# danieldugas/DeepMimic_mujoco

Hardware: AMD Instinct MI355X
Metric: env-steps/sec (whole node), 34-DoF humanoid, 4096 envs, at 1/2/4/8 MI355X (higher is better)
Workload: dtype f32

## Files before the change

deepmimic_mujoco_amd/_lib.py:

```python
from __future__ import annotations

import ctypes as C
import os

import numpy as np

from .model import DmModel, NQ, NV, NU, NOBS

_HERE = os.path.dirname(os.path.abspath(__file__))
LIB_PATH = os.path.join(_HERE, "libdeepmimic_hip.so")
DEBUG_STRIDE = 416

REASONS = {0: None, 1: "low_z", 2: "high_z", 3: "max_ep_len", 4: "acyclical_end",
           5: "sim_error", 6: "obs_out_of_bounds", 7: "fallen without amnesty"}
TASK_DPENV, TASK_COMBINED = 0, 1

EXPORTS = ["dm_default_config", "dm_create", "dm_destroy", "dm_last_error", "dm_num_envs",
           "dm_load_clip", "dm_set_env_clips", "dm_reset", "dm_step", "dm_step_forced", "dm_physics_step",
           "dm_set_state", "dm_get_state", "dm_get_counters", "dm_set_counters", "dm_set_debug",
           "dm_fill_random_actions", "dm_last_step_ms", "dm_enable_timing", "dm_get_work",
           "dm_set_clip_flags", "dm_obs_dim", "dm_terms_dim", "dm_get_env_clips", "dm_mean_step_ms", "dm_ppo_loss", "dm_forward", "dm_linear_wgrad", "dm_ppo_gather", "dm_flat_adam_step", "dm_policy_sample",
           "dm_rollout_store", "dm_policy_pack", "dm_policy_forward", "dm_policy_packed_floats", "dm_ppo_mlp_grad", "dm_ppo_mlp_workspace_floats", "dm_flat_adam_update", "dm_flat_adam_step_gather", "dm_colsum", "dm_set_seed",
           "dm_linear_tanh", "dm_tanh_linear_wgrad", "dm_tanh_bwd_colsum",
           "dm_ppo_wide_grad", "dm_ppo_wide_packed_elems", "dm_ppo_wide_dp", "dm_ppo_wide_supported",
           "dm_sac_act", "dm_sac_store", "dm_sac_gather", "dm_sac_head_fwd", "dm_sac_critic_loss", "dm_sac_actor_loss",
           "dm_sac_head_bwd", "dm_sac_linear_relu", "dm_sac_relu_bwd_colsum", "dm_sac_polyak",
           "dm_rollout_finish", "dm_rollout_finish_workspace_bytes",
           "dm_policy_forward_bf16", "dm_rollout_store_bf16", "dm_ppo_gather_bf16", "dm_flat_adam_step_gather_bf16"]


class DmConfig(C.Structure):
    _fields_ = [("num_envs", C.c_int32), ("max_ep_length", C.c_int32),
                ("vel_obs_scale", C.c_float), ("low_z", C.c_float), ("high_z", C.c_float),
                ("w_pose", C.c_float), ("w_vel", C.c_float), ("w_end_eff", C.c_float),
                ("w_com", C.c_float), ("w_joint_limit", C.c_float), ("obs_bound", C.c_float),
                ("seed", C.c_uint64), ("auto_reset", C.c_int32), ("device", C.c_int32),
                ("lpt_schedule", C.c_int32), ("task", C.c_int32),
                ("amnesty_steps", C.c_int32), ("to_getup_len", C.c_int32),
                ("integrator", C.c_int32), ("stale_contact_slots", C.c_int32)]


INTEGRATORS = {None: 0, "model": 0, "Euler": 1, "euler": 1, "RK4": 2, "rk4": 2}


class DmPpoMlpStep(C.Structure):
    _fields_ = [("B", C.c_int32), ("D", C.c_int32), ("H1", C.c_int32), ("H2", C.c_int32), ("A", C.c_int32),
                ("normalize_advantage", C.c_int32), ("clip_range", C.c_float), ("vf_coef", C.c_float), ("ent_coef", C.c_float),
                ("reserved", C.c_int32),
                ("obs", C.c_void_p), ("act", C.c_void_p), ("adv", C.c_void_p), ("ret", C.c_void_p), ("old_logp", C.c_void_p),
                ("log_std", C.c_void_p),
                ("W", (C.c_void_p * 3) * 2), ("b", (C.c_void_p * 3) * 2), ("gW", (C.c_void_p * 3) * 2), ("gb", (C.c_void_p * 3) * 2),
                ("g_log_std", C.c_void_p), ("out8", C.c_void_p), ("workspace", C.c_void_p), ("workspace_floats", C.c_longlong),
                ("zero_ptr", C.c_void_p), ("zero_floats", C.c_longlong), ("adam_state2", C.c_void_p), ("loss_acc", C.c_void_p)]


class DmGatherSpec(C.Structure):
    _fields_ = [("idx", C.c_void_p), ("B", C.c_int32), ("D", C.c_int32), ("A", C.c_int32), ("reserved", C.c_int32),
                ("obs", C.c_void_p), ("act", C.c_void_p), ("adv", C.c_void_p), ("ret", C.c_void_p), ("logp", C.c_void_p),
                ("o_obs", C.c_void_p), ("o_act", C.c_void_p), ("o_adv", C.c_void_p), ("o_ret", C.c_void_p), ("o_logp", C.c_void_p)]


class DmGatherSpecBf16(DmGatherSpec):
    """include/deepmimic_hip.h: DmGatherSpecBf16 — DmGatherSpec's layout; obs / act point at bf16 rows"""


class DmPpoWideStep(C.Structure):
    _fields_ = [("B", C.c_int32), ("D", C.c_int32), ("H1", C.c_int32), ("H2", C.c_int32), ("A", C.c_int32),
                ("normalize_advantage", C.c_int32), ("clip_range", C.c_float), ("vf_coef", C.c_float), ("ent_coef", C.c_float),
                ("reserved", C.c_int32),
                ("obs", C.c_void_p), ("act", C.c_void_p), ("adv", C.c_void_p), ("ret", C.c_void_p), ("old_logp", C.c_void_p),
                ("log_std", C.c_void_p),
                ("W", (C.c_void_p * 3) * 2), ("b", (C.c_void_p * 3) * 2), ("gW", (C.c_void_p * 3) * 2), ("gb", (C.c_void_p * 3) * 2),
                ("g_log_std", C.c_void_p),
                ("wpk", C.c_void_p * 2), ("xbT", C.c_void_p), ("h1T", C.c_void_p * 2), ("dz1T", C.c_void_p * 2), ("h2T", C.c_void_p * 2),
                ("dz2T", C.c_void_p * 2), ("dz3T", C.c_void_p * 2), ("part", C.c_void_p), ("stats8", C.c_void_p), ("out8", C.c_void_p),
                ("zero_ptr", C.c_void_p), ("zero_floats", C.c_longlong), ("adam_state2", C.c_void_p), ("loss_acc", C.c_void_p)]


_LIB = None


def load_library():
    global _LIB
    if _LIB is not None:
        return _LIB
    if not os.path.exists(LIB_PATH):
        raise RuntimeError(
            "libdeepmimic_hip.so is missing (%s). Build it with `python -c 'import __graft_entry__ as g; "
            "g.build()'` or `make -C deepmimic_mujoco_amd/csrc`. There is no CPU fallback." % LIB_PATH)
    import torch
    L = C.CDLL(LIB_PATH)
    vp, i32 = C.c_void_p, C.c_int
    L.dm_default_config.argtypes = [C.POINTER(DmConfig)]
    L.dm_default_config.restype = None
    L.dm_create.argtypes = [C.POINTER(DmModel), C.POINTER(DmConfig), C.POINTER(vp)]
    L.dm_destroy.argtypes = [vp]
    L.dm_last_error.argtypes = [vp]
    L.dm_last_error.restype = C.c_char_p
    L.dm_num_envs.argtypes = [vp]
    L.dm_obs_dim.argtypes = [vp]
    L.dm_terms_dim.argtypes = [vp]
    L.dm_get_env_clips.argtypes = [vp, vp, vp]
    L.dm_load_clip.argtypes = [vp, i32, i32, vp, vp, vp, vp]
    L.dm_set_env_clips.argtypes = [vp, vp, vp]
    L.dm_reset.argtypes = [vp, vp, vp, vp, vp]
    L.dm_step.argtypes = [vp] * 9
    L.dm_step_forced.argtypes = [vp] * 9
    L.dm_physics_step.argtypes = [vp] * 3
    L.dm_set_state.argtypes = [vp, vp, i32, vp, vp, vp, vp, i32, vp]
    L.dm_get_state.argtypes = [vp, vp, i32, vp, vp, vp, vp, vp]
    L.dm_forward.argtypes = [vp, vp, i32, vp]
    L.dm_linear_wgrad.argtypes = [vp, vp, vp, vp, i32, i32, i32, vp]
    L.dm_policy_sample.argtypes = [vp, vp, i32, i32, C.c_uint64, vp, vp, vp, vp, vp, vp, vp]
    L.dm_rollout_store.argtypes = [i32, i32, i32] + [vp] * 16
    L.dm_rollout_store_bf16.argtypes = L.dm_rollout_store.argtypes
    L.dm_policy_packed_floats.argtypes = [i32] * 4
    L.dm_ppo_mlp_workspace_floats.argtypes = [i32] * 5
    L.dm_ppo_mlp_grad.argtypes = [C.POINTER(DmPpoMlpStep), vp]
    L.dm_ppo_wide_grad.argtypes = [C.POINTER(DmPpoWideStep), vp]
    L.dm_ppo_wide_packed_elems.argtypes = [i32, i32, i32]
    L.dm_ppo_wide_dp.argtypes = [i32]
    L.dm_ppo_wide_supported.argtypes = [i32] * 5
    L.dm_policy_pack.argtypes = [vp, vp, vp, i32, i32, i32, i32, vp, vp]
    L.dm_policy_forward.argtypes = [vp] + [i32] * 5 + [vp] * 9 + [C.c_uint64, vp, C.c_uint32, i32] + [vp] * 9
    L.dm_policy_forward_bf16.argtypes = L.dm_policy_forward.argtypes
    L.dm_flat_adam_step.argtypes = [vp, vp, vp, vp, i32] + [C.c_float] * 6 + [vp, i32, vp]
    L.dm_colsum.argtypes = [vp, i32, i32, vp, vp]
    L.dm_linear_tanh.argtypes = [vp, vp, vp, vp, i32, i32, i32, vp]
    L.dm_tanh_linear_wgrad.argtypes = [vp, vp, vp, vp, vp, i32, i32, i32, vp]
    L.dm_tanh_bwd_colsum.argtypes = [vp, vp, vp, vp, i32, i32, vp]
    L.dm_flat_adam_update.argtypes = [vp, vp, vp, vp, i32] + [C.c_float] * 6 + [vp, i32, vp]
    L.dm_flat_adam_step_gather.argtypes = [vp, vp, vp, vp, i32] + [C.c_float] * 6 + [vp, i32, i32, vp, vp]
    L.dm_flat_adam_step_gather.restype = i32
    L.dm_flat_adam_step_gather_bf16.argtypes = L.dm_flat_adam_step_gather.argtypes
    L.dm_ppo_gather.argtypes = [vp, i32, vp, i32, vp, i32, vp, vp, vp, vp, vp, vp, vp, vp, vp]
    L.dm_ppo_gather_bf16.argtypes = L.dm_ppo_gather.argtypes
    L.dm_get_counters.argtypes = [vp, vp, vp, vp, vp]
    L.dm_set_counters.argtypes = [vp, vp, vp, vp]
    L.dm_set_debug.argtypes = [vp, vp]
    L.dm_set_seed.argtypes = [vp, C.c_uint64]
    L.dm_get_work.argtypes = [vp, vp, vp]
    L.dm_set_clip_flags.argtypes = [vp, i32, i32]
    L.dm_fill_random_actions.argtypes = [vp, vp, C.c_uint32, vp]
    L.dm_last_step_ms.argtypes = [vp, C.POINTER(C.c_float)]
    L.dm_enable_timing.argtypes = [vp, i32]
    L.dm_ppo_loss.argtypes = [vp] * 7 + [i32, i32, C.c_float, C.c_float, C.c_float, i32] + [vp] * 6
    L.dm_mean_step_ms.argtypes = [vp, C.POINTER(C.c_float), C.POINTER(C.c_int32)]
    u64, f32 = C.c_uint64, C.c_float
    L.dm_sac_act.argtypes = [vp, i32, i32, i32, u64, vp, i32, i32, vp, vp, vp, vp, vp]
    L.dm_sac_store.argtypes = [i32, i32, i32, i32] + [vp] * 17
    L.dm_sac_gather.argtypes = [i32, i32, i32, i32, u64] + [vp] * 15
    L.dm_sac_head_fwd.argtypes = [vp, i32, i32, i32, u64, vp, vp, vp, i32, vp, vp, i32, f32, f32, vp]
    L.dm_sac_critic_loss.argtypes = [vp] * 5 + [i32, f32] + [vp] * 4
    L.dm_sac_actor_loss.argtypes = [vp, vp, i32, vp, vp, vp]
    L.dm_sac_head_bwd.argtypes = [vp, i32, i32, u64, vp, vp, i32, i32, vp, vp, vp, vp]
    L.dm_sac_linear_relu.argtypes = [vp, i32, vp, vp, vp, i32, i32, i32, i32, vp]
    L.dm_sac_relu_bwd_colsum.argtypes = [vp, vp, vp, vp, i32, i32, i32, vp]
    L.dm_sac_polyak.argtypes = [vp, vp, C.c_longlong, f32, vp, vp]
    L.dm_rollout_finish_workspace_bytes.argtypes = [i32, i32]
    L.dm_rollout_finish.argtypes = [i32, i32, vp, vp, i32, vp, vp, C.c_double, C.c_double] + [vp] * 7 + [C.c_longlong, vp]
    for name in EXPORTS:
        if name not in ("dm_default_config", "dm_last_error"):
            getattr(L, name).restype = C.c_longlong if name in ("dm_policy_packed_floats", "dm_ppo_mlp_workspace_floats", "dm_ppo_wide_packed_elems", "dm_rollout_finish_workspace_bytes") else C.c_int
    _LIB = L
    return L


def default_config(**kw) -> DmConfig:
    cfg = DmConfig()
    load_library().dm_default_config(C.byref(cfg))
    for k, v in kw.items():
        setattr(cfg, k, v)
    return cfg


def _ptr(t):
    return None if t is None else C.c_void_p(t.data_ptr())


class HipEngine:

    def __init__(self, model, num_envs, device=0, seed=1234, auto_reset=True, integrator=None, **cfg_kw):
        import torch
        cfg_kw["integrator"] = INTEGRATORS[integrator]
        if not torch.cuda.is_available():
            raise RuntimeError("no MI355X visible to HIP: the DeepMimic engine has no CPU fallback")
        self.torch = torch
        self.L = load_library()
        self.model = model
        self.N = int(num_envs)
        self.device = torch.device("cuda", device)
        self.cfg = default_config(num_envs=self.N, device=device, seed=seed,
                                  auto_reset=1 if auto_reset else 0, **cfg_kw)
        h = C.c_void_p()
        rc = self.L.dm_create(C.byref(model.cstruct), C.byref(self.cfg), C.byref(h))
        if rc != 0:
            raise RuntimeError("dm_create failed with code %d" % rc)
        self.h = h
        self.obs_dim = self.L.dm_obs_dim(h)
        self.terms_dim = self.L.dm_terms_dim(h)
        self.clip_len = {}
        self._debug = None

    def set_seed(self, seed):
        self._chk(self.L.dm_set_seed(self.h, C.c_uint64(int(seed) & 0xFFFFFFFFFFFFFFFF)), "dm_set_seed")

    def close(self):
        if getattr(self, "h", None):
            self.L.dm_destroy(self.h)
            self.h = None

    def __del__(self):
        try:
            self.close()
        except Exception:
            pass

    def _chk(self, rc, what):
        if rc != 0:
            msg = self.L.dm_last_error(self.h)
            raise RuntimeError("%s failed (%d): %s" % (what, rc, msg.decode() if msg else ""))

    def _stream(self):
        return C.c_void_p(self.torch.cuda.current_stream(self.device).cuda_stream)

    def load_clip(self, clip_id, mocap, floor=False, acyclic=False):
        q, v, b, g = [np.ascontiguousarray(a, np.float64) for a in mocap.tables()]
        self._chk(self.L.dm_load_clip(self.h, clip_id, len(q), q.ctypes.data_as(C.c_void_p),
                                      v.ctypes.data_as(C.c_void_p), b.ctypes.data_as(C.c_void_p),
                                      g.ctypes.data_as(C.c_void_p)), "dm_load_clip")
        self.clip_len[clip_id] = len(q)
        self._chk(self.L.dm_set_clip_flags(self.h, clip_id, (1 if floor else 0) | (2 if acyclic else 0)), "dm_set_clip_flags")

    def set_env_clips(self, clip_ids):
        t = None if clip_ids is None else clip_ids.to(self.device, self.torch.int32).contiguous()
        self._chk(self.L.dm_set_env_clips(self.h, _ptr(t), self._stream()), "dm_set_env_clips")
        self._keep = t

    def get_env_clips(self):
        out = self.torch.zeros(self.N, dtype=self.torch.int32, device=self.device)
        self._chk(self.L.dm_get_env_clips(self.h, _ptr(out), self._stream()), "dm_get_env_clips")
        return out

    def alloc_outputs(self):
        t, d = self.torch, self.device
        return dict(obs=t.zeros(self.N, self.obs_dim, device=d), rew=t.zeros(self.N, device=d),
                    done=t.zeros(self.N, dtype=t.uint8, device=d), terms=t.zeros(self.N, self.terms_dim, device=d),
                    reason=t.zeros(self.N, dtype=t.int32, device=d),
                    terminal_obs=t.zeros(self.N, self.obs_dim, device=d))

    def enable_debug(self, on=True):
        if on:
            self._debug = self.torch.zeros(self.N, DEBUG_STRIDE, device=self.device)
            self._chk(self.L.dm_set_debug(self.h, _ptr(self._debug)), "dm_set_debug")
        else:
            self._chk(self.L.dm_set_debug(self.h, None), "dm_set_debug")
            self._debug = None
        return self._debug

    def reset(self, obs, mask=None, idx_init=None):
        self._chk(self.L.dm_reset(self.h, _ptr(mask), _ptr(idx_init), _ptr(obs), self._stream()), "dm_reset")

    def step(self, actions, out):
        self._chk(self.L.dm_step(self.h, _ptr(actions), _ptr(out["obs"]), _ptr(out["rew"]), _ptr(out["done"]),
                                 _ptr(out.get("terms")), _ptr(out.get("reason")), _ptr(out.get("terminal_obs")),
                                 self._stream()), "dm_step")

    def physics_step(self, actions):
        self._chk(self.L.dm_physics_step(self.h, _ptr(actions), self._stream()), "dm_physics_step")

    def step_forced(self, qpos, qvel, out):
        self._chk(self.L.dm_step_forced(self.h, _ptr(qpos), _ptr(qvel), _ptr(out["obs"]), _ptr(out["rew"]),
                                        _ptr(out["done"]), _ptr(out.get("terms")), _ptr(out.get("reason")),
                                        self._stream()), "dm_step_forced")

    def set_state(self, qpos, qvel, warm=None, ctrl=None, env_ids=None, run_forward=False):
        n = qpos.shape[0]
        self._chk(self.L.dm_set_state(self.h, _ptr(env_ids), n, _ptr(qpos), _ptr(qvel), _ptr(warm), _ptr(ctrl),
                                      1 if run_forward else 0, self._stream()), "dm_set_state")

    def forward(self, env_ids=None, n=None):
        self._chk(self.L.dm_forward(self.h, _ptr(env_ids), self.N if n is None else n, self._stream()), "dm_forward")

    def get_state(self, env_ids=None, n=None):
        t, d = self.torch, self.device
        n = self.N if n is None else n
        qpos, qvel = t.zeros(n, NQ, device=d), t.zeros(n, NV, device=d)
        warm, ctrl = t.zeros(n, NV, device=d), t.zeros(n, NU, device=d)
        self._chk(self.L.dm_get_state(self.h, _ptr(env_ids), n, _ptr(qpos), _ptr(qvel), _ptr(warm), _ptr(ctrl),
                                      self._stream()), "dm_get_state")
        return qpos, qvel, warm, ctrl

    def get_counters(self):
        t, d = self.torch, self.device
        idx = t.zeros(self.N, dtype=t.int32, device=d)
        ln = t.zeros(self.N, dtype=t.int32, device=d)
        rew = t.zeros(self.N, device=d)
        self._chk(self.L.dm_get_counters(self.h, _ptr(idx), _ptr(ln), _ptr(rew), self._stream()), "dm_get_counters")
        return idx, ln, rew

    def set_counters(self, idx=None, ep_len=None):
        self._chk(self.L.dm_set_counters(self.h, _ptr(idx), _ptr(ep_len), self._stream()), "dm_set_counters")

    def fill_random_actions(self, actions, step_index):
        self._chk(self.L.dm_fill_random_actions(self.h, _ptr(actions), int(step_index), self._stream()),
                  "dm_fill_random_actions")

    def get_work(self):
        w = self.torch.zeros(self.N, dtype=self.torch.int32, device=self.device)
        self._chk(self.L.dm_get_work(self.h, _ptr(w), self._stream()), "dm_get_work")
        return w

    def enable_timing(self, on=True, stride=1):
        self._chk(self.L.dm_enable_timing(self.h, max(1, int(stride)) if on else 0), "dm_enable_timing")

    def mean_step_ms(self):
        ms, n = C.c_float(0), C.c_int32(0)
        self._chk(self.L.dm_mean_step_ms(self.h, C.byref(ms), C.byref(n)), "dm_mean_step_ms")
        return ms.value, n.value

    def last_step_ms(self):
        ms = C.c_float(0)
        self._chk(self.L.dm_last_step_ms(self.h, C.byref(ms)), "dm_last_step_ms")
        return ms.value
```

deepmimic_mujoco_amd/csrc/dm_abi.hip:

```cpp
#include "../../include/deepmimic_hip.h"
#include "dm_device.h"
#include "dm_topology.h"

#include <math.h>
#include <stdio.h>
#include <string.h>

#include <string>
#include <vector>

#include "dm_kernels.hip"
#include "dm_ppo.hip"
#include "dm_policy.hip"
#include "dm_ppo_mlp.hip"
#include "dm_ppo_wide.hip"
#include "dm_sac.hip"

struct DmEngine {
  DmConfig cfg;
  DmModel model;
  int N = 0;
  DmDev *dT = nullptr;
  float *dState = nullptr;
  float *dArScratch = nullptr;
  float *dClipRows[DM_MAX_CLIPS] = {nullptr};
  float *dClipReset[DM_MAX_CLIPS] = {nullptr};
  int clipL[DM_MAX_CLIPS] = {0};
  int clipFlags[DM_MAX_CLIPS] = {0};
  float *debug = nullptr;
  int32_t *dOrder = nullptr;
  int32_t *dCost = nullptr;
  static constexpr int NEV = 512;
  hipEvent_t ev0[NEV] = {}, ev1[NEV] = {};
  long nrec = 0;
  long nlaunch = 0;
  int stride = 1;
  int waves = 0;
  bool timing = false;
  float last_ms = 0;
  std::string err;
};

static int fail(DmEngine *e, int code, const char *what, hipError_t he = hipSuccess) {
  if (e) {
    e->err = what;
    if (he != hipSuccess) { e->err += ": "; e->err += hipGetErrorString(he); }
  }
  return code;
}
#define HIPCHK(e, call)                                   \
  do {                                                    \
    hipError_t _r = (call);                               \
    if (_r != hipSuccess) return fail(e, DM_EHIP, #call, _r); \
  } while (0)

extern "C" void dm_default_config(DmConfig *c) {
  memset(c, 0, sizeof(*c));
  c->num_envs = 1;
  c->max_ep_length = 1000;
  c->vel_obs_scale = 0.1f;
  c->low_z = 0.7f;
  c->high_z = 2.0f;
  c->w_pose = 0.75f; c->w_vel = 0.1f; c->w_end_eff = 0.15f; c->w_com = 0.0f; c->w_joint_limit = -0.1f;
  c->obs_bound = 100.0f;
  c->seed = 1234;
  c->auto_reset = 1;
  c->device = 0;
  c->lpt_schedule = 1;
  c->task = DM_TASK_DPENV;
  c->amnesty_steps = 150;
  c->to_getup_len = 180;
  c->integrator = DM_CFG_INT_MODEL;
}

static void build_tables(const DmModel &m, DmDev &T) {
  memset(&T, 0, sizeof(T));
  T.timestep = (float)m.timestep;
  T.tolerance = (float)m.tolerance;
  T.pgs_scale = (float)(1.0 / (m.meaninertia * (DM_NV > 1 ? DM_NV : 1)));
  for (int i = 0; i < 3; i++) T.gravity[i] = (float)m.gravity[i];
  double tc = fmax(m.solref[0], 2 * m.timestep), dr = m.solref[1], dmax = m.solimp[1];
  T.K = (float)(1.0 / fmax(1e-15, dmax * dmax * tc * tc * dr * dr));
  T.B = (float)(2.0 / fmax(1e-15, dmax * tc));
  for (int i = 0; i < 5; i++) T.solimp[i] = (float)m.solimp[i];
  double mt = 0;
  for (int b = 0; b < DM_NBODY; b++) mt += m.body_mass[b];
  T.total_mass_inv = (float)(1.0 / mt);
  for (int i = 0; i < DM_NQ; i++) T.qpos0[i] = (float)m.qpos0[i];
  T.iterations = m.iterations;
  T.npair = m.npair;
  T.torso_body = m.torso_body; T.rfoot_geom = m.rfoot_geom; T.lfoot_geom = m.lfoot_geom; T.floor_geom = m.floor_geom;
  for (int i = 0; i < 4; i++) T.ee_geom[i] = m.ee_geom[i];
  for (int b = 0; b < DM_NBODY; b++) {
    T.b_parent[b] = m.body_parent[b]; T.b_depth[b] = m.body_depth[b];
    T.b_dofadr[b] = m.body_dofadr[b] < 0 ? 0 : m.body_dofadr[b]; T.b_dofnum[b] = m.body_dofnum[b];
    for (int i = 0; i < 3; i++) { T.b_pos[b][i] = (float)m.body_pos[b][i]; T.b_ipos[b][i] = (float)m.body_ipos[b][i]; }
    for (int i = 0; i < 6; i++) T.b_inertia[b][i] = (float)m.body_inertia[b][i];
    T.b_mass[b] = (float)m.body_mass[b];
    T.b_invw[b] = (float)m.body_invweight0[b][0];
    uint32_t sub = 0;
    for (int c = 1; c < DM_NBODY; c++) {
      int a = c;
      while (a > 0 && a != b) a = m.body_parent[a];
      if (a == b && b > 0) sub |= 1u << c;
    }
    T.b_subtree[b] = sub;
    uint64_t chain = 0;
    for (int a = b; a > 0; a = m.body_parent[a])
      for (int k = 0; k < m.body_dofnum[a]; k++) chain |= 1ull << (m.body_dofadr[a] + k);
    T.b_chain[b] = chain;
    uint32_t cb = 0;
    int ids[8], nc = 0;
    for (int a = b; a > 0; a = m.body_parent[a]) ids[nc++] = a;
    for (int c = 0; c < nc && c < 4; c++) cb |= (uint32_t)ids[nc - 1 - c] << (8 * c);
    T.b_chainb[b] = cb;
  }
  for (int k = 0; k < DM_NV; k++) {
    int j = m.dof_jnt[k];
    T.d_body[k] = m.dof_body[k];
    T.d_act[k] = -1;
    T.d_limited[k] = (m.jnt_type[j] == DM_JNT_HINGE) ? m.jnt_limited[j] : 0;
    for (int i = 0; i < 3; i++) T.d_axis[k][i] = (float)m.jnt_axis[j][i];
    T.d_arm[k] = (float)m.dof_armature[k]; T.d_damp[k] = (float)m.dof_damping[k];
    T.d_invw[k] = (float)m.dof_invweight0[k];
    T.d_lo[k] = (float)m.jnt_range[j][0]; T.d_hi[k] = (float)m.jnt_range[j][1];
    int n = 0;
    for (int a = m.dof_parent[k]; a >= 0 && n < DMK_MAXANC; a = m.dof_parent[a]) T.d_anc[k][n++] = (uint8_t)a;
    T.d_nanc[k] = n;
    for (int d = 0; d < n; d++) T.d_ancabs[k][d] = T.d_anc[k][n - 1 - d];
    T.d_pbody[k] = m.body_parent[m.dof_body[k]];
  }
  for (int k = 0; k < DM_NV; k++) {
    for (int a = 0; a < T.d_nanc[k]; a++) T.d_desc[T.d_anc[k][a]] |= 1ull << k;
    T.nanc_pack[k >> 4] |= (uint64_t)T.d_nanc[k] << (4 * (k & 15));
    for (int a = 0; a < T.d_nanc[k]; a++) T.d_ancm[k] |= 1ull << T.d_anc[k][a];
    T.d_madr[k] = m.dof_Madr[k];
  }
  for (int a = 0; a < DM_NU; a++) {
    int k = m.act_dof[a];
    T.d_act[k] = a; T.d_gear[k] = (float)m.act_gear[a];
    T.d_clo[k] = (float)m.act_ctrlrange[a][0]; T.d_chi[k] = (float)m.act_ctrlrange[a][1];
  }
  for (int g = 0; g < DM_NGEOM; g++) {
    T.g_body[g] = m.geom_body[g]; T.g_type[g] = m.geom_type[g]; T.g_condim[g] = m.geom_condim[g];
    for (int i = 0; i < 3; i++) { T.g_pos[g][i] = (float)m.geom_pos[g][i]; T.g_size[g][i] = (float)m.geom_size[g][i]; }
    const double *q = m.geom_quat[g];
    double w = q[0], x = q[1], y = q[2], z = q[3];
    double M[9] = {w * w + x * x - y * y - z * z, 2 * (x * y - w * z), 2 * (x * z + w * y),
                   2 * (x * y + w * z), w * w - x * x + y * y - z * z, 2 * (y * z - w * x),
                   2 * (x * z - w * y), 2 * (y * z + w * x), w * w - x * x - y * y + z * z};
    for (int i = 0; i < 9; i++) T.g_mat[g][i] = (float)M[i];
    T.g_rbound[g] = (float)m.geom_rbound[g]; T.g_margin[g] = (float)m.geom_margin[g];
    T.g_mu[g] = (float)m.geom_friction[g][0];
  }
  for (int p = 0; p < DM_MAXPAIR; p++) { T.p_g1[p] = (int16_t)m.pair_geom1[p]; T.p_g2[p] = (int16_t)m.pair_geom2[p]; }
  for (int p = 0; p < m.npair; p++) {
    int g1 = m.pair_geom1[p], g2 = m.pair_geom2[p];
    DmPairDev &pr = T.pairs[p];
    pr.g1 = (int16_t)g1; pr.g2 = (int16_t)g2;
    pr.t1 = (int8_t)m.geom_type[g1]; pr.t2 = (int8_t)m.geom_type[g2];
    pr.margin = (float)fmax(m.geom_margin[g1], m.geom_margin[g2]);
    pr.rbsum = (float)((m.geom_type[g1] == DM_GEOM_PLANE ? 0.0 : m.geom_rbound[g1]) + m.geom_rbound[g2]);
    for (int i = 0; i < 3; i++) { pr.z1[i] = (float)m.geom_size[g1][i]; pr.z2[i] = (float)m.geom_size[g2][i]; }
  }
  int p = 0;
  for (int b = 0; b < DMK_MAXANC; b++)
    for (int a = 0; a <= b; a++) { T.tri_a[p] = (uint8_t)a; T.tri_b[p] = (uint8_t)b; p++; }
}

static int check_model(DmEngine *e, const DmModel &m) {
  if (m.nq != DM_NQ || m.nv != DM_NV || m.nu != DM_NU || m.nbody != DM_NBODY || m.ngeom != DM_NGEOM)
    return fail(e, DM_EINVAL, "model dimensions do not match the compiled-in humanoid3d dimensions");
  if (m.integrator != DM_INT_RK4 && m.integrator != DM_INT_EULER) return fail(e, DM_EINVAL, "integrator must be RK4 or Euler");
  if (m.npair < 0 || m.npair > DM_MAXPAIR) return fail(e, DM_EINVAL, "npair out of range");
  for (int b = 1; b < DM_NBODY; b++) {
    if (m.body_quat[b][0] != 1.0) return fail(e, DM_EINVAL, "kernels assume identity body quaternions");
    if (m.body_dofnum[b] != 1 && m.body_dofnum[b] != 3 && m.body_dofnum[b] != 6)
      return fail(e, DM_EINVAL, "kernels assume 1- or 3-hinge bodies under a free root");
    if (m.body_depth[b] < 1 || m.body_depth[b] > 4) return fail(e, DM_EINVAL, "tree depth > 4");
  }
  for (int j = 0; j < DM_NJNT; j++)
    for (int i = 0; i < 3; i++)
      if (m.jnt_pos[j][i] != 0.0) return fail(e, DM_EINVAL, "kernels assume joint anchors at the body origin");
  if (m.jnt_type[0] != DM_JNT_FREE || m.jnt_body[0] != 1) return fail(e, DM_EINVAL, "joint 0 must be the free root");
  for (int k = 0; k < DM_NV; k++)
    if (m.dof_parent[k] != topo::PARENT[k] || m.dof_Madr[k] != topo::MADR[k])
      return fail(e, DM_EINVAL, "dof tree differs from the compiled-in topology (regenerate csrc/dm_topology.h)");
  for (int b = 0; b < DM_NBODY; b++)
    if (m.body_parent[b] != topo::BPARENT[b])
      return fail(e, DM_EINVAL, "body tree differs from the compiled-in topology (regenerate csrc/dm_topology.h)");
  return DM_OK;
}

extern "C" int dm_create(const DmModel *model, const DmConfig *cfg, DmHandle *out) {
  if (!model || !cfg || !out || cfg->num_envs < 1) return DM_EINVAL;
  int ndev = 0;
  if (hipGetDeviceCount(&ndev) != hipSuccess || ndev <= 0) return DM_ENODEV;
  DmEngine *e = new DmEngine();
  e->cfg = *cfg;
  e->model = *model;
  e->N = cfg->num_envs;
  if (const char *w = getenv("DM_WAVES")) e->waves = atoi(w);
  int rc = check_model(e, *model);
  if (rc != DM_OK) { fprintf(stderr, "dm_create: %s\n", e->err.c_str()); delete e; return rc; }
  if (hipSetDevice(cfg->device) != hipSuccess) { delete e; return DM_ENODEV; }
  DmDev T;
  build_tables(*model, T);
  if (hipMalloc(&e->dT, sizeof(DmDev)) != hipSuccess) { delete e; return DM_ENOMEM; }
  hipMemcpy(e->dT, &T, sizeof(DmDev), hipMemcpyHostToDevice);
  size_t sb = (size_t)e->N * DMK_STATE_STRIDE * sizeof(float);
  if (hipMalloc(&e->dState, sb) != hipSuccess) { hipFree(e->dT); delete e; return DM_ENOMEM; }
  std::vector<float> init((size_t)e->N * DMK_STATE_STRIDE, 0.f);
  for (int i = 0; i < e->N; i++)
    for (int k = 0; k < DM_NQ; k++) init[(size_t)i * DMK_STATE_STRIDE + DMS_QPOS + k] = (float)model->qpos0[k];
  hipMemcpy(e->dState, init.data(), sb, hipMemcpyHostToDevice);
  if (hipMalloc(&e->dArScratch, (size_t)e->N * DMK_MAXROW * DMK_MAXROW * sizeof(float)) != hipSuccess) {
    hipFree(e->dState); hipFree(e->dT); delete e; return DM_ENOMEM;
  }
  if (hipMalloc(&e->dOrder, e->N * sizeof(int32_t)) != hipSuccess || hipMalloc(&e->dCost, e->N * sizeof(int32_t)) != hipSuccess) {
    hipFree(e->dArScratch); hipFree(e->dState); hipFree(e->dT); delete e; return DM_ENOMEM;
  }
  hipMemset(e->dCost, 0, e->N * sizeof(int32_t));
  { std::vector<int32_t> ident(e->N);
    for (int i = 0; i < e->N; i++) ident[i] = i;
    hipMemcpy(e->dOrder, ident.data(), e->N * sizeof(int32_t), hipMemcpyHostToDevice); }
  for (int i = 0; i < DmEngine::NEV; i++) { hipEventCreate(&e->ev0[i]); hipEventCreate(&e->ev1[i]); }
  *out = e;
  return DM_OK;
}

extern "C" int dm_destroy(DmHandle e) {
  if (!e) return DM_EINVAL;
  hipSetDevice(e->cfg.device);
  hipDeviceSynchronize();
  for (int i = 0; i < DM_MAX_CLIPS; i++) { if (e->dClipRows[i]) hipFree(e->dClipRows[i]); if (e->dClipReset[i]) hipFree(e->dClipReset[i]); }
  if (e->dState) hipFree(e->dState);
  if (e->dArScratch) hipFree(e->dArScratch);
  if (e->dOrder) hipFree(e->dOrder);
  if (e->dCost) hipFree(e->dCost);
  if (e->dT) hipFree(e->dT);
  for (int i = 0; i < DmEngine::NEV; i++) { if (e->ev0[i]) hipEventDestroy(e->ev0[i]); if (e->ev1[i]) hipEventDestroy(e->ev1[i]); }
  delete e;
  return DM_OK;
}

extern "C" const char *dm_last_error(DmHandle e) { return e ? e->err.c_str() : "null handle"; }
extern "C" int dm_num_envs(DmHandle e) { return e ? e->N : DM_EINVAL; }
extern "C" int dm_obs_dim(DmHandle e) { return e ? (e->cfg.task == DM_TASK_COMBINED ? DM_NOBS_COMBINED : DM_NOBS) : DM_EINVAL; }
extern "C" int dm_terms_dim(DmHandle e) { return e ? (e->cfg.task == DM_TASK_COMBINED ? 8 : 5) : DM_EINVAL; }

extern "C" int dm_load_clip(DmHandle e, int clip_id, int L, const double *qpos, const double *qvel,
                            const double *body_xpos, const double *geom_xpos) {
  if (!e || clip_id < 0 || clip_id >= DM_MAX_CLIPS || L < 1 || !qpos || !qvel || !body_xpos || !geom_xpos)
    return fail(e, DM_EINVAL, "dm_load_clip: bad argument");
  HIPCHK(e, hipSetDevice(e->cfg.device));
  const DmModel &m = e->model;
  std::vector<float> rows((size_t)L * DMK_CLIP_ROW, 0.f), reset((size_t)L * DMK_RESET_ROW, 0.f);
  double mt = 0;
  for (int b = 0; b < DM_NBODY; b++) mt += m.body_mass[b];
  for (int f = 0; f < L; f++) {
    float *r = &rows[(size_t)f * DMK_CLIP_ROW];
    const double *q = qpos + (size_t)f * DM_NQ, *v = qvel + (size_t)f * DM_NV;
    for (int i = 0; i < 28; i++) { r[i] = (float)q[7 + i]; r[28 + i] = (float)v[6 + i]; }
    for (int i = 0; i < 4; i++) r[56 + i] = (float)q[3 + i];
    for (int ee = 0; ee < 4; ee++)
      for (int i = 0; i < 3; i++) r[60 + 3 * ee + i] = (float)geom_xpos[((size_t)f * DM_NGEOM + m.ee_geom[ee]) * 3 + i];
    for (int i = 0; i < 3; i++) {
      double c = 0;
      for (int b = 0; b < DM_NBODY; b++) c += body_xpos[((size_t)f * DM_NBODY + b) * 3 + i] * m.body_mass[b];
      r[72 + i] = (float)(c / mt);
      r[75 + i] = (float)q[i];
    }
    r[78] = (float)v[0]; r[79] = (float)v[1];
    float *rr = &reset[(size_t)f * DMK_RESET_ROW];
    for (int i = 0; i < DM_NQ; i++) rr[i] = (float)q[i];
    for (int i = 0; i < DM_NV; i++) rr[35 + i] = (float)v[i];
  }
  if (e->dClipRows[clip_id]) { hipFree(e->dClipRows[clip_id]); hipFree(e->dClipReset[clip_id]); }
  HIPCHK(e, hipMalloc(&e->dClipRows[clip_id], rows.size() * sizeof(float)));
  HIPCHK(e, hipMalloc(&e->dClipReset[clip_id], reset.size() * sizeof(float)));
  HIPCHK(e, hipMemcpy(e->dClipRows[clip_id], rows.data(), rows.size() * sizeof(float), hipMemcpyHostToDevice));
  HIPCHK(e, hipMemcpy(e->dClipReset[clip_id], reset.data(), reset.size() * sizeof(float), hipMemcpyHostToDevice));
  e->clipL[clip_id] = L;
  return DM_OK;
}

__global__ void dm_schedule_kernel(const int32_t *cost, int32_t *order, int n);

__global__ void dm_set_clip_kernel(float *state, const int32_t *ids, int n) {
  int i = blockIdx.x * blockDim.x + threadIdx.x;
  if (i < n) reinterpret_cast<int *>(state + (size_t)i * DMK_STATE_STRIDE)[DMS_CLIP] = ids ? ids[i] : 0;
}
__global__ void dm_get_clip_kernel(const float *state, int32_t *ids, int n) {
  int i = blockIdx.x * blockDim.x + threadIdx.x;
  if (i < n) ids[i] = reinterpret_cast<const int *>(state + (size_t)i * DMK_STATE_STRIDE)[DMS_CLIP];
}
__global__ void dm_counters_kernel(float *state, int n, int32_t *idx, int32_t *len, float *rew, const int32_t *sidx,
                                   const int32_t *slen) {
  int i = blockIdx.x * blockDim.x + threadIdx.x;
  if (i >= n) return;
  int *si = reinterpret_cast<int *>(state + (size_t)i * DMK_STATE_STRIDE);
  if (sidx) si[DMS_IDX] = sidx[i];
  if (slen) si[DMS_EPLEN] = slen[i];
  if (idx) idx[i] = si[DMS_IDX];
  if (len) len[i] = si[DMS_EPLEN];
  if (rew) rew[i] = state[(size_t)i * DMK_STATE_STRIDE + DMS_EPREW];
}
__global__ void dm_get_state_kernel(const float *state, const int32_t *ids, int n, int N, float *qpos, float *qvel,
                                    float *warm, float *ctrl) {
  int slot = blockIdx.x, lane = threadIdx.x;
  if (slot >= n) return;
  int env = ids ? ids[slot] : slot;
  if (env < 0 || env >= N) return;
  const float *st = state + (size_t)env * DMK_STATE_STRIDE;
  if (qpos && lane < DM_NQ) qpos[(size_t)slot * DM_NQ + lane] = st[DMS_QPOS + lane];
  if (qvel && lane < DM_NV) qvel[(size_t)slot * DM_NV + lane] = st[DMS_QVEL + lane];
  if (warm && lane < DM_NV) warm[(size_t)slot * DM_NV + lane] = st[DMS_WARM + lane];
  if (ctrl && lane < DM_NU) ctrl[(size_t)slot * DM_NU + lane] = st[DMS_CTRL + lane];
}

extern "C" int dm_get_env_clips(DmHandle e, int32_t *clip_ids, void *stream) {
  if (!e || !clip_ids) return DM_EINVAL;
  HIPCHK(e, hipSetDevice(e->cfg.device));
  hipLaunchKernelGGL(dm_get_clip_kernel, dim3((e->N + 255) / 256), dim3(256), 0, (hipStream_t)stream, e->dState, clip_ids, e->N);
  HIPCHK(e, hipGetLastError());
  return DM_OK;
}

extern "C" int dm_set_clip_flags(DmHandle e, int clip_id, int flags) {
  if (!e || clip_id < 0 || clip_id >= DM_MAX_CLIPS) return DM_EINVAL;
  e->clipFlags[clip_id] = flags;
  return DM_OK;
}

extern "C" int dm_set_env_clips(DmHandle e, const int32_t *clip_ids, void *stream) {
  if (!e) return DM_EINVAL;
  HIPCHK(e, hipSetDevice(e->cfg.device));
  hipLaunchKernelGGL(dm_set_clip_kernel, dim3((e->N + 255) / 256), dim3(256), 0, (hipStream_t)stream, e->dState, clip_ids, e->N);
  HIPCHK(e, hipGetLastError());
  return DM_OK;
}

static void fill_launch(DmEngine *e, DmLaunch &P, int mode) {
  memset(&P, 0, sizeof(P));
  P.T = e->dT;
  P.state = e->dState;
  P.ar_scratch = e->dArScratch;
  for (int i = 0; i < DM_MAX_CLIPS; i++) { P.clips[i].rows = e->dClipRows[i]; P.clips[i].reset = e->dClipReset[i]; P.clips[i].L = e->clipL[i]; P.clips[i].flags = e->clipFlags[i]; }
  P.N = e->N; P.mode = mode; P.auto_reset = e->cfg.auto_reset; P.max_ep_length = e->cfg.max_ep_length;
  P.vel_obs_scale = e->cfg.vel_obs_scale; P.low_z = e->cfg.low_z; P.high_z = e->cfg.high_z; P.obs_bound = e->cfg.obs_bound;
  P.w_pose = e->cfg.w_pose; P.w_vel = e->cfg.w_vel; P.w_ee = e->cfg.w_end_eff; P.w_com = e->cfg.w_com; P.w_jl = e->cfg.w_joint_limit;
  P.seed = e->cfg.seed;
  P.amnesty_steps = e->cfg.amnesty_steps; P.to_getup_len = e->cfg.to_getup_len;
  P.integrator = e->cfg.integrator == DM_CFG_INT_EULER ? DM_INT_EULER : e->cfg.integrator == DM_CFG_INT_RK4 ? DM_INT_RK4 : e->model.integrator;
  P.f8 = e->cfg.stale_contact_slots ? 1 : 0;
  P.debug = e->debug;
}

static int launch(DmEngine *e, DmLaunch &P, int nslots, void *stream) {
  P.nslots = nslots;
  if (e->clipL[0] < 1) return fail(e, DM_EINVAL, "no clip loaded (dm_load_clip clip 0 first)");
  if (e->cfg.task == DM_TASK_COMBINED && (e->clipL[1] < 1 || e->clipL[2] < 2))
    return fail(e, DM_EINVAL, "combined task needs clips 0,1,2 = walk, run, getup");
  HIPCHK(e, hipSetDevice(e->cfg.device));
  hipStream_t s = (hipStream_t)stream;
  const int evi = (int)(e->nrec % DmEngine::NEV);
  const bool rec = e->timing && (e->nlaunch++ % e->stride) == 0;
  if (rec) hipEventRecord(e->ev0[evi], s);
  const dim3 grid((P.nslots + DMK_ENVS_PER_BLOCK - 1) / DMK_ENVS_PER_BLOCK), block(64 * DMK_ENVS_PER_BLOCK);
  const bool three_waves = e->waves == 3 || (e->waves == 0 && P.nslots >= 3072);
  if (e->cfg.task == DM_TASK_COMBINED) {
    if (three_waves) hipLaunchKernelGGL(dm_step_combined_kernel_w3, grid, block, 0, s, P);
    else hipLaunchKernelGGL(dm_step_combined_kernel, grid, block, 0, s, P);
#ifdef DM_EXPERIMENT_W4
  } else if (e->waves == 4) {
    hipLaunchKernelGGL(dm_step_kernel_w4, grid, block, 0, s, P);
#endif
  } else if (three_waves) {
    hipLaunchKernelGGL(dm_step_kernel_w3, grid, block, 0, s, P);
  } else {
    hipLaunchKernelGGL(dm_step_kernel, grid, block, 0, s, P);
  }
  if (rec) { hipEventRecord(e->ev1[evi], s); e->nrec++; }
  HIPCHK(e, hipGetLastError());
  return DM_OK;
}

extern "C" int dm_reset(DmHandle e, const uint8_t *mask, const int32_t *idx_init, float *obs_out, void *stream) {
  if (!e) return DM_EINVAL;
  DmLaunch P;
  fill_launch(e, P, DMK_MODE_RESET);
  P.mask = mask; P.idx_init = idx_init; P.obs = obs_out;
  return launch(e, P, e->N, stream);
}

extern "C" int dm_step(DmHandle e, const float *actions, float *obs, float *rew, uint8_t *done, float *terms,
                       int32_t *reason, float *terminal_obs, void *stream) {
  if (!e || !actions || !obs || !rew || !done) return fail(e, DM_EINVAL, "dm_step: null buffer");
  DmLaunch P;
  fill_launch(e, P, DMK_MODE_STEP);
  P.actions = actions; P.obs = obs; P.rew = rew; P.done = done; P.terms = terms; P.reason = reason; P.terminal_obs = terminal_obs;
  P.cost = e->dCost;
  if (e->cfg.lpt_schedule) {
    HIPCHK(e, hipSetDevice(e->cfg.device));
    hipLaunchKernelGGL(dm_schedule_kernel, dim3(1), dim3(1024), 0, (hipStream_t)stream, e->dCost, e->dOrder, e->N);
    P.env_ids = e->dOrder;
  }
  return launch(e, P, e->N, stream);
}

extern "C" int dm_physics_step(DmHandle e, const float *actions, void *stream) {
  if (!e || !actions) return fail(e, DM_EINVAL, "dm_physics_step: null buffer");
  DmLaunch P;
  fill_launch(e, P, DMK_MODE_PHYSICS);
  P.actions = actions;
  P.auto_reset = 0;
  if (e->cfg.lpt_schedule) {
    HIPCHK(e, hipSetDevice(e->cfg.device));
    hipLaunchKernelGGL(dm_schedule_kernel, dim3(1), dim3(1024), 0, (hipStream_t)stream, e->dCost, e->dOrder, e->N);
    P.env_ids = e->dOrder;
  }
  return launch(e, P, e->N, stream);
}

extern "C" int dm_step_forced(DmHandle e, const float *qpos, const float *qvel, float *obs, float *rew, uint8_t *done,
                              float *terms, int32_t *reason, void *stream) {
  if (!e || !qpos || !qvel || !obs || !rew || !done) return fail(e, DM_EINVAL, "dm_step_forced: null buffer");
  DmLaunch P;
  fill_launch(e, P, DMK_MODE_FORCED);
  P.in_qpos = qpos; P.in_qvel = qvel; P.obs = obs; P.rew = rew; P.done = done; P.terms = terms; P.reason = reason;
  P.auto_reset = 0;
  return launch(e, P, e->N, stream);
}

extern "C" int dm_set_state(DmHandle e, const int32_t *env_ids, int n, const float *qpos, const float *qvel,
                            const float *warm, const float *ctrl, int run_forward, void *stream) {
  if (!e || !qpos || !qvel || n < 1 || n > e->N) return fail(e, DM_EINVAL, "dm_set_state: bad argument");
  DmLaunch P;
  fill_launch(e, P, DMK_MODE_SETSTATE);
  P.env_ids = env_ids; P.in_qpos = qpos; P.in_qvel = qvel; P.in_warm = warm; P.in_ctrl = ctrl; P.run_forward = run_forward;
  return launch(e, P, n, stream);
}

extern "C" int dm_forward(DmHandle e, const int32_t *env_ids, int n, void *stream) {
  if (!e || n < 1 || n > e->N) return fail(e, DM_EINVAL, "dm_forward: bad argument");
  DmLaunch P;
  fill_launch(e, P, DMK_MODE_SETSTATE);
  P.env_ids = env_ids; P.run_forward = 1;
  return launch(e, P, n, stream);
}

extern "C" int dm_get_state(DmHandle e, const int32_t *env_ids, int n, float *qpos, float *qvel, float *warm,
                            float *ctrl, void *stream) {
  if (!e || n < 1 || n > e->N) return fail(e, DM_EINVAL, "dm_get_state: bad argument");
  HIPCHK(e, hipSetDevice(e->cfg.device));
  hipLaunchKernelGGL(dm_get_state_kernel, dim3(n), dim3(64), 0, (hipStream_t)stream, e->dState, env_ids, n, e->N, qpos, qvel, warm, ctrl);
  HIPCHK(e, hipGetLastError());
  return DM_OK;
}

extern "C" int dm_get_counters(DmHandle e, int32_t *idx, int32_t *len, float *rew, void *stream) {
  if (!e) return DM_EINVAL;
  HIPCHK(e, hipSetDevice(e->cfg.device));
  hipLaunchKernelGGL(dm_counters_kernel, dim3((e->N + 255) / 256), dim3(256), 0, (hipStream_t)stream, e->dState, e->N, idx, len, rew,
                     (const int32_t *)nullptr, (const int32_t *)nullptr);
  HIPCHK(e, hipGetLastError());
  return DM_OK;
}
extern "C" int dm_set_counters(DmHandle e, const int32_t *idx, const int32_t *len, void *stream) {
  if (!e) return DM_EINVAL;
  HIPCHK(e, hipSetDevice(e->cfg.device));
  hipLaunchKernelGGL(dm_counters_kernel, dim3((e->N + 255) / 256), dim3(256), 0, (hipStream_t)stream, e->dState, e->N,
                     (int32_t *)nullptr, (int32_t *)nullptr, (float *)nullptr, idx, len);
  HIPCHK(e, hipGetLastError());
  return DM_OK;
}

__global__ void dm_schedule_kernel(const int32_t *cost, int32_t *order, int n) {
  __shared__ int hist[256];
  __shared__ int base[256];
  const int tid = threadIdx.x;
  if (tid < 256) hist[tid] = 0;
  __syncthreads();
  for (int i = tid; i < n; i += 1024) {
    int b = cost[i] >> 5;
    b = 255 - (b > 255 ? 255 : (b < 0 ? 0 : b));
    atomicAdd(&hist[b], 1);
  }
  __syncthreads();
  if (tid == 0) {
    int acc = 0;
    for (int b = 0; b < 256; b++) { base[b] = acc; acc += hist[b]; }
  }
  __syncthreads();
  for (int i = tid; i < n; i += 1024) {
    int b = cost[i] >> 5;
    b = 255 - (b > 255 ? 255 : (b < 0 ? 0 : b));
    order[atomicAdd(&base[b], 1)] = i;
  }
}

extern "C" int dm_get_work(DmHandle e, int32_t *work_out, void *stream) {
  if (!e || !work_out) return DM_EINVAL;
  HIPCHK(e, hipSetDevice(e->cfg.device));
  HIPCHK(e, hipMemcpyAsync(work_out, e->dCost, e->N * sizeof(int32_t), hipMemcpyDeviceToDevice, (hipStream_t)stream));
  return DM_OK;
}

extern "C" int dm_set_seed(DmHandle e, uint64_t seed) {
  if (!e) return DM_EINVAL;
  e->cfg.seed = seed;
  return DM_OK;
}

extern "C" int dm_set_debug(DmHandle e, float *buf) {
  if (!e) return DM_EINVAL;
  e->debug = buf;
  return DM_OK;
}

extern "C" int dm_fill_random_actions(DmHandle e, float *actions, uint32_t step_index, void *stream) {
  if (!e || !actions) return DM_EINVAL;
  HIPCHK(e, hipSetDevice(e->cfg.device));
  int n = e->N * DM_NU;
  hipLaunchKernelGGL(dm_fill_actions_kernel, dim3((n + 255) / 256), dim3(256), 0, (hipStream_t)stream, actions, e->N, e->cfg.seed, step_index);
  HIPCHK(e, hipGetLastError());
  return DM_OK;
}

extern "C" int dm_enable_timing(DmHandle e, int enable) {
  if (!e) return DM_EINVAL;
  e->timing = enable != 0;
  e->stride = enable > 1 ? enable : 1;
  e->nrec = 0;
  e->nlaunch = 0;
  return DM_OK;
}
extern "C" int dm_last_step_ms(DmHandle e, float *ms) {
  if (!e || !ms || !e->timing || e->nrec < 1) return DM_EINVAL;
  const int i = (int)((e->nrec - 1) % DmEngine::NEV);
  HIPCHK(e, hipEventSynchronize(e->ev1[i]));
  HIPCHK(e, hipEventElapsedTime(ms, e->ev0[i], e->ev1[i]));
  return DM_OK;
}
extern "C" int dm_mean_step_ms(DmHandle e, float *ms, int32_t *count) {
  if (!e || !ms || !e->timing || e->nrec < 1) return DM_EINVAL;
  const long n = e->nrec < DmEngine::NEV ? e->nrec : DmEngine::NEV;
  double acc = 0;
  for (long k = 0; k < n; k++) {
    const int i = (int)((e->nrec - 1 - k) % DmEngine::NEV);
    float t = 0;
    HIPCHK(e, hipEventSynchronize(e->ev1[i]));
    HIPCHK(e, hipEventElapsedTime(&t, e->ev0[i], e->ev1[i]));
    acc += t;
  }
  *ms = (float)(acc / (double)n);
  if (count) *count = (int32_t)n;
  return DM_OK;
}
```

deepmimic_mujoco_amd/csrc/dm_device.h:

```cpp
#pragma once

#include <hip/hip_runtime.h>
#include <stdint.h>

#include "../../include/dm_model.h"

#define DMK_NQ DM_NQ
#define DMK_NV DM_NV
#define DMK_NU DM_NU
#define DMK_NB DM_NBODY
#define DMK_NG DM_NGEOM
#define DMK_MAXCON DM_MAXCON
#define DMK_MAXROW DM_MAXROW
#define DMK_LANEROW 64
#define DMK_REGROW 32
#define DMK_MSTRIDE 35
#define DMK_MAXANC 12
#define DMK_STATE_STRIDE 144
#define DMK_CLIP_ROW 80

struct DmPairDev {
  int16_t g1, g2;
  int8_t t1, t2, pad0, pad1;
  float margin, rbsum;
  float z1[3], z2[3];
};

struct DmDev {
  float timestep, tolerance, pgs_scale, gravity[3];
  float K, B;
  float solimp[5];
  float total_mass_inv;
  float qpos0[36];
  int32_t iterations, npair;
  int32_t torso_body, rfoot_geom, lfoot_geom, floor_geom;
  int32_t ee_geom[4];
  int32_t b_parent[16], b_depth[16], b_dofadr[16], b_dofnum[16];
  float b_pos[16][3], b_ipos[16][3], b_inertia[16][6], b_mass[16], b_invw[16];
  uint32_t b_subtree[16];
  uint64_t b_chain[16];
  uint32_t b_chainb[16];
  int32_t d_body[DM_NV], d_nanc[DM_NV], d_act[DM_NV], d_limited[DM_NV];
  float d_axis[DM_NV][3];
  float d_arm[DM_NV], d_damp[DM_NV], d_invw[DM_NV], d_lo[DM_NV], d_hi[DM_NV];
  float d_gear[DM_NV], d_clo[DM_NV], d_chi[DM_NV];
  uint8_t d_anc[DM_NV][DMK_MAXANC];
  uint8_t d_ancabs[DM_NV][DMK_MAXANC + 4];
  uint64_t d_desc[DM_NV];
  int32_t d_pbody[DM_NV];
  uint64_t nanc_pack[3];
  uint64_t d_ancm[DM_NV];
  int32_t d_madr[DM_NV];
  int32_t g_body[16], g_type[16], g_condim[16];
  float g_pos[16][3], g_mat[16][9], g_size[16][3], g_rbound[16], g_margin[16], g_mu[16];
  int16_t p_g1[DM_MAXPAIR], p_g2[DM_MAXPAIR];
  DmPairDev pairs[DM_MAXPAIR];
  uint8_t tri_a[80], tri_b[80];
};

struct EnvLds {
  float qpos[36], qvel[36], warm[36], ctrl[28];
  float qacc_smooth[36], qacc[36];
  float cs[36][2];
  float xpos[DMK_NB][3], xquat[DMK_NB][4], xmat[DMK_NB][9], xipos[DMK_NB][3];
  float xaxis[DMK_NV][3];
  float gpos[DMK_NG][3], gmat[DMK_NG][9];
  float com[4];
  float cinert[DMK_NB][10];
  float cdof[DMK_NV][8];
  float cvel[DMK_NB][6];
  float M[DM_NM + 2];
  float dinv[36], dsqrtinv[36];
  float rk[5][36], rkq[4];
  float c_dist[DMK_MAXCON], c_pos[DMK_MAXCON][3], c_frame[DMK_MAXCON][9];
  int32_t c_g1[DMK_MAXCON], c_g2[DMK_MAXCON];
#ifdef DM_PROFILE
  unsigned long long prof_t, prof_t0; unsigned prof[16], prof_stage[4];
#endif
  int32_t info[8];
  int16_t rowinfo[DMK_MAXROW];
  union {
    struct {
      float crb[DMK_NB][10];
      float qloc[DMK_NB][8];
      union {
        struct { float cdofdot[DMK_NV][6]; float cacc[DMK_NB][6]; };
        alignas(16) float mbuf[DMK_NV][8];
      };
      float cfrc[DMK_NB][6], cfrcsub[DMK_NB][6];
    } v;
    struct {
      float tr[20][DM_NV + 1];
    } fin;
    struct {
      float poly[2][16][3];
      float cand[8][8];
      int32_t ncand;
    } bb;
  } u;
};

#define DMS_QPOS 0
#define DMS_QVEL 35
#define DMS_WARM 69
#define DMS_CTRL 103
#define DMS_IDX 131
#define DMS_EPLEN 132
#define DMS_EPREW 133
#define DMS_CLIP 134
#define DMS_RCNT 135
#define DMS_F8R 136
#define DMS_F8L 137

#define DMK_RESET_ROW 72

struct DmClipDev {
  const float *rows;
  const float *reset;
  int32_t L, flags;
};

enum { DMK_MODE_STEP = 0, DMK_MODE_FORCED = 1, DMK_MODE_RESET = 2, DMK_MODE_SETSTATE = 3,
       DMK_MODE_PHYSICS = 4 };

struct DmLaunch {
  const DmDev *T;
  float *state;
  float *ar_scratch;
  DmClipDev clips[8];
  int32_t N, nslots, mode, auto_reset, max_ep_length;
  int32_t amnesty_steps, to_getup_len;
  int32_t integrator, f8;
  float vel_obs_scale, low_z, high_z, obs_bound;
  float w_pose, w_vel, w_ee, w_com, w_jl;
  uint64_t seed;
  const float *actions;
  const float *in_qpos;
  const float *in_qvel;
  const float *in_warm;
  const float *in_ctrl;
  const int32_t *env_ids;
  int32_t *cost;
  const uint8_t *mask;
  const int32_t *idx_init;
  int32_t run_forward;
  float *obs, *rew, *terms, *terminal_obs, *debug;
  uint8_t *done;
  int32_t *reason;
};
```

deepmimic_mujoco_amd/csrc/dm_kernels.hip:

```cpp
#include "../../include/deepmimic_hip.h"
#include "dm_device.h"
#include "dm_topology.h"

#include <math.h>

#include <type_traits>

#define SYNC()                                              \
  do {                                                      \
    __builtin_amdgcn_fence(__ATOMIC_RELEASE, "wavefront");  \
    __builtin_amdgcn_wave_barrier();                        \
    __builtin_amdgcn_fence(__ATOMIC_ACQUIRE, "wavefront");  \
  } while (0)
#define DMK_ENVS_PER_BLOCK 1
#ifndef DMK_WAVES_PER_SIMD
#define DMK_WAVES_PER_SIMD 2
#endif
#ifdef DM_PROFILE
#define PROF_DECL do { if ((threadIdx.x & 63) == 0) { for (int _i = 0; _i < 16; _i++) g_S.prof[_i] = 0; for (int _i = 0; _i < 4; _i++) g_S.prof_stage[_i] = 0; g_S.prof_t = g_S.prof_t0 = __builtin_amdgcn_s_memtime(); } } while (0)
#define PROF_STAGE(i) do { if ((threadIdx.x & 63) == 0 && (i) < 4) g_S.prof_stage[i] = (unsigned)(__builtin_amdgcn_s_memtime() - g_S.prof_t0); } while (0)
#define PROF(i) do { if ((threadIdx.x & 63) == 0) { unsigned long long _t = __builtin_amdgcn_s_memtime(); g_S.prof[i] += (unsigned)(_t - g_S.prof_t); g_S.prof_t = _t; } } while (0)
#if DM_PROFILE == 2
#define PROF2(i) PROF(i)
#else
#define PROF2(i) do {} while (0)
#endif
#else
#define PROF2(i) do {} while (0)
#define PROF_STAGE(i) do {} while (0)
#define PROF_DECL do {} while (0)
#define PROF(i) do {} while (0)
#endif
typedef __attribute__((address_space(3))) const float *lds_cfloat_p;
typedef float mfma_f16v __attribute__((ext_vector_type(16)));
#ifndef DMK_MFMA_MIN_ROWS
#define DMK_MFMA_MIN_ROWS 8
#endif
typedef const __attribute__((address_space(1))) DmDev GDev;
typedef const __attribute__((address_space(1))) DmPairDev GPair;
#define MINVALF 1e-15f
#define MAXVALF 1e10f

namespace {

template <int I, int N>
struct StaticFor {
  template <class F>
  static __device__ __forceinline__ void run(F &&f) {
    if constexpr (I < N) {
      if (f(std::integral_constant<int, I>{})) StaticFor<I + 1, N>::run(f);
    }
  }
};

__device__ __forceinline__ float rl(float v, int lane) {
  return __int_as_float(__builtin_amdgcn_readlane(__float_as_int(v), lane));
}
template <unsigned long long MASK>
__device__ __forceinline__ float lane_sel(float a, float b) {
  float out;
  asm("v_cndmask_b32_e64 %0, %1, %2, %3" : "=v"(out) : "v"(b), "v"(a), "s"(MASK));
  return out;
}
template <unsigned long long MASK>
__device__ __forceinline__ int lane_sel_i(int a, int b) {
  int out;
  asm("v_cndmask_b32_e64 %0, %1, %2, %3" : "=v"(out) : "v"(b), "v"(a), "s"(MASK));
  return out;
}
template <int K, int I>
struct ElimAnc {
  static __device__ __forceinline__ void run(float (&C)[DMK_NV], const float Cs) {
    if constexpr (I >= 0) {
      C[I] = fmaf(-rl(Cs, I), C[K], C[I]);
      ElimAnc<K, (I >= 0 ? topo::PARENT[I >= 0 ? I : 0] : -1)>::run(C, Cs);
    }
  }
};
__device__ __forceinline__ float solve_LT(float x, const float dv, const int negdep, const float *M) {
  StaticFor<0, DMK_NV - 1>::run([&](auto ic) {
    constexpr int i = DMK_NV - 1 - decltype(ic)::value;
    const float xi = rl(x * dv, i);
    const float l = lane_sel<topo::anc_mask(i)>(M[topo::MADR[i] + topo::NANC[i] + negdep], 0.f);
    x = fmaf(-l, xi, x);
    return true;
  });
  return x;
}
__device__ __forceinline__ float solve_L(float x, const float dv, const int mrow, const float *M) {
  StaticFor<0, DMK_NV - 1>::run([&](auto jc) {
    constexpr int j = decltype(jc)::value;
    const float xj = rl(x * dv, j);
    const float l = lane_sel<topo::desc_mask(j)>(M[mrow - topo::NANC[j]], 0.f);
    x = fmaf(-l, xj, x);
    return true;
  });
  return x;
}
template <int CTRL>
__device__ __forceinline__ float dpp_mov(float v) {
  return __int_as_float(__builtin_amdgcn_update_dpp(0, __float_as_int(v), CTRL, 0xF, 0xF, true));
}
__device__ __forceinline__ float wave_sum(float v) {
  v += dpp_mov<0xB1>(v);
  v += dpp_mov<0x4E>(v);
  v += dpp_mov<0x141>(v);
  v += dpp_mov<0x140>(v);
  return (rl(v, 0) + rl(v, 16)) + (rl(v, 32) + rl(v, 48));
}
__device__ __forceinline__ unsigned long long lanemask_lt(int lane) {
  return (lane == 0) ? 0ull : (~0ull >> (64 - lane));
}
__device__ __forceinline__ int prefix_count(bool flag, int lane, int *total) {
  unsigned long long m = __ballot(flag);
  *total = __popcll(m);
  return __popcll(m & lanemask_lt(lane));
}

__device__ __forceinline__ void cross3(float *r, const float *a, const float *b) {
  float x = a[1] * b[2] - a[2] * b[1], y = a[2] * b[0] - a[0] * b[2], z = a[0] * b[1] - a[1] * b[0];
  r[0] = x; r[1] = y; r[2] = z;
}
__device__ __forceinline__ float dot3(const float *a, const float *b) {
  return a[0] * b[0] + a[1] * b[1] + a[2] * b[2];
}
__device__ __forceinline__ void quat_mul(float *r, const float *a, const float *b) {
  float w = a[0] * b[0] - a[1] * b[1] - a[2] * b[2] - a[3] * b[3];
  float x = a[0] * b[1] + a[1] * b[0] + a[2] * b[3] - a[3] * b[2];
  float y = a[0] * b[2] - a[1] * b[3] + a[2] * b[0] + a[3] * b[1];
  float z = a[0] * b[3] + a[1] * b[2] - a[2] * b[1] + a[3] * b[0];
  r[0] = w; r[1] = x; r[2] = y; r[3] = z;
}
__device__ __forceinline__ void quat_rot(float *r, const float *q, const float *v) {
  float t[3], u[3];
  cross3(t, q + 1, v);
  t[0] *= 2.f; t[1] *= 2.f; t[2] *= 2.f;
  cross3(u, q + 1, t);
  r[0] = v[0] + q[0] * t[0] + u[0];
  r[1] = v[1] + q[0] * t[1] + u[1];
  r[2] = v[2] + q[0] * t[2] + u[2];
}
__device__ __forceinline__ void quat2mat(float *m, const float *q) {
  float w = q[0], x = q[1], y = q[2], z = q[3];
  m[0] = w * w + x * x - y * y - z * z; m[1] = 2 * (x * y - w * z); m[2] = 2 * (x * z + w * y);
  m[3] = 2 * (x * y + w * z); m[4] = w * w - x * x + y * y - z * z; m[5] = 2 * (y * z - w * x);
  m[6] = 2 * (x * z - w * y); m[7] = 2 * (y * z + w * x); m[8] = w * w - x * x - y * y + z * z;
}
__device__ __forceinline__ void quat_normalize(float *q) {
  float n = sqrtf(q[0] * q[0] + q[1] * q[1] + q[2] * q[2] + q[3] * q[3]);
  if (n < MINVALF) { q[0] = 1; q[1] = q[2] = q[3] = 0; }
  else { float i = 1.0f / n; q[0] *= i; q[1] *= i; q[2] *= i; q[3] *= i; }
}
__device__ __forceinline__ void mat_vec(float *r, const float *m, const float *v) {
  float x = m[0] * v[0] + m[1] * v[1] + m[2] * v[2];
  float y = m[3] * v[0] + m[4] * v[1] + m[5] * v[2];
  float z = m[6] * v[0] + m[7] * v[1] + m[8] * v[2];
  r[0] = x; r[1] = y; r[2] = z;
}
__device__ __forceinline__ void mat_t_vec(float *r, const float *m, const float *v) {
  float x = m[0] * v[0] + m[3] * v[1] + m[6] * v[2];
  float y = m[1] * v[0] + m[4] * v[1] + m[7] * v[2];
  float z = m[2] * v[0] + m[5] * v[1] + m[8] * v[2];
  r[0] = x; r[1] = y; r[2] = z;
}
__device__ __forceinline__ void mul_inert_vec(float *r, const float *I, const float *v) {
  r[0] = I[0] * v[0] + I[3] * v[1] + I[4] * v[2] - I[8] * v[4] + I[7] * v[5];
  r[1] = I[3] * v[0] + I[1] * v[1] + I[5] * v[2] - I[6] * v[5] + I[8] * v[3];
  r[2] = I[4] * v[0] + I[5] * v[1] + I[2] * v[2] - I[7] * v[3] + I[6] * v[4];
  r[3] = I[8] * v[1] - I[7] * v[2] + I[9] * v[3];
  r[4] = I[6] * v[2] - I[8] * v[0] + I[9] * v[4];
  r[5] = I[7] * v[0] - I[6] * v[1] + I[9] * v[5];
}
__device__ __forceinline__ void cross_motion(float *r, const float *vel, const float *v) {
  float a[3], b[3], c[3];
  cross3(a, vel, v);
  cross3(b, vel, v + 3);
  cross3(c, vel + 3, v);
  r[0] = a[0]; r[1] = a[1]; r[2] = a[2];
  r[3] = b[0] + c[0]; r[4] = b[1] + c[1]; r[5] = b[2] + c[2];
}
__device__ __forceinline__ void cross_force(float *r, const float *vel, const float *f) {
  float a[3], b[3], c[3];
  cross3(a, vel, f);
  cross3(b, vel + 3, f + 3);
  cross3(c, vel, f + 3);
  r[0] = a[0] + b[0]; r[1] = a[1] + b[1]; r[2] = a[2] + b[2];
  r[3] = c[0]; r[4] = c[1]; r[5] = c[2];
}
__device__ __forceinline__ float clampf(float x, float lo, float hi) { return fminf(fmaxf(x, lo), hi); }

__device__ __forceinline__ void quat_to_rpy(const float *q, float *rpy) {
  float w = q[0], x = q[1], y = q[2], z = q[3];
  rpy[0] = atan2f(2 * (w * x + y * z), 1 - 2 * (x * x + y * y));
  rpy[1] = asinf(clampf(2 * (w * y - z * x), -1.f, 1.f));
  rpy[2] = atan2f(2 * (w * z + x * y), 1 - 2 * (y * y + z * z));
}

__device__ __host__ __forceinline__ uint32_t dm_hash32(uint64_t seed, uint32_t env, uint32_t step, uint32_t j) {
  uint64_t x = seed ^ ((uint64_t)env * 0x9E3779B97F4A7C15ull) ^ ((uint64_t)step * 0xBF58476D1CE4E5B9ull) ^
               ((uint64_t)j * 0x94D049BB133111EBull);
  x ^= x >> 30; x *= 0xBF58476D1CE4E5B9ull;
  x ^= x >> 27; x *= 0x94D049BB133111EBull;
  x ^= x >> 31;
  return (uint32_t)(x >> 32);
}

struct Cand {
  float d[4], p[4][3], n[4][3], t[3];
  int valid;
};

template <int S>
__device__ __forceinline__ void np_plane_sphere(Cand &c, float margin, const float *ppos, const float *pn,
                                                const float *spos, float r) {
  float df[3] = {spos[0] - ppos[0], spos[1] - ppos[1], spos[2] - ppos[2]};
  float dist = dot3(df, pn) - r;
  if (dist > margin) return;
  c.valid |= 1 << S;
  c.d[S] = dist;
  for (int i = 0; i < 3; i++) { c.n[S][i] = pn[i]; c.p[S][i] = spos[i] - pn[i] * (r + 0.5f * dist); }
}
template <int S>
__device__ __forceinline__ void np_sphere_sphere(Cand &c, float margin, const float *p1, float r1,
                                                 const float *p2, float r2) {
  float df[3] = {p2[0] - p1[0], p2[1] - p1[1], p2[2] - p1[2]};
  float cd = sqrtf(dot3(df, df)), dist = cd - r1 - r2;
  if (dist > margin) return;
  c.valid |= 1 << S;
  c.d[S] = dist;
  float inv = (cd < MINVALF) ? 0.f : 1.0f / cd;
  c.n[S][0] = (cd < MINVALF) ? 1.f : df[0] * inv;
  c.n[S][1] = df[1] * inv;
  c.n[S][2] = df[2] * inv;
  for (int i = 0; i < 3; i++) c.p[S][i] = p1[i] + c.n[S][i] * (r1 + 0.5f * dist);
}
template <int S>
__device__ __forceinline__ void np_sphere_box(Cand &c, float margin, const float *spos, float r,
                                              const float *bpos, const float *bmat, const float *size) {
  float t[3] = {spos[0] - bpos[0], spos[1] - bpos[1], spos[2] - bpos[2]}, ctr[3], cl[3], nl[3];
  mat_t_vec(ctr, bmat, t);
  for (int i = 0; i < 3; i++) { cl[i] = clampf(ctr[i], -size[i], size[i]); nl[i] = cl[i] - ctr[i]; }
  float dd = sqrtf(dot3(nl, nl)), dist;
  if (dd - r > margin) return;
  if (dd <= MINVALF) {
    float closest = 2 * (size[0] + size[1] + size[2]);
    int k = 0;
#pragma unroll
    for (int i = 0; i < 6; i++) {
      float test = size[i / 2] - ((i % 2) ? -1.0f : 1.0f) * ctr[i / 2];
      if (test < closest) { closest = test; k = i; }
    }
    nl[0] = nl[1] = nl[2] = 0;
    float sgn = (k % 2) ? 1.0f : -1.0f;
    if (k / 2 == 0) nl[0] = sgn; else if (k / 2 == 1) nl[1] = sgn; else nl[2] = sgn;
    dist = -closest - r;
  } else {
    float inv = 1.0f / dd;
    nl[0] *= inv; nl[1] *= inv; nl[2] *= inv;
    dist = dd - r;
  }
  float pl[3] = {ctr[0] + nl[0] * (r + 0.5f * dist), ctr[1] + nl[1] * (r + 0.5f * dist),
                 ctr[2] + nl[2] * (r + 0.5f * dist)};
  c.valid |= 1 << S;
  c.d[S] = dist;
  mat_vec(c.n[S], bmat, nl);
  mat_vec(t, bmat, pl);
  for (int i = 0; i < 3; i++) c.p[S][i] = t[i] + bpos[i];
}
__device__ __forceinline__ float cb_grad(const float *p, const float *a, const float *size, float t) {
  float g = 0;
  for (int i = 0; i < 3; i++) {
    float x = p[i] + a[i] * t;
    g += a[i] * (x - clampf(x, -size[i], size[i]));
  }
  return g;
}

__device__ __forceinline__ void make_frame(float *f) {
  float n = sqrtf(dot3(f, f));
  if (n < MINVALF) { f[0] = 1; f[1] = 0; f[2] = 0; }
  else { float i = 1.f / n; f[0] *= i; f[1] *= i; f[2] *= i; }
  if (sqrtf(dot3(f + 3, f + 3)) < 0.5f) {
    f[3] = f[4] = f[5] = 0;
    if (f[1] < 0.5f && f[1] > -0.5f) f[4] = 1; else f[5] = 1;
  }
  float t = dot3(f, f + 3);
  f[3] -= t * f[0]; f[4] -= t * f[1]; f[5] -= t * f[2];
  n = sqrtf(dot3(f + 3, f + 3));
  if (n < MINVALF) { f[3] = 1; f[4] = 0; f[5] = 0; }
  else { float i = 1.f / n; f[3] *= i; f[4] *= i; f[5] *= i; }
  cross3(f + 6, f, f + 3);
}

__device__ __noinline__ void np_box_box(EnvLds &S, GPair *pr) {
  const float margin = pr->margin;
  float p1[3], p2[3], R1[9], R2[9], s1[3], s2[3];
  for (int i = 0; i < 3; i++) { p1[i] = S.gpos[pr->g1][i]; p2[i] = S.gpos[pr->g2][i]; s1[i] = pr->z1[i]; s2[i] = pr->z2[i]; }
  for (int i = 0; i < 9; i++) { R1[i] = S.gmat[pr->g1][i]; R2[i] = S.gmat[pr->g2][i]; }
  S.u.bb.ncand = 0;
  float R[9], AR[9], t[3], tw[3] = {p2[0] - p1[0], p2[1] - p1[1], p2[2] - p1[2]};
  mat_t_vec(t, R1, tw);
#pragma unroll
  for (int i = 0; i < 3; i++)
#pragma unroll
    for (int j = 0; j < 3; j++) {
      R[3 * i + j] = R1[i] * R2[j] + R1[3 + i] * R2[3 + j] + R1[6 + i] * R2[6 + j];
      AR[3 * i + j] = fabsf(R[3 * i + j]) + 1e-9f;
    }
  float best = -1e30f, bn[3] = {0, 0, 0};
  int code = -1;
#pragma unroll
  for (int i = 0; i < 3; i++) {
    float s = fabsf(t[i]) - (s1[i] + s2[0] * AR[3 * i] + s2[1] * AR[3 * i + 1] + s2[2] * AR[3 * i + 2]);
    if (s > margin) return;
    if (s > best) { best = s; code = i; }
  }
#pragma unroll
  for (int j = 0; j < 3; j++) {
    float tj = t[0] * R[j] + t[1] * R[3 + j] + t[2] * R[6 + j];
    float s = fabsf(tj) - (s2[j] + s1[0] * AR[j] + s1[1] * AR[3 + j] + s1[2] * AR[6 + j]);
    if (s > margin) return;
    if (s > best) { best = s; code = 3 + j; }
  }
#pragma unroll
  for (int i = 0; i < 3; i++)
#pragma unroll
    for (int j = 0; j < 3; j++) {
      float ei[3] = {0, 0, 0}, ej[3] = {R[j], R[3 + j], R[6 + j]}, ax[3];
      ei[i] = 1;
      cross3(ax, ei, ej);
      float l = sqrtf(dot3(ax, ax));
      if (l < 1e-6f) continue;
      ax[0] /= l; ax[1] /= l; ax[2] /= l;
      float ra = s1[0] * fabsf(ax[0]) + s1[1] * fabsf(ax[1]) + s1[2] * fabsf(ax[2]), rb = 0;
#pragma unroll
      for (int k = 0; k < 3; k++) {
        float ek[3] = {R[k], R[3 + k], R[6 + k]};
        rb += s2[k] * fabsf(dot3(ax, ek));
      }
      float s = fabsf(dot3(t, ax)) - (ra + rb);
      if (s > margin) return;
      if (s > best + 0.05f * fabsf(best) + 1e-6f) { best = s; code = 6 + 3 * i + j; bn[0] = ax[0]; bn[1] = ax[1]; bn[2] = ax[2]; }
    }
  if (code < 0) return;
  float (*cand)[8] = S.u.bb.cand;
  if (code >= 6) {
    int i = (code - 6) / 3, j = (code - 6) % 3;
    float n1[3] = {bn[0], bn[1], bn[2]};
    if (dot3(n1, t) < 0) { n1[0] = -n1[0]; n1[1] = -n1[1]; n1[2] = -n1[2]; }
    float pa[3], pb[3] = {t[0], t[1], t[2]};
    for (int k = 0; k < 3; k++) pa[k] = (k == i) ? 0.f : ((n1[k] > 0) ? s1[k] : -s1[k]);
    for (int k = 0; k < 3; k++) {
      if (k == j) continue;
      float ek[3] = {R[k], R[3 + k], R[6 + k]};
      float sg = (dot3(n1, ek) > 0) ? -s2[k] : s2[k];
      pb[0] += sg * ek[0]; pb[1] += sg * ek[1]; pb[2] += sg * ek[2];
    }
    float ua[3] = {0, 0, 0}, ub[3] = {R[j], R[3 + j], R[6 + j]}, w[3];
    ua[i] = 1;
    for (int k = 0; k < 3; k++) w[k] = pb[k] - pa[k];
    float uaub = dot3(ua, ub), q1 = dot3(ua, w), q2 = -dot3(ub, w), dd = 1 - uaub * uaub;
    float alpha = 0, beta = 0;
    if (dd > 1e-12f) { alpha = (q1 + uaub * q2) / dd; beta = (uaub * q1 + q2) / dd; }
    alpha = clampf(alpha, -s1[i], s1[i]);
    beta = clampf(beta, -s2[j], s2[j]);
    float mid[3], mw[3], nw[3];
    for (int k = 0; k < 3; k++) mid[k] = 0.5f * ((pa[k] + ua[k] * alpha) + (pb[k] + ub[k] * beta));
    mat_vec(mw, R1, mid);
    mat_vec(nw, R1, n1);
    cand[0][0] = best;
    for (int k = 0; k < 3; k++) { cand[0][1 + k] = mw[k] + p1[k]; cand[0][4 + k] = nw[k]; }
    S.u.bb.ncand = 1;
    return;
  }
  const float *Ra, *Rb, *sa, *sb, *pa, *pb;
  int ax, flip;
  if (code < 3) { Ra = R1; Rb = R2; sa = s1; sb = s2; pa = p1; pb = p2; ax = code; flip = 0; }
  else { Ra = R2; Rb = R1; sa = s2; sb = s1; pa = p2; pb = p1; ax = code - 3; flip = 1; }
  float nrm[3] = {Ra[ax], Ra[3 + ax], Ra[6 + ax]}, dab[3] = {pb[0] - pa[0], pb[1] - pa[1], pb[2] - pa[2]};
  if (dot3(nrm, dab) < 0) { nrm[0] = -nrm[0]; nrm[1] = -nrm[1]; nrm[2] = -nrm[2]; }
  int ib = 0;
  float bestd = -1, nb[3];
  mat_t_vec(nb, Rb, nrm);
  for (int k = 0; k < 3; k++) if (fabsf(nb[k]) > bestd) { bestd = fabsf(nb[k]); ib = k; }
  float sgn = (nb[ib] > 0) ? -1.0f : 1.0f;
  int u = (ib + 1) % 3, v = (ib + 2) % 3;
  float (*poly)[3] = S.u.bb.poly[0];
  float (*tmp)[3] = S.u.bb.poly[1];
  int np = 4;
  for (int q = 0; q < 4; q++) {
    float su = (q == 0 || q == 3) ? -sb[u] : sb[u], sv = (q < 2) ? -sb[v] : sb[v];
    float loc[3];
    loc[ib] = sgn * sb[ib]; loc[u] = su; loc[v] = sv;
    float w[3], rel[3], pq[3];
    mat_vec(w, Rb, loc);
    for (int k = 0; k < 3; k++) rel[k] = w[k] + pb[k] - pa[k];
    mat_t_vec(pq, Ra, rel);
    poly[q][0] = pq[0]; poly[q][1] = pq[1]; poly[q][2] = pq[2];
  }
  int axes[2] = {(ax + 1) % 3, (ax + 2) % 3};
  for (int e = 0; e < 2; e++)
    for (int sd = -1; sd <= 1; sd += 2) {
      int a = axes[e], nn = 0;
      for (int q = 0; q < np; q++) {
        float *Pq = poly[q], *Qq = poly[(q + 1) % np];
        float dp = sd * Pq[a] - sa[a], dq = sd * Qq[a] - sa[a];
        if (dp <= 0) { tmp[nn][0] = Pq[0]; tmp[nn][1] = Pq[1]; tmp[nn][2] = Pq[2]; nn++; }
        if ((dp < 0 && dq > 0) || (dp > 0 && dq < 0)) {
          float f = dp / (dp - dq);
          for (int k = 0; k < 3; k++) tmp[nn][k] = Pq[k] + f * (Qq[k] - Pq[k]);
          nn++;
        }
        if (nn >= 15) break;
      }
      np = nn;
      for (int q = 0; q < np; q++) { poly[q][0] = tmp[q][0]; poly[q][1] = tmp[q][1]; poly[q][2] = tmp[q][2]; }
      if (np == 0) return;
    }
  float nl[3];
  mat_t_vec(nl, Ra, nrm);
  int cnt = 0;
  for (int q = 0; q < np && cnt < 8; q++) {
    float pq[3] = {poly[q][0], poly[q][1], poly[q][2]};
    float depth = dot3(nl, pq) - sa[ax];
    if (depth > margin) continue;
    float pl[3], pw[3];
    for (int k = 0; k < 3; k++) pl[k] = pq[k] - nl[k] * 0.5f * depth;
    mat_vec(pw, Ra, pl);
    cand[cnt][0] = depth;
    for (int k = 0; k < 3; k++) { cand[cnt][1 + k] = pw[k] + pa[k]; cand[cnt][4 + k] = flip ? -nrm[k] : nrm[k]; }
    cnt++;
  }
  while (cnt > 4) {
    int w = 0;
    for (int q = 1; q < cnt; q++) if (cand[q][0] >= cand[w][0]) w = q;
    for (int q = w; q < cnt - 1; q++)
      for (int k = 0; k < 7; k++) cand[q][k] = cand[q + 1][k];
    cnt--;
  }
  S.u.bb.ncand = cnt;
}

__device__ __noinline__ float impedance_pow(float x, float mid, float power) {
  return (x <= mid) ? powf(x, power) / powf(mid, power - 1) : 1 - powf(1 - x, power) / powf(1 - mid, power - 1);
}
__device__ __forceinline__ float impedance(const float *solimp, float pos, float margin) {
  float dmin = solimp[0], dmax = solimp[1], width = solimp[2], mid = solimp[3], power = solimp[4];
  if (dmin == dmax || width <= MINVALF) return 0.5f * (dmin + dmax);
  float x = fabsf(pos - margin) / width;
  if (x >= 1) return dmax;
  if (x <= 0) return dmin;
  float y;
  if (power == 1) y = x;
  else if (power == 2) y = (x <= mid) ? x * x / mid : 1 - (1 - x) * (1 - x) / (1 - mid);
  else y = impedance_pow(x, mid, power);
  return dmin + y * (dmax - dmin);
}

}

__shared__ EnvLds g_S;

#define bp (T.b_parent[lb])
#define bdofadr (T.b_dofadr[lb])
#define bdofnum (T.b_dofnum[lb])
#define bpos (T.b_pos[lb])
#define bipos (T.b_ipos[lb])
#define binert (T.b_inertia[lb])
#define bsub (T.b_subtree[lb])
#define baxis(j) (T.d_axis[(bdofadr + (j)) < DMK_NV ? (bdofadr + (j)) : 0])
#define dbody (T.d_body[lk])
#define dnanc (T.d_nanc[lk])
#define dact (T.d_act[lk])
#define dlimited (T.d_limited[lk])
#define darm (T.d_arm[lk])
#define ddamp (T.d_damp[lk])
#define dlo (T.d_lo[lk])
#define dhi (T.d_hi[lk])
#define dgear (T.d_gear[lk])
#define dclo (T.d_clo[lk])
#define dchi (T.d_chi[lk])
#define gbody (T.g_body[lg])
#define gposl (T.g_pos[lg])
#define gmatl (T.g_mat[lg])

template <bool DAMP2 = false>
__device__ __forceinline__ float fwd_smooth(GDev &T, const int lane, const float rhs = 0.f) {
  EnvLds &S = g_S;
  const int lb = lane < DMK_NB ? lane : 0;
  const int lk = lane < DMK_NV ? lane : 0;
  const int lg = lane < DMK_NG ? lane : 0;
  const bool isbody = lane >= 1 && lane < DMK_NB, isdof = lane < DMK_NV;
  const float bmass = (lane < DMK_NB) ? T.b_mass[lb] : 0.f;
  const int b_dofadr = T.b_dofadr[lb], b_dofnum = T.b_dofnum[lb];
  const uint32_t b_chain4 = T.b_chainb[lb];
  const unsigned b_sub = T.b_subtree[lb];
  const int d_body = T.d_body[lk], d_nanc = T.d_nanc[lk], d_pbody = T.d_pbody[lk];
  const float mtot_inv = T.total_mass_inv;

  if constexpr (!DAMP2) {
  {
    float q[4] = {S.qpos[3], S.qpos[4], S.qpos[5], S.qpos[6]};
    quat_normalize(q);
    SYNC();
    if (lane < 4) S.qpos[3 + lane] = (lane == 0) ? q[0] : (lane == 1) ? q[1] : (lane == 2) ? q[2] : q[3];
    if (lane >= 6 && lane < DMK_NV) {
      float sn, cs;
      sincosf(0.5f * S.qpos[lane + 1], &sn, &cs);
      S.cs[lane][0] = cs; S.cs[lane][1] = sn;
    }
    SYNC();
  }
  PROF2(12);
  if (isbody) {
    float q[4] = {1.f, 0.f, 0.f, 0.f};
    if (lb == 1) {
      for (int i = 0; i < 4; i++) q[i] = S.qpos[3 + i];
    } else {
      {
        const int k = b_dofadr;
        const float al[3] = {T.d_axis[k][0], T.d_axis[k][1], T.d_axis[k][2]};
        S.xaxis[k][0] = al[0]; S.xaxis[k][1] = al[1]; S.xaxis[k][2] = al[2];
        const float c = S.cs[k][0], sn = S.cs[k][1];
        q[0] = c; q[1] = al[0] * sn; q[2] = al[1] * sn; q[3] = al[2] * sn;
      }
#pragma unroll
      for (int j = 1; j < 3; j++) {
        if (j < b_dofnum) {
          const int k = b_dofadr + j;
          const float al[3] = {T.d_axis[k][0], T.d_axis[k][1], T.d_axis[k][2]};
          float ax[3], ql[4], qn[4];
          quat_rot(ax, q, al);
          S.xaxis[k][0] = ax[0]; S.xaxis[k][1] = ax[1]; S.xaxis[k][2] = ax[2];
          const float c = S.cs[k][0], sn = S.cs[k][1];
          ql[0] = c; ql[1] = al[0] * sn; ql[2] = al[1] * sn; ql[3] = al[2] * sn;
          quat_mul(qn, q, ql);
          q[0] = qn[0]; q[1] = qn[1]; q[2] = qn[2]; q[3] = qn[3];
        }
      }
    }
    for (int i = 0; i < 4; i++) S.u.v.qloc[lb][i] = q[i];
    for (int i = 0; i < 3; i++) S.u.v.qloc[lb][4 + i] = (lb == 1) ? S.qpos[i] : T.b_pos[lb][i];
  }
  SYNC();
  if (isbody) {
    float q[4], pos[3];
    for (int i = 0; i < 4; i++) q[i] = S.u.v.qloc[1][i];
    for (int i = 0; i < 3; i++) pos[i] = S.u.v.qloc[1][4 + i];
#pragma unroll
    for (int c = 1; c < 4; c++) {
      const int cb = (b_chain4 >> (8 * c)) & 0xFF;
      if (cb != 0) {
        float ql[4], pl[3], t[3], qn[4];
        for (int i = 0; i < 4; i++) ql[i] = S.u.v.qloc[cb][i];
        for (int i = 0; i < 3; i++) pl[i] = S.u.v.qloc[cb][4 + i];
        quat_rot(t, q, pl);
        pos[0] += t[0]; pos[1] += t[1]; pos[2] += t[2];
        quat_mul(qn, q, ql);
        q[0] = qn[0]; q[1] = qn[1]; q[2] = qn[2]; q[3] = qn[3];
      }
    }
    quat_normalize(q);
    float m9[9], tv[3];
    quat2mat(m9, q);
    const float ip[3] = {T.b_ipos[lb][0], T.b_ipos[lb][1], T.b_ipos[lb][2]};
    mat_vec(tv, m9, ip);
    for (int i = 0; i < 3; i++) { S.xpos[lb][i] = pos[i]; S.xipos[lb][i] = pos[i] + tv[i]; }
    for (int i = 0; i < 4; i++) S.xquat[lb][i] = q[i];
    for (int i = 0; i < 9; i++) S.xmat[lb][i] = m9[i];
  }
  SYNC();
  PROF2(13);
  float com[3];
  {
    float ax[3] = {0.f, 0.f, 0.f};
    if (lane >= 6 && isdof) {
      const float pq[4] = {S.xquat[d_pbody][0], S.xquat[d_pbody][1], S.xquat[d_pbody][2], S.xquat[d_pbody][3]};
      const float al[3] = {S.xaxis[lk][0], S.xaxis[lk][1], S.xaxis[lk][2]};
      quat_rot(ax, pq, al);
    } else if (lane >= 3 && lane < 6) {
      ax[0] = S.xmat[1][lane - 3]; ax[1] = S.xmat[1][3 + lane - 3]; ax[2] = S.xmat[1][6 + lane - 3];
    }
    if (lane < DMK_NG) {
      const int gb = T.g_body[lg];
      float bm[9], tv[3], gl[3] = {T.g_pos[lg][0], T.g_pos[lg][1], T.g_pos[lg][2]}, gm[9];
      for (int i = 0; i < 9; i++) { bm[i] = S.xmat[gb][i]; gm[i] = T.g_mat[lg][i]; }
      mat_vec(tv, bm, gl);
      for (int i = 0; i < 3; i++) S.gpos[lg][i] = S.xpos[gb][i] + tv[i];
      for (int i = 0; i < 3; i++)
        for (int j = 0; j < 3; j++)
          S.gmat[lg][3 * i + j] = bm[3 * i] * gm[j] + bm[3 * i + 1] * gm[3 + j] + bm[3 * i + 2] * gm[6 + j];
    }
    const float xi[3] = {S.xipos[lb][0], S.xipos[lb][1], S.xipos[lb][2]};
    for (int i = 0; i < 3; i++) com[i] = wave_sum(bmass * xi[i]) * mtot_inv;
    if (lane == 0) { S.com[0] = com[0]; S.com[1] = com[1]; S.com[2] = com[2]; }
    SYNC();
    if (isdof) {
      float cd[6] = {0, 0, 0, 0, 0, 0};
      if (lane < 3) {
        cd[3 + lane] = 1.f;
      } else {
        const float off[3] = {com[0] - S.xpos[d_body][0], com[1] - S.xpos[d_body][1], com[2] - S.xpos[d_body][2]};
        cd[0] = ax[0]; cd[1] = ax[1]; cd[2] = ax[2];
        cross3(cd + 3, ax, off);
        S.xaxis[lk][0] = ax[0]; S.xaxis[lk][1] = ax[1]; S.xaxis[lk][2] = ax[2];
      }
      for (int i = 0; i < 6; i++) S.cdof[lk][i] = cd[i];
      S.cdof[lk][6] = 0; S.cdof[lk][7] = 0;
    }
  }
  PROF2(14);
  if (isbody) {
    float R[9], Tm[9], W[6], bi[6];
    for (int i = 0; i < 9; i++) R[i] = S.xmat[lb][i];
    for (int i = 0; i < 6; i++) bi[i] = T.b_inertia[lb][i];
    const float Ib[9] = {bi[0], bi[3], bi[4], bi[3], bi[1], bi[5], bi[4], bi[5], bi[2]};
    for (int i = 0; i < 3; i++)
      for (int j = 0; j < 3; j++) Tm[3 * i + j] = R[3 * i] * Ib[j] + R[3 * i + 1] * Ib[3 + j] + R[3 * i + 2] * Ib[6 + j];
    W[0] = Tm[0] * R[0] + Tm[1] * R[1] + Tm[2] * R[2];
    W[1] = Tm[3] * R[3] + Tm[4] * R[4] + Tm[5] * R[5];
    W[2] = Tm[6] * R[6] + Tm[7] * R[7] + Tm[8] * R[8];
    W[3] = Tm[0] * R[3] + Tm[1] * R[4] + Tm[2] * R[5];
    W[4] = Tm[0] * R[6] + Tm[1] * R[7] + Tm[2] * R[8];
    W[5] = Tm[3] * R[6] + Tm[4] * R[7] + Tm[5] * R[8];
    const float o[3] = {S.xipos[lb][0] - com[0], S.xipos[lb][1] - com[1], S.xipos[lb][2] - com[2]};
    const float oo = dot3(o, o);
    float *ci = S.cinert[lb];
    ci[0] = W[0] + bmass * (oo - o[0] * o[0]);
    ci[1] = W[1] + bmass * (oo - o[1] * o[1]);
    ci[2] = W[2] + bmass * (oo - o[2] * o[2]);
    ci[3] = W[3] - bmass * o[0] * o[1];
    ci[4] = W[4] - bmass * o[0] * o[2];
    ci[5] = W[5] - bmass * o[1] * o[2];
    ci[6] = bmass * o[0]; ci[7] = bmass * o[1]; ci[8] = bmass * o[2];
    ci[9] = bmass;
  }
  SYNC();
  PROF(1);
  }
  {
    float acc[10];
    for (int i = 0; i < 10; i++) acc[i] = 0;
    StaticFor<1, DMK_NB>::run([&](auto cc) {
      constexpr int c = decltype(cc)::value;
      const float w = lane_sel<topo::body_ancself_mask(c)>(1.f, 0.f);
#pragma unroll
      for (int i = 0; i < 10; i++) acc[i] = fmaf(w, g_S.cinert[c][i], acc[i]);
      return true;
    });
    if (isbody)
      for (int i = 0; i < 10; i++) S.u.v.crb[lb][i] = acc[i];
  }
  SYNC();
  float C[DMK_NV];
  {
    float cd[6] = {0, 0, 0, 0, 0, 0};
    if (isdof) {
      float buf[6], I[10];
      for (int i = 0; i < 10; i++) I[i] = S.u.v.crb[d_body][i];
      for (int i = 0; i < 6; i++) cd[i] = S.cdof[lk][i];
      mul_inert_vec(buf, I, cd);
      for (int i = 0; i < 6; i++) S.u.v.mbuf[lk][i] = buf[i];
    }
    SYNC();
    const float armv = isdof ? (DAMP2 ? fmaf(T.timestep, T.d_damp[lk], T.d_arm[lk]) : T.d_arm[lk]) : 0.f;
    float dots[DMK_NV];
    {
      const float *bufp = &S.u.v.mbuf[lane & 31][lane >> 5];
      mfma_f16v acc;
#pragma unroll
      for (int v = 0; v < 16; v++) acc[v] = 0.f;
#pragma unroll
      for (int p = 0; p < 3; p++) {
        const auto sw = __builtin_amdgcn_permlane32_swap(__float_as_uint(cd[2 * p]), __float_as_uint(cd[2 * p + 1]), false, false);
        acc = __builtin_amdgcn_mfma_f32_32x32x2f32(bufp[2 * p], __uint_as_float(sw[0]), acc, 0, 0, 0);
      }
#pragma unroll
      for (int v = 0; v < 16; v++) {
        const auto sw = __builtin_amdgcn_permlane32_swap(__float_as_uint(acc[v]), __float_as_uint(acc[v]), false, false);
        dots[(v / 4) * 8 + (v % 4)] = acc[v];
        dots[(v / 4) * 8 + (v % 4) + 4] = __uint_as_float(sw[1]);
      }
#pragma unroll
      for (int k = 32; k < DMK_NV; k++) {
        float d = 0;
#pragma unroll
        for (int i = 0; i < 6; i++) d = fmaf(cd[i], S.u.v.mbuf[k][i], d);
        dots[k] = d;
      }
    }
    StaticFor<0, DMK_NV>::run([&](auto kc) {
      constexpr int k = decltype(kc)::value;
      const float off = lane_sel<topo::anc_mask(k)>(dots[k], 0.f);
      C[k] = lane_sel<(1ull << k)>(dots[k] + armv, off);
      return true;
    });
  }
  PROF(2);
  StaticFor<0, DMK_NV - 1>::run([&](auto ic) {
    constexpr int k = DMK_NV - 1 - decltype(ic)::value;
    const float rk = __builtin_amdgcn_rcpf(rl(C[k], k));
    const float Cs = C[k] * rk;
    ElimAnc<k, topo::PARENT[k]>::run(C, Cs);
    return true;
  });
  const int d_nanc_s = isdof ? d_nanc : 0;
  {
    StaticFor<0, DMK_NV>::run([&](auto kc) {
      constexpr int k = decltype(kc)::value;
      const int real = topo::MADR[k] + topo::NANC[k] - d_nanc_s;
      const int idx = lane_sel_i<(topo::anc_mask(k) | (1ull << k))>(real, DM_NM + 1);
      g_S.M[idx] = C[k];
      return true;
    });
  }
  SYNC();
  float dv = 0.f;
  const int mrow = T.d_madr[lk] + d_nanc;
  const uint64_t ancm = T.d_ancm[lk];
  if (isdof) {
    const float Md = S.M[T.d_madr[lk]];
    dv = 1.0f / Md;
    S.dinv[lk] = dv;
    S.dsqrtinv[lk] = 1.0f / sqrtf(Md);
  }
  SYNC();
  PROF(3);
  float xs = 0;
  if constexpr (DAMP2) {
    xs = isdof ? rhs : 0.f;
  } else {
  if (isbody) {
    float w[6] = {0, 0, 0, 0, 0, 0};
    const int nd = (lb == 1) ? 6 : b_dofnum;
    for (int j = 0; j < 6; j++)
      if (j < nd) {
        const int k = b_dofadr + j;
        const float qv = S.qvel[k];
        for (int i = 0; i < 6; i++) w[i] += S.cdof[k][i] * qv;
      }
    for (int i = 0; i < 6; i++) S.u.v.cacc[lb][i] = w[i];
  }
  SYNC();
  if (isbody) {
    float cv[6] = {0, 0, 0, 0, 0, 0}, u[6] = {0, 0, 0, 0, 0, 0};
#pragma unroll
    for (int c = 0; c < 3; c++) {
      const int cb = (b_chain4 >> (8 * c)) & 0xFF;
      if (cb != 0 && cb != lb)
        for (int i = 0; i < 6; i++) cv[i] += S.u.v.cacc[cb][i];
    }
    if (lb == 1) {
      for (int k = 0; k < 3; k++) {
        const float qv = S.qvel[k];
        for (int i = 0; i < 6; i++) cv[i] += S.cdof[k][i] * qv;
      }
      float dd[3][6];
#pragma unroll
      for (int k = 3; k < 6; k++) {
        float cd[6];
        for (int i = 0; i < 6; i++) cd[i] = S.cdof[k][i];
        cross_motion(dd[k - 3], cv, cd);
      }
#pragma unroll
      for (int k = 3; k < 6; k++) {
        const float qv = S.qvel[k];
        for (int i = 0; i < 6; i++) { u[i] += dd[k - 3][i] * qv; cv[i] += S.cdof[k][i] * qv; }
      }
    } else {
#pragma unroll
      for (int j = 0; j < 3; j++) {
        if (j < b_dofnum) {
          const int k = b_dofadr + j;
          float cd[6], dd[6];
          const float qv = S.qvel[k];
          for (int i = 0; i < 6; i++) cd[i] = S.cdof[k][i];
          cross_motion(dd, cv, cd);
          for (int i = 0; i < 6; i++) { u[i] += dd[i] * qv; cv[i] += cd[i] * qv; }
        }
      }
    }
    for (int i = 0; i < 6; i++) { S.cvel[lb][i] = cv[i]; S.u.v.cfrcsub[lb][i] = u[i]; }
  }
  SYNC();
  PROF2(15);
  if (isbody) {
    float ca[6] = {0, 0, 0, -T.gravity[0], -T.gravity[1], -T.gravity[2]}, cv[6], I[10], f0[6], t0[6], t1[6];
#pragma unroll
    for (int c = 0; c < 4; c++) {
      const int cb = (b_chain4 >> (8 * c)) & 0xFF;
      if (cb != 0)
        for (int i = 0; i < 6; i++) ca[i] += S.u.v.cfrcsub[cb][i];
    }
    for (int i = 0; i < 6; i++) cv[i] = S.cvel[lb][i];
    for (int i = 0; i < 10; i++) I[i] = S.cinert[lb][i];
    mul_inert_vec(f0, I, ca);
    mul_inert_vec(t0, I, cv);
    cross_force(t1, cv, t0);
    for (int i = 0; i < 6; i++) S.u.v.cfrc[lb][i] = f0[i] + t1[i];
  }
  SYNC();
  {
    float acc[6] = {0, 0, 0, 0, 0, 0};
    StaticFor<1, DMK_NB>::run([&](auto cc) {
      constexpr int c = decltype(cc)::value;
      const float w = lane_sel<topo::body_ancself_mask(c)>(1.f, 0.f);
#pragma unroll
      for (int i = 0; i < 6; i++) acc[i] = fmaf(w, g_S.u.v.cfrc[c][i], acc[i]);
      return true;
    });
    if (isbody)
      for (int i = 0; i < 6; i++) S.u.v.cacc[lb][i] = acc[i];
  }
  SYNC();
  PROF2(10);
  if (isdof) {
    float bias = 0;
    for (int i = 0; i < 6; i++) bias += S.cdof[lk][i] * S.u.v.cacc[d_body][i];
    float act = 0;
    const int da = T.d_act[lk];
    if (da >= 0) act = T.d_gear[lk] * clampf(S.ctrl[da], T.d_clo[lk], T.d_chi[lk]);
    xs = -T.d_damp[lk] * S.qvel[lk] - bias + act;
  }
  }
  xs = solve_LT(xs, dv, -d_nanc_s, g_S.M);
  xs = solve_L(xs, dv, isdof ? mrow : DMK_MAXANC, g_S.M);
  xs *= dv;
  if constexpr (!DAMP2) {
    if (isdof) S.qacc_smooth[lk] = xs;
  }
  SYNC();
  PROF(4);
  return xs;
}

__device__ __noinline__ float euler_damped_solve(GDev &T, const int lane, const float rhs) {
  return fwd_smooth<true>(T, lane, rhs);
}

__device__ __forceinline__ int fwd_collide(GDev &T, const int lane) {
  EnvLds &S = g_S;
  int ncon = 0, overflow = 0;
  const int lb = lane < DMK_NB ? lane : 0;
  const int lk = lane < DMK_NV ? lane : 0;
  const int lg = lane < DMK_NG ? lane : 0;
  const int bdep = (lane < DMK_NB) ? T.b_depth[lb] : -1;
  const float bmass = (lane < DMK_NB) ? T.b_mass[lb] : 0.f;
  const float mtot_inv = T.total_mass_inv;
  (void)lg; (void)bdep; (void)bmass; (void)mtot_inv; (void)lb; (void)lk;
    int base = 0;
    overflow = 0;
    for (int round = 0; round < 2; round++) {
      const int p = round * 64 + lane;
      Cand c;
      c.valid = 0;
      c.t[0] = c.t[1] = c.t[2] = 0;
#pragma unroll
      for (int s = 0; s < 4; s++) {
        c.d[s] = 0;
#pragma unroll
        for (int i = 0; i < 3; i++) { c.p[s][i] = 0; c.n[s][i] = 0; }
      }
      int g1 = 0, g2 = 0;
      bool isbb = false;
      float margin = 0;
      bool act = false;
      int t1 = 0, t2 = 0;
      float x1[3], x2[3], z1[3], z2[3];
      if (p < T.npair) {
        GPair &pr = T.pairs[p];
        g1 = pr.g1; g2 = pr.g2; t1 = pr.t1; t2 = pr.t2;
        margin = pr.margin;
        for (int i = 0; i < 3; i++) { x1[i] = S.gpos[g1][i]; x2[i] = S.gpos[g2][i]; z1[i] = pr.z1[i]; z2[i] = pr.z2[i]; }
        const float df[3] = {x2[0] - x1[0], x2[1] - x1[1], x2[2] - x1[2]};
        if (t1 == DM_GEOM_PLANE) {
          const float pn[3] = {S.gmat[g1][2], S.gmat[g1][5], S.gmat[g1][8]};
          act = dot3(df, pn) - pr.rbsum <= margin;
        } else {
          act = !(dot3(df, df) > (pr.rbsum + margin) * (pr.rbsum + margin));
        }
      }
      if (!__any(act)) continue;
      if (act) {
        float M1[9], M2[9];
        for (int i = 0; i < 9; i++) { M1[i] = S.gmat[g1][i]; M2[i] = S.gmat[g2][i]; }
        if (act) {
          if (t1 == DM_GEOM_PLANE) {
            float pn[3] = {M1[2], M1[5], M1[8]};
            if (t2 == DM_GEOM_SPHERE) {
              np_plane_sphere<0>(c, margin, x1, pn, x2, z2[0]);
            } else if (t2 == DM_GEOM_CAPSULE) {
              float ax[3] = {M2[2], M2[5], M2[8]}, e[3];
              for (int i = 0; i < 3; i++) e[i] = x2[i] + ax[i] * z2[1];
              np_plane_sphere<0>(c, margin, x1, pn, e, z2[0]);
              for (int i = 0; i < 3; i++) e[i] = x2[i] - ax[i] * z2[1];
              np_plane_sphere<1>(c, margin, x1, pn, e, z2[0]);
              c.t[0] = ax[0]; c.t[1] = ax[1]; c.t[2] = ax[2];
            } else {
              const float df[3] = {x2[0] - x1[0], x2[1] - x1[1], x2[2] - x1[2]};
              const float dist = dot3(df, pn);
              float A[3][3], a[3];
#pragma unroll
              for (int j = 0; j < 3; j++) {
                A[j][0] = M2[j] * z2[j]; A[j][1] = M2[3 + j] * z2[j]; A[j][2] = M2[6 + j] * z2[j];
                a[j] = pn[0] * A[j][0] + pn[1] * A[j][1] + pn[2] * A[j][2];
              }
              unsigned okm = 0;
#pragma unroll
              for (int i = 0; i < 8; i++) {
                const float ld = ((i & 1) ? a[0] : -a[0]) + ((i & 2) ? a[1] : -a[1]) + ((i & 4) ? a[2] : -a[2]);
                okm |= (!(dist + ld > margin || ld > 0)) ? (1u << i) : 0u;
              }
#pragma unroll
              for (int s = 0; s < 4; s++) {
                if (okm) {
                  const int i = __ffs(okm) - 1;
                  okm &= okm - 1;
                  const float s0 = (i & 1) ? 1.f : -1.f, s1 = (i & 2) ? 1.f : -1.f, s2 = (i & 4) ? 1.f : -1.f;
                  const float corner[3] = {s0 * A[0][0] + s1 * A[1][0] + s2 * A[2][0], s0 * A[0][1] + s1 * A[1][1] + s2 * A[2][1],
                                           s0 * A[0][2] + s1 * A[1][2] + s2 * A[2][2]};
                  const float cdist = dist + dot3(pn, corner);
                  c.d[s] = cdist;
                  for (int q = 0; q < 3; q++) { c.p[s][q] = corner[q] + x2[q] - pn[q] * 0.5f * cdist; c.n[s][q] = pn[q]; }
                  c.valid |= 1 << s;
                }
              }
            }
          } else if (t2 != DM_GEOM_BOX) {
            float r1 = z1[0], r2 = z2[0];
            if (t1 == DM_GEOM_SPHERE && t2 == DM_GEOM_SPHERE) {
              np_sphere_sphere<0>(c, margin, x1, r1, x2, r2);
            } else if (t1 == DM_GEOM_SPHERE) {
              float ax[3] = {M2[2], M2[5], M2[8]}, v[3] = {x1[0] - x2[0], x1[1] - x2[1], x1[2] - x2[2]}, pt[3];
              float x = clampf(dot3(ax, v), -z2[1], z2[1]);
              for (int i = 0; i < 3; i++) pt[i] = x2[i] + ax[i] * x;
              np_sphere_sphere<0>(c, margin, x1, r1, pt, r2);
            } else {
              float a1[3] = {M1[2], M1[5], M1[8]}, a2[3] = {M2[2], M2[5], M2[8]};
              float df[3] = {x1[0] - x2[0], x1[1] - x2[1], x1[2] - x2[2]};
              float ma = dot3(a1, a1), mb = -dot3(a1, a2), mc = dot3(a2, a2);
              float u = -dot3(a1, df), v = dot3(a2, df);
              float det = ma * mc - mb * mb;
              float v1[3], v2[3];
              if (fabsf(det) >= MINVALF) {
                float xx1 = (mc * u - mb * v) / det, xx2 = (ma * v - mb * u) / det;
                if (xx1 > z1[1]) { xx1 = z1[1]; xx2 = (v - mb * z1[1]) / mc; }
                else if (xx1 < -z1[1]) { xx1 = -z1[1]; xx2 = (v + mb * z1[1]) / mc; }
                if (xx2 > z2[1]) { xx2 = z2[1]; xx1 = clampf((u - mb * z2[1]) / ma, -z1[1], z1[1]); }
                else if (xx2 < -z2[1]) { xx2 = -z2[1]; xx1 = clampf((u + mb * z2[1]) / ma, -z1[1], z1[1]); }
                for (int i = 0; i < 3; i++) { v1[i] = x1[i] + a1[i] * xx1; v2[i] = x2[i] + a2[i] * xx2; }
                np_sphere_sphere<0>(c, margin, v1, r1, v2, r2);
              } else {
                Cand e;
                e.valid = 0;
                for (int i = 0; i < 3; i++) v1[i] = x1[i] + a1[i] * z1[1];
                float d2[3] = {v1[0] - x2[0], v1[1] - x2[1], v1[2] - x2[2]};
                float xx2 = clampf(dot3(d2, a2), -z2[1], z2[1]);
                for (int i = 0; i < 3; i++) v2[i] = x2[i] + a2[i] * xx2;
                np_sphere_sphere<0>(e, margin, v1, r1, v2, r2);
                for (int i = 0; i < 3; i++) v1[i] = x1[i] - a1[i] * z1[1];
                for (int i = 0; i < 3; i++) d2[i] = v1[i] - x2[i];
                xx2 = clampf(dot3(d2, a2), -z2[1], z2[1]);
                for (int i = 0; i < 3; i++) v2[i] = x2[i] + a2[i] * xx2;
                np_sphere_sphere<1>(e, margin, v1, r1, v2, r2);
                for (int i = 0; i < 3; i++) v2[i] = x2[i] + a2[i] * z2[1];
                float d1[3] = {v2[0] - x1[0], v2[1] - x1[1], v2[2] - x1[2]};
                float xx1 = clampf(dot3(d1, a1), -z1[1], z1[1]);
                for (int i = 0; i < 3; i++) v1[i] = x1[i] + a1[i] * xx1;
                np_sphere_sphere<2>(e, margin, v1, r1, v2, r2);
                for (int i = 0; i < 3; i++) v2[i] = x2[i] - a2[i] * z2[1];
                for (int i = 0; i < 3; i++) d1[i] = v2[i] - x1[i];
                xx1 = clampf(dot3(d1, a1), -z1[1], z1[1]);
                for (int i = 0; i < 3; i++) v1[i] = x1[i] + a1[i] * xx1;
                np_sphere_sphere<3>(e, margin, v1, r1, v2, r2);
                int cnt = 0;
#pragma unroll
                for (int s = 0; s < 4; s++) {
                  bool ok = ((e.valid >> s) & 1) && cnt < 2;
#pragma unroll
                  for (int o = 0; o < 2; o++)
                    if (ok && cnt == o) {
                      c.d[o] = e.d[s];
                      for (int q = 0; q < 3; q++) { c.p[o][q] = e.p[s][q]; c.n[o][q] = e.n[s][q]; }
                      c.valid |= 1 << o;
                    }
                  cnt += ok ? 1 : 0;
                }
              }
            }
          } else if (t1 == DM_GEOM_SPHERE) {
            np_sphere_box<0>(c, margin, x1, z1[0], x2, M2, z2);
          } else if (t1 == DM_GEOM_CAPSULE) {
            float axw[3] = {M1[2], M1[5], M1[8]}, tt[3] = {x1[0] - x2[0], x1[1] - x2[1], x1[2] - x2[2]}, pp[3], aa[3];
            float hl = z1[1], r = z1[0];
            mat_t_vec(pp, M2, tt);
            mat_t_vec(aa, M2, axw);
            float lo = -hl, hi = hl, ts;
            if (cb_grad(pp, aa, z2, lo) >= 0) ts = lo;
            else if (cb_grad(pp, aa, z2, hi) <= 0) ts = hi;
            else {
              for (int q = 0; q < 26; q++) {
                float mid = 0.5f * (lo + hi);
                if (cb_grad(pp, aa, z2, mid) < 0) lo = mid; else hi = mid;
              }
              ts = 0.5f * (lo + hi);
            }
            float pt[3];
            for (int i = 0; i < 3; i++) pt[i] = x1[i] + axw[i] * ts;
            np_sphere_box<0>(c, margin, pt, r, x2, M2, z2);
            float te = (ts > 0) ? -hl : hl;
            if (fabsf(te - ts) > 1e-3f * hl) {
              for (int i = 0; i < 3; i++) pt[i] = x1[i] + axw[i] * te;
              np_sphere_box<1>(c, margin, pt, r, x2, M2, z2);
            }
          } else {
            isbb = true;
          }
        }
        if (isbb) {
          np_box_box(S, &T.pairs[p]);
          int nc = S.u.bb.ncand;
#pragma unroll
          for (int s = 0; s < 4; s++)
            if (s < nc) {
              c.valid |= 1 << s;
              c.d[s] = S.u.bb.cand[s][0];
              for (int q = 0; q < 3; q++) { c.p[s][q] = S.u.bb.cand[s][1 + q]; c.n[s][q] = S.u.bb.cand[s][4 + q]; }
            }
        }
      }
      int cnt = __popc(c.valid);
      unsigned long long lt = lanemask_lt(lane);
      unsigned long long b0 = __ballot(cnt & 1), b1 = __ballot(cnt & 2), b2 = __ballot(cnt & 4);
      int off = __popcll(b0 & lt) + 2 * __popcll(b1 & lt) + 4 * __popcll(b2 & lt);
      int total = __popcll(b0) + 2 * __popcll(b1) + 4 * __popcll(b2);
      if (total == 0) continue;
      int w = base + off;
#pragma unroll
      for (int s = 0; s < 4; s++) {
        if ((c.valid >> s) & 1) {
          if (w < DMK_MAXCON) {
            float fr[9] = {c.n[s][0], c.n[s][1], c.n[s][2], c.t[0], c.t[1], c.t[2], 0, 0, 0};
            make_frame(fr);
            S.c_dist[w] = c.d[s];
            for (int q = 0; q < 3; q++) S.c_pos[w][q] = c.p[s][q];
            for (int q = 0; q < 9; q++) S.c_frame[w][q] = fr[q];
            S.c_g1[w] = g1; S.c_g2[w] = g2;
          }
          w++;
        }
      }
      base += total;
    }
    if (base > DMK_MAXCON) { overflow |= 1; base = DMK_MAXCON; }
    ncon = base;
    SYNC();

    PROF(5);
  return ncon | (overflow << 8);
}

template <bool MF>
__device__ __forceinline__ void build_row(GDev &T, EnvLds &S, const int r, const int nefc, const float (&com)[3],
                                          float (&J)[DMK_NV], float &R, float &Dd, float &aref, float &bb, float &jw) {
      float rpos = 0, rmargin = 0, rdiag = 1, mu = 0;
      int rtype = -1, full = 0;
      float wl[3] = {0, 0, 0}, wa[3] = {0, 0, 0};
      unsigned long long cm1 = 0, cm2 = 0;
      int ldof = -1;
      float lsign = 0;
      if (r < nefc) {
        int info = S.rowinfo[r];
        if (info < 0) {
          int v = -info - 1;
          ldof = v >> 1;
          lsign = (v & 1) ? -1.f : 1.f;
          rtype = 0;
          float q = S.qpos[ldof + 1];
          rpos = (v & 1) ? (T.d_hi[ldof] - q) : (q - T.d_lo[ldof]);
          rmargin = 0;
          rdiag = T.d_invw[ldof];
        } else {
          int ci = (info >> 3) & 0x3F, e = info & 7;
          full = (info & 0x4000) ? 1 : 0;
          int g1 = S.c_g1[ci], g2 = S.c_g2[ci];
          int b1 = T.g_body[g1], b2 = T.g_body[g2];
          int cd1 = T.g_condim[g1], cd2 = T.g_condim[g2];
          int dim = cd1 > cd2 ? cd1 : cd2;
          mu = fmaxf(T.g_mu[g1], T.g_mu[g2]);
          float fr[9];
          for (int i = 0; i < 9; i++) fr[i] = S.c_frame[ci][i];
          float tran = T.b_invw[b1] + T.b_invw[b2];
          if (dim < 3) {
            rtype = 1;
            wl[0] = fr[0]; wl[1] = fr[1]; wl[2] = fr[2];
            rdiag = tran;
          } else {
            rtype = 2;
            const bool second = (e >> 1) != 0;
            const float tx = second ? fr[6] : fr[3], ty = second ? fr[7] : fr[4], tz = second ? fr[8] : fr[5];
            float sg = (e & 1) ? -mu : mu;
            wl[0] = fr[0] + sg * tx; wl[1] = fr[1] + sg * ty; wl[2] = fr[2] + sg * tz;
            rdiag = tran + mu * mu * tran;
          }
          float off[3] = {S.c_pos[ci][0] - com[0], S.c_pos[ci][1] - com[1], S.c_pos[ci][2] - com[2]};
          cross3(wa, off, wl);
          cm1 = T.b_chain[b1]; cm2 = T.b_chain[b2];
          rpos = S.c_dist[ci];
          rmargin = fmaxf(T.g_margin[g1], T.g_margin[g2]);
        }
      }
      float vel = 0, jqs = 0;
      jw = 0;
      float vals[32];
      if (MF) {
        const float wv[6] = {wa[0], wa[1], wa[2], wl[0], wl[1], wl[2]};
        const int lane_ = (int)(threadIdx.x & 63);
        const float *cdp = &S.cdof[lane_ & 31][lane_ >> 5];
        mfma_f16v acc;
#pragma unroll
        for (int v = 0; v < 16; v++) acc[v] = 0.f;
#pragma unroll
        for (int p = 0; p < 3; p++) {
          const auto sw = __builtin_amdgcn_permlane32_swap(__float_as_uint(wv[2 * p]), __float_as_uint(wv[2 * p + 1]), false, false);
          acc = __builtin_amdgcn_mfma_f32_32x32x2f32(cdp[2 * p], __uint_as_float(sw[0]), acc, 0, 0, 0);
        }
#pragma unroll
        for (int v = 0; v < 16; v++) {
          const auto sw = __builtin_amdgcn_permlane32_swap(__float_as_uint(acc[v]), __float_as_uint(acc[v]), false, false);
          vals[(v / 4) * 8 + (v % 4)] = acc[v];
          vals[(v / 4) * 8 + (v % 4) + 4] = __uint_as_float(sw[1]);
        }
      }
#pragma unroll
      for (int k = 0; k < DMK_NV; k++) {
        float val;
        if (MF && k < 32) {
          val = vals[k];
        } else {
          const float4 ca = *reinterpret_cast<const float4 *>(&S.cdof[k][0]);
          const float2 cb = *reinterpret_cast<const float2 *>(&S.cdof[k][4]);
          val = ca.x * wa[0] + ca.y * wa[1] + ca.z * wa[2] + ca.w * wl[0] + cb.x * wl[1] + cb.y * wl[2];
        }
        float sg = (float)((int)((cm2 >> k) & 1ull) - (int)((cm1 >> k) & 1ull));
        float j = (k == ldof) ? lsign : sg * val;
        J[k] = j;
        vel += j * S.qvel[k];
        jqs += j * S.qacc_smooth[k];
        jw += j * S.warm[k];
      }
      R = 1; Dd = 0; aref = 0; bb = 0;
      if (r < nefc) {
        float sol[5] = {T.solimp[0], T.solimp[1], T.solimp[2], T.solimp[3], T.solimp[4]};
        float imp = impedance(sol, rpos, rmargin);
        R = fmaxf(MINVALF, (1 - imp) * rdiag / imp);
        if (rtype == 2 && full) R = 2 * mu * mu * R;
        aref = -T.B * vel - T.K * imp * (rpos - rmargin);
        bb = jqs - aref;
        Dd = 1.0f / R;
      }
      {
        lds_cfloat_p Mp = (lds_cfloat_p)S.M;
#pragma unroll
        for (int i = DMK_NV - 1; i >= 1; i--) {
          const float xi = J[i] * S.dinv[i];
          asm volatile("" : "+v"(Mp), "+v"(J[0]));
#pragma unroll
          for (int j = 0; j < i; j++)
            if (topo::is_anc(j, i)) J[j] -= Mp[topo::midx(i, j)] * xi;
        }
      }
#pragma unroll
      for (int k = 0; k < DMK_NV; k++) J[k] *= S.dsqrtinv[k];
}

__device__ __noinline__ float fwd_constraint_wide(GDev &T, const int lane, const int nefc, const float xs, const float dv,
                                                  float *ar) {
  EnvLds &S = g_S;
  const int lk = lane < DMK_NV ? lane : 0;
  const float com[3] = {S.com[0], S.com[1], S.com[2]};
  float Ja[DMK_NV], Jb[DMK_NV];
  float Ra, Da, arefa, bba, jwa, Rb, Db, arefb, bbb, jwb;
  build_row<false>(T, S, lane, nefc, com, Ja, Ra, Da, arefa, bba, jwa);
  build_row<false>(T, S, lane + 64, nefc, com, Jb, Rb, Db, arefb, bbb, jwb);
  float ARda = Ra, ARdb = Rb;
#pragma unroll
  for (int k = 0; k < DMK_NV; k++) { ARda += Ja[k] * Ja[k]; ARdb += Jb[k] * Jb[k]; }
  const bool va = lane < nefc, vb = lane + 64 < nefc;
#pragma unroll 1
  for (int i = 0; i < nefc; i++) {
    const int src = i & 63;
    float acca = 0, accb = 0;
    if (i < 64) {
#pragma unroll
      for (int k = 0; k < DMK_NV; k++) { const float bi = rl(Ja[k], src); acca = fmaf(Ja[k], bi, acca); accb = fmaf(Jb[k], bi, accb); }
      if (lane == src) acca += Ra;
    } else {
#pragma unroll
      for (int k = 0; k < DMK_NV; k++) { const float bi = rl(Jb[k], src); acca = fmaf(Ja[k], bi, acca); accb = fmaf(Jb[k], bi, accb); }
      if (lane == src) accb += Rb;
    }
    ar[i * 128 + lane] = acca;
    ar[i * 128 + 64 + lane] = accb;
  }
  const float ARinva = va ? 1.0f / ARda : 0.f, ARinvb = vb ? 1.0f / ARdb : 0.f;
  float fa = 0, fb = 0, ra = bba, rb = bbb;
  {
    const float jara = jwa - arefa, jarb = jwb - arefb;
    const float fwa = (va && jara < 0) ? -Da * jara : 0.f, fwb = (vb && jarb < 0) ? -Db * jarb : 0.f;
    float rwa = bba, rwb = bbb;
#pragma unroll 1
    for (int i = 0; i < nefc; i++) {
      const float fi = (i < 64) ? rl(fwa, i & 63) : rl(fwb, i & 63);
      rwa = fmaf(ar[i * 128 + lane], fi, rwa);
      rwb = fmaf(ar[i * 128 + 64 + lane], fi, rwb);
    }
    const float cost = wave_sum(fwa * (0.5f * (rwa - bba) + bba) + fwb * (0.5f * (rwb - bbb) + bbb));
    if (!(cost > 0)) { fa = fwa; fb = fwb; ra = rwa; rb = rwb; }
  }
  const float scale = T.pgs_scale, tol = T.tolerance;
  const int max_iter = T.iterations;
  int iter = 0;
  while (iter < max_iter) {
    float na = ar[lane], nb = ar[64 + lane];
    const float nfa = -fa, nfb = -fb;
    float rsa = ra, rsb = rb;
#pragma unroll 1
    for (int i = 0; i < 64; i++) {
      const float ca = na, cb = nb;
      na = ar[(i + 1) * 128 + lane]; nb = ar[(i + 1) * 128 + 64 + lane];
      const float dli = rl(fmaxf(nfa, -ra * ARinva), i);
      rsa = (lane == i) ? ra : rsa;
      ra = fmaf(ca, dli, ra);
      rb = fmaf(cb, dli, rb);
    }
#pragma unroll 1
    for (int i = 64; i < nefc; i++) {
      const float ca = na, cb = nb;
      if (i + 1 < nefc) { na = ar[(i + 1) * 128 + lane]; nb = ar[(i + 1) * 128 + 64 + lane]; }
      const float dli = rl(fmaxf(nfb, -rb * ARinvb), i - 64);
      rsb = (lane == i - 64) ? rb : rsb;
      ra = fmaf(ca, dli, ra);
      rb = fmaf(cb, dli, rb);
    }
    const float dla = fmaxf(nfa, -rsa * ARinva), dlb = fmaxf(nfb, -rsb * ARinvb);
    const float impv = -wave_sum(dla * fmaf(0.5f * dla, ARda, rsa) + dlb * fmaf(0.5f * dlb, ARdb, rsb));
    fa += dla;
    fb += dlb;
    iter++;
    if (impv * scale < tol) break;
  }
  if (lane == 0) S.info[3] = iter;
  float v = 0;
#pragma unroll
  for (int k = 0; k < DMK_NV; k++) {
    const float sm = wave_sum(fa * Ja[k] + fb * Jb[k]);
    if (lane == k) v = sm;
  }
  const int mrow = T.d_madr[lk] + T.d_nanc[lk];
  const uint64_t ancm = T.d_ancm[lk];
  v *= S.dsqrtinv[lk] * S.M[T.d_madr[lk]];
  v = solve_L(v, dv, (lane < DMK_NV) ? mrow : DMK_MAXANC, g_S.M);
  return xs + v * dv;
}

__device__ __forceinline__ float fwd_constraint(GDev &T, const int lane, const int ncon, int overflow, float *dbg_force,
                                                float *ar_scratch) {
  EnvLds &S = g_S;
  int nefc = 0, nlimit = 0, solver_iter = 0;
  const int lb = lane < DMK_NB ? lane : 0;
  const int lk = lane < DMK_NV ? lane : 0;
  const int lg = lane < DMK_NG ? lane : 0;
  const int bdep = (lane < DMK_NB) ? T.b_depth[lb] : -1;
  const float bmass = (lane < DMK_NB) ? T.b_mass[lb] : 0.f;
  const float mtot_inv = T.total_mass_inv;
  (void)lg; (void)bdep; (void)bmass; (void)mtot_inv; (void)lb; (void)lk;
  const float xs = (lane < DMK_NV) ? S.qacc_smooth[lk] : 0.f;
  const float dv = (lane < DMK_NV) ? S.dinv[lk] : 0.f;
  const float com[3] = {S.com[0], S.com[1], S.com[2]};
  float qacc_out;
    {
      bool lim = false;
      float ldist = 0;
      int lneg = 0;
      if (lane >= 6 && lane < DMK_NV && dlimited) {
        float q = S.qpos[lane + 1];
        if (q < dlo) { lim = true; ldist = q - dlo; lneg = 0; }
        else if (q > dhi) { lim = true; ldist = dhi - q; lneg = 1; }
      }
      int myrow = prefix_count(lim, lane, &nlimit);
      if (lim) { S.rowinfo[myrow] = (int16_t)(-(((lane << 1) | lneg) + 1)); }
      int dim3 = 0, have = lane < ncon;
      if (have) {
        int cd1 = T.g_condim[S.c_g1[lane]], cd2 = T.g_condim[S.c_g2[lane]];
        dim3 = (cd1 > cd2 ? cd1 : cd2) >= 3;
      }
      unsigned long long lt = lanemask_lt(lane);
      unsigned long long m1 = __ballot(have && !dim3), m4 = __ballot(have && dim3);
      int roff = nlimit + __popcll(m1 & lt) + 4 * __popcll(m4 & lt);
      int rtot = nlimit + __popcll(m1) + 4 * __popcll(m4);
      if (have) {
        int nr = dim3 ? 4 : 1;
        for (int e = 0; e < nr; e++)
          if (roff + e < DMK_MAXROW) S.rowinfo[roff + e] = (int16_t)((lane << 3) | e | (((roff + nr) <= DMK_MAXROW) ? 0x4000 : 0));
      }
      if (rtot > DMK_MAXROW) { overflow |= 2; rtot = DMK_MAXROW; }
      nefc = rtot;
    }
    SYNC();

    qacc_out = xs;
    solver_iter = 0;
    if (nefc > DMK_LANEROW) {
      qacc_out = fwd_constraint_wide(T, lane, nefc, xs, dv, ar_scratch);
      solver_iter = S.info[3];
    } else if (nefc > 0) {
      float J[DMK_NV];
      float R, Dd, aref, bb, jw;
      if (nefc <= DMK_REGROW) build_row<true>(T, S, lane, nefc, com, J, R, Dd, aref, bb, jw);
      else build_row<false>(T, S, lane, nefc, com, J, R, Dd, aref, bb, jw);
      PROF(6);
      float AR[DMK_REGROW];
      float *arx = ar_scratch + lane;
      float ARd = R;
#pragma unroll
      for (int k = 0; k < DMK_NV; k++) ARd += J[k] * J[k];
      if (nefc <= DMK_REGROW && nefc >= DMK_MFMA_MIN_ROWS) {
        mfma_f16v acc;
#pragma unroll
        for (int v = 0; v < 16; v++) acc[v] = 0.f;
        StaticFor<0, DMK_NV / 2>::run([&](auto kc) {
          constexpr int k0 = decltype(kc)::value * 2;
          const auto sw = __builtin_amdgcn_permlane32_swap(__float_as_uint(J[k0]), __float_as_uint(J[k0 + 1]), false, false);
          const float x = __uint_as_float(sw[0]);
          acc = __builtin_amdgcn_mfma_f32_32x32x2f32(x, x, acc, 0, 0, 0);
          return true;
        });
        StaticFor<0, 16>::run([&](auto vc) {
          constexpr int v = decltype(vc)::value;
          const auto sw = __builtin_amdgcn_permlane32_swap(__float_as_uint(acc[v]), __float_as_uint(acc[v]), false, false);
          constexpr int i0 = (v / 4) * 8 + (v % 4);
          AR[i0] = lane_sel<(1ull << i0)>(acc[v] + R, acc[v]);
          const float up = __uint_as_float(sw[1]);
          AR[i0 + 4] = lane_sel<(1ull << (i0 + 4))>(up + R, up);
          return true;
        });
      } else
      StaticFor<0, DMK_REGROW>::run([&](auto ic) {
        constexpr int i = decltype(ic)::value;
        if (i >= nefc) {
          if ((i & 3) == 0) return false;
          AR[i] = 0.f;
          return true;
        }
        float acc0 = 0, acc1 = 0;
#pragma unroll
        for (int k = 0; k < DMK_NV; k += 2) {
          acc0 = fmaf(J[k], rl(J[k], i), acc0);
          acc1 = fmaf(J[k + 1], rl(J[k + 1], i), acc1);
        }
        float acc = acc0 + acc1;
        if (lane == i) acc += R;
        AR[i] = acc;
        return true;
      });
#pragma unroll 1
      for (int i = DMK_REGROW; i < nefc; i++) {
        float acc0 = 0, acc1 = 0;
#pragma unroll
        for (int k = 0; k < DMK_NV; k += 2) {
          acc0 = fmaf(J[k], rl(J[k], i), acc0);
          acc1 = fmaf(J[k + 1], rl(J[k + 1], i), acc1);
        }
        float acc = acc0 + acc1;
        if (lane == i) acc += R;
        arx[(i - DMK_REGROW) * 64] = acc;
      }
      const float ARinv = (lane < nefc) ? 1.0f / ARd : 0.f;
      PROF(7);
      float f = 0, r = bb;
      {
        float jar = jw - aref;
        float fw = (lane < nefc && jar < 0) ? -Dd * jar : 0.f;
        float rw = bb;
        StaticFor<0, DMK_REGROW>::run([&](auto ic) {
          constexpr int i = decltype(ic)::value;
          if (i >= nefc) return false;
          rw += AR[i] * rl(fw, i);
          return true;
        });
#pragma unroll 1
        for (int i = DMK_REGROW; i < nefc; i++) rw += arx[(i - DMK_REGROW) * 64] * rl(fw, i);
        float cost = wave_sum(fw * (0.5f * (rw - bb) + bb));
        if (!(cost > 0)) { f = fw; r = rw; }
      }
      const float scale = T.pgs_scale, tol = T.tolerance;
      const int max_iter = T.iterations;
      const float nAinv = -ARinv;
      float g = r * nAinv;
      StaticFor<0, DMK_REGROW / 4>::run([&](auto bc) {
        constexpr int b = decltype(bc)::value * 4;
        if (b >= nefc) return false;
        AR[b] *= nAinv; AR[b + 1] *= nAinv; AR[b + 2] *= nAinv; AR[b + 3] *= nAinv;
        return true;
      });
      int iter = 0;
      while (iter < max_iter) {
        int lane_s = lane;
        asm volatile("" : "+v"(lane_s));
        const float nf = -f;
        float gs = g;
        StaticFor<0, DMK_REGROW / 4>::run([&](auto bc) {
          constexpr int b = decltype(bc)::value * 4;
          if (b >= nefc) return false;
          auto step = [&](auto ic) {
            constexpr int i = decltype(ic)::value;
            const float dli = rl(fmaxf(nf, g), i);
            gs = (lane_s == i) ? g : gs;
            g = fmaf(AR[i], dli, g);
          };
          step(std::integral_constant<int, b>{});
          step(std::integral_constant<int, b + 1>{});
          step(std::integral_constant<int, b + 2>{});
          step(std::integral_constant<int, b + 3>{});
          return true;
        });
        if (nefc > DMK_REGROW) {
          float anext = arx[0];
#pragma unroll 1
          for (int i = DMK_REGROW; i < nefc; i++) {
            const float acur = anext * nAinv;
            if (i + 1 < nefc) anext = arx[(i + 1 - DMK_REGROW) * 64];
            const float dli = rl(fmaxf(nf, g), i);
            gs = (lane_s == i) ? g : gs;
            g = fmaf(acur, dli, g);
          }
        }
        const float dl = fmaxf(nf, gs);
        const float impv = -wave_sum(dl * ARd * (0.5f * dl - gs));
        f += dl;
        iter++;
        if (impv * scale < tol) break;
      }
      solver_iter = iter;
      PROF(8);
      float v = 0;
      {
        const bool actv = (lane < nefc) && (f != 0.f);
        int nact;
        const int slot = prefix_count(actv, lane, &nact);
        if (nact <= 20) {
          if (actv) {
#pragma unroll
            for (int k = 0; k < DMK_NV; k++) S.u.fin.tr[slot][k] = f * J[k];
          }
          SYNC();
          if (lane < DMK_NV)
            for (int a = 0; a < nact; a++) v += S.u.fin.tr[a][lk];
          SYNC();
        } else {
#pragma unroll
          for (int k = 0; k < DMK_NV; k++) {
            float s = wave_sum(f * J[k]);
            if (lane == k) v = s;
          }
        }
      }
      const int mrow = T.d_madr[lk] + T.d_nanc[lk];
      const uint64_t ancm = T.d_ancm[lk];
      v *= S.dsqrtinv[lk] * S.M[T.d_madr[lk]];
      v = solve_L(v, dv, (lane < DMK_NV) ? mrow : DMK_MAXANC, g_S.M);
      qacc_out = xs + v * dv;
#ifndef DM_PROFILE
      if (dbg_force && lane < DMK_LANEROW) dbg_force[lane] = (lane < nefc) ? f : 0.f;
#endif
    }
    SYNC();
    if (lane < DMK_NV) { S.qacc[lk] = qacc_out; S.warm[lk] = qacc_out; }
    SYNC();
    PROF(9);
  if (lane == 0) { S.info[0] = ncon; S.info[1] = nefc; S.info[2] = nlimit; S.info[3] = solver_iter; S.info[4] = overflow; }
  return qacc_out;
}

template <int TASK>
__device__ __forceinline__ void step_body(const DmLaunch &P) {
  constexpr int NOBS_T = TASK ? DM_NOBS_COMBINED : DM_NOBS;
  constexpr int NOBS_B = NOBS_T - 64;
  constexpr int NTERMS = TASK ? 8 : 5;
  GDev &T = *(GDev *)P.T;
  const int lane = threadIdx.x & 63;
  EnvLds &S = g_S;
  const int slot = blockIdx.x;
  if (slot >= P.nslots) return;
  const int env = P.env_ids ? P.env_ids[slot] : slot;
  if (env < 0 || env >= P.N) return;
  const int mode = P.mode;
  if (mode == DMK_MODE_RESET && P.mask && !P.mask[env]) return;
  float *st = P.state + (size_t)env * DMK_STATE_STRIDE;
  int *sti = reinterpret_cast<int *>(st);

  const int lb = lane < DMK_NB ? lane : 0;
  const int lk = lane < DMK_NV ? lane : 0;
  const int lg = lane < DMK_NG ? lane : 0;
  const float h = T.timestep;
  const float mtot_inv = T.total_mass_inv;

  PROF_DECL;
  if (lane == 0) {
    S.xpos[0][0] = S.xpos[0][1] = S.xpos[0][2] = 0;
    S.xquat[0][0] = 1; S.xquat[0][1] = S.xquat[0][2] = S.xquat[0][3] = 0;
    for (int i = 0; i < 9; i++) S.xmat[0][i] = (i % 4 == 0) ? 1.f : 0.f;
    S.xipos[0][0] = S.xipos[0][1] = S.xipos[0][2] = 0;
    for (int i = 0; i < 6; i++) S.cvel[0][i] = 0;
    for (int i = 0; i < 10; i++) S.cinert[0][i] = 0;
  }

  const int clip_id = sti[DMS_CLIP];
  int motion = TASK ? ((clip_id >= 0 && clip_id < 4) ? clip_id : 0) : 0;
  DmClipDev clip = P.clips[TASK ? (motion == 3 ? 2 : motion) : ((clip_id >= 0 && clip_id < 8) ? clip_id : 0)];
  if (clip.L < 1 || clip.rows == nullptr) return;
  if (TASK && (P.clips[0].L < 1 || P.clips[1].L < 1 || P.clips[2].L < 2)) return;
  int idx_curr = sti[DMS_IDX], ep_len = sti[DMS_EPLEN], rcnt = sti[DMS_RCNT];
  if (TASK) idx_curr = idx_curr < 0 ? 0 : idx_curr;
  else idx_curr = idx_curr < 0 ? 0 : (idx_curr >= clip.L ? clip.L - 1 : idx_curr);
  float ep_rew = st[DMS_EPREW];
  unsigned f8r = P.f8 ? (unsigned)sti[DMS_F8R] : 0u, f8l = P.f8 ? (unsigned)sti[DMS_F8L] : 0u;
  if (lane < DMK_NQ) S.qpos[lane] = st[DMS_QPOS + lane];
  if (lane < DMK_NV) { S.qvel[lane] = st[DMS_QVEL + lane]; S.warm[lane] = st[DMS_WARM + lane]; }
  if (lane < DMK_NU) S.ctrl[lane] = st[DMS_CTRL + lane];
  SYNC();
  if (mode == DMK_MODE_STEP || mode == DMK_MODE_PHYSICS) {
    if (lane < DMK_NU) S.ctrl[lane] = P.actions[(size_t)env * DMK_NU + lane];
  } else if (mode == DMK_MODE_FORCED || mode == DMK_MODE_SETSTATE) {
    if (P.in_qpos) {
      if (lane < DMK_NQ) S.qpos[lane] = P.in_qpos[(size_t)slot * DMK_NQ + lane];
      if (lane < DMK_NV) S.qvel[lane] = P.in_qvel[(size_t)slot * DMK_NV + lane];
    }
    if (mode == DMK_MODE_SETSTATE) {
      if (P.in_warm && lane < DMK_NV) S.warm[lane] = P.in_warm[(size_t)slot * DMK_NV + lane];
      if (P.in_ctrl && lane < DMK_NU) S.ctrl[lane] = P.in_ctrl[(size_t)slot * DMK_NU + lane];
    }
  } else if (mode == DMK_MODE_RESET) {
    int fi;
    if (TASK) {
      if (P.idx_init) { idx_curr = P.idx_init[env] < 0 ? 0 : P.idx_init[env]; }
      else {
        motion = (dm_hash32(P.seed, env, rcnt, 0x5EED) & 1) ? 2 : 0;
        clip = P.clips[motion];
        idx_curr = (int)(dm_hash32(P.seed, env, rcnt, 0x5EEE) % (uint32_t)clip.L) + (motion == 0 ? P.amnesty_steps + 10 : 0);
      }
      fi = (motion == 3) ? 1 : idx_curr % clip.L;
    } else {
      fi = P.idx_init ? P.idx_init[env] : (int)(dm_hash32(P.seed, env, rcnt, 0x5EED) % (uint32_t)clip.L);
      fi = fi < 0 ? 0 : (fi >= clip.L ? clip.L - 1 : fi);
      idx_curr = fi;
    }
    const float *rr = clip.reset + (size_t)fi * DMK_RESET_ROW;
    if (lane < DMK_NQ) S.qpos[lane] = rr[lane];
    if (lane < DMK_NV) S.qvel[lane] = rr[35 + lane];
    ep_len = 0; ep_rew = 0; rcnt++;
  }
  SYNC();

  int it = (mode == DMK_MODE_STEP || mode == DMK_MODE_PHYSICS) ? 0 : 4;
  bool after_reset = false, done = false, sim_err = false;
  int reason = DM_REASON_NONE;
  float reward = 0;
  int ncon = 0, nefc = 0, nlimit = 0, solver_iter = 0, overflow = 0;
  float com[3] = {0, 0, 0};
  unsigned stage_ncon = 0, stage_nefc = 0;
  int work = 0;

  if (mode == DMK_MODE_SETSTATE && !P.run_forward) {
    if (lane < DMK_NQ) st[DMS_QPOS + lane] = S.qpos[lane];
    if (lane < DMK_NV) { st[DMS_QVEL + lane] = S.qvel[lane]; st[DMS_WARM + lane] = S.warm[lane]; }
    if (lane < DMK_NU) st[DMS_CTRL + lane] = S.ctrl[lane];
    return;
  }
  if (mode == DMK_MODE_STEP || mode == DMK_MODE_FORCED || mode == DMK_MODE_PHYSICS) {
    float a = (lane < DMK_NQ) ? S.qpos[lane] : 0.f, b = (lane < DMK_NV) ? S.qvel[lk] : 0.f;
    sim_err = __any(!(fabsf(a) <= MAXVALF) || !(fabsf(b) <= MAXVALF));
  }

  PROF(0);
  for (;;) {
   float qacc_out = 0;
   if (!sim_err) {
    GDev *Tp = (GDev *)P.T;
    asm volatile("" : "+s"(Tp));
    GDev &Ts = *Tp;
#ifndef DM_NO_LANE_LAUNDER
    int lane_st = lane;
    asm volatile("" : "+v"(lane_st));
#else
    const int lane_st = lane;
#endif
    fwd_smooth(Ts, lane_st);
    if (it == 0) {
      if (lane < DMK_NV) {
        const float v0 = S.qvel[lk];
        S.rk[0][lk] = (lane < 3) ? S.qpos[lane] : ((lane >= 6) ? S.qpos[lane + 1] : 0.f);
        S.rk[1][lk] = v0; S.rk[2][lk] = 0.f; S.rk[3][lk] = 0.f; S.rk[4][lk] = v0;
      }
      if (lane < 4) S.rkq[lane] = S.qpos[3 + lane];
    }
    {
      const int cr = fwd_collide(Ts, lane_st);
      ncon = cr & 0xFF;
      qacc_out = fwd_constraint(Ts, lane_st, ncon, cr >> 8, P.debug ? P.debug + (size_t)env * DM_DEBUG_STRIDE + 352 : nullptr,
                                P.ar_scratch + (size_t)env * DMK_MAXROW * DMK_MAXROW);
      nefc = S.info[1]; nlimit = S.info[2]; solver_iter = S.info[3]; overflow = S.info[4];
      if (it < 4) { stage_ncon |= (unsigned)(ncon & 0xFF) << (8 * it); stage_nefc |= (unsigned)(nefc & 0xFF) << (8 * it); }
      work = (work >> 1) + 64 + (nefc > 0 ? 48 + 16 * nefc : 0) + nefc * solver_iter;
      if (P.f8) {
        bool rfs = false, lfs = false;
        if (lane < ncon) {
          const int g1 = S.c_g1[lane], g2 = S.c_g2[lane];
          const bool fl = (g1 == Ts.floor_geom || g2 == Ts.floor_geom);
          rfs = fl && (g1 == Ts.rfoot_geom || g2 == Ts.rfoot_geom);
          lfs = fl && (g1 == Ts.lfoot_geom || g2 == Ts.lfoot_geom);
        }
        const unsigned keep = ncon >= 32 ? 0u : (~0u << ncon);
        f8r = (f8r & keep) | (unsigned)__ballot(rfs);
        f8l = (f8l & keep) | (unsigned)__ballot(lfs);
      }
    }
    if (it == 0 || (it == 4 && mode == DMK_MODE_FORCED && !after_reset)) {
      bool badv = (lane < DMK_NV) && !(fabsf(qacc_out) <= MAXVALF);
      sim_err = __any(badv);
    }
   }

    const bool euler = (P.integrator == DM_INT_EULER) && (mode == DMK_MODE_STEP || mode == DMK_MODE_PHYSICS);
    float x0q = 0, x0v = 0, accq = 0, accv = 0, curv = 0;
    float q0[4] = {1, 0, 0, 0};
    if (!sim_err && it < 4) {
      const bool dl = lane < DMK_NV;
      x0q = dl ? S.rk[0][lk] : 0.f; x0v = dl ? S.rk[1][lk] : 0.f; accq = dl ? S.rk[2][lk] : 0.f;
      accv = dl ? S.rk[3][lk] : 0.f; curv = dl ? S.rk[4][lk] : 0.f;
      for (int i = 0; i < 4; i++) q0[i] = S.rkq[i];
    }
    if (!sim_err && it < 3 && !euler) {
      const float Bw = (it == 0) ? (1.f / 6.f) : (1.f / 3.f);
      const float Aw = (it == 2) ? 1.f : 0.5f;
      accq += Bw * curv;
      accv += Bw * qacc_out;
      float dq = Aw * curv, dv = Aw * qacc_out;
      curv = x0v + h * dv;
      float w3[3] = {rl(dq, 3), rl(dq, 4), rl(dq, 5)};
      float wn = sqrtf(dot3(w3, w3));
      float qr[4] = {1, 0, 0, 0}, qn[4];
      if (wn >= MINVALF) {
        float s, c;
        sincosf(0.5f * h * wn, &s, &c);
        float inv = s / wn;
        qr[0] = c; qr[1] = w3[0] * inv; qr[2] = w3[1] * inv; qr[3] = w3[2] * inv;
      }
      quat_mul(qn, q0, qr);
      quat_normalize(qn);
      if (lane < DMK_NV) { S.qvel[lk] = curv; S.rk[2][lk] = accq; S.rk[3][lk] = accv; S.rk[4][lk] = curv; }
      if (lane < 3) S.qpos[lane] = x0q + h * dq;
      if (lane >= 6 && lane < DMK_NV) S.qpos[lane + 1] = x0q + h * dq;
      if (lane < 4) S.qpos[3 + lane] = (lane == 0) ? qn[0] : (lane == 1) ? qn[1] : (lane == 2) ? qn[2] : qn[3];
      SYNC();
      PROF_STAGE(it);
      it++;
      continue;
    }
    if (!sim_err && (it == 3 || (it == 0 && euler))) {
      if (euler) {
        const float hb = (lane < DMK_NV) ? h * T.d_damp[lk] : 0.f;
        float a2 = qacc_out;
        if (__any(hb != 0.f)) a2 = qacc_out - euler_damped_solve(T, lane, hb * qacc_out);
        accv = a2;
        accq = x0v + h * a2;
        it = 3;
      } else {
        accq += (1.f / 6.f) * curv;
        accv += (1.f / 6.f) * qacc_out;
      }
      float w3[3] = {rl(accq, 3), rl(accq, 4), rl(accq, 5)};
      float wn = sqrtf(dot3(w3, w3));
      float qr[4] = {1, 0, 0, 0}, qn[4];
      if (wn >= MINVALF) {
        float s, c;
        sincosf(0.5f * h * wn, &s, &c);
        float inv = s / wn;
        qr[0] = c; qr[1] = w3[0] * inv; qr[2] = w3[1] * inv; qr[3] = w3[2] * inv;
      }
      quat_mul(qn, q0, qr);
      quat_normalize(qn);
      if (lane < DMK_NV) S.qvel[lk] = x0v + h * accv;
      if (lane < 3) S.qpos[lane] = x0q + h * accq;
      if (lane >= 6 && lane < DMK_NV) S.qpos[lane + 1] = x0q + h * accq;
      if (lane < 4) S.qpos[3 + lane] = (lane == 0) ? qn[0] : (lane == 1) ? qn[1] : (lane == 2) ? qn[2] : qn[3];
      SYNC();
    }

    PROF(10);
    PROF_STAGE(it);
    if (mode == DMK_MODE_PHYSICS) {
      if (sim_err) {
        f8r = f8l = 0;
        SYNC();
        if (lane < DMK_NQ) S.qpos[lane] = T.qpos0[lane];
        if (lane < DMK_NV) { S.qvel[lane] = 0; S.warm[lane] = 0; }
        if (lane < DMK_NU) S.ctrl[lane] = 0;
        SYNC();
      }
      break;
    }
    const bool task_pass = !after_reset && (mode == DMK_MODE_STEP || mode == DMK_MODE_FORCED);
    float obs_a = 0, obs_b = 0;
    float terms[5] = {0, 0, 0, 0, 0};
    float extra[3] = {0, 0, 0};
    if (sim_err) {
      reward = 0; done = true; reason = DM_REASON_SIM_ERROR;
      f8r = f8l = 0;
      SYNC();
      if (lane < DMK_NQ) S.qpos[lane] = T.qpos0[lane];
      if (lane < DMK_NV) { S.qvel[lane] = 0; S.warm[lane] = 0; }
      if (lane < DMK_NU) S.ctrl[lane] = 0;
      SYNC();
    } else {
      const float Sc = P.vel_obs_scale;
      if (lane < 28) obs_a = S.qpos[7 + lane];
      else if (lane < 56) obs_a = S.qvel[6 + lane - 28] * Sc;
      const int tb = T.torso_body;
      float rpy[3], tq[4] = {S.xquat[tb][0], S.xquat[tb][1], S.xquat[tb][2], S.xquat[tb][3]};
      quat_to_rpy(tq, rpy);
      float cv[6];
      for (int i = 0; i < 6; i++) cv[i] = S.cvel[tb][i];
      float sy, cy;
      sincosf(-rpy[2], &sy, &cy);
      const float tor[8] = {rpy[0] * Sc, rpy[1] * Sc, (cy * cv[3] - sy * cv[4]) * Sc, (sy * cv[3] + cy * cv[4]) * Sc,
                            cv[5] * Sc, cv[0] * Sc, cv[1] * Sc, cv[2] * Sc};
#pragma unroll
      for (int i = 0; i < 8; i++)
        if (lane == 56 + i) obs_a = tor[i];
      bool rf = false, lf = false;
      if (lane < ncon) {
        int g1 = S.c_g1[lane], g2 = S.c_g2[lane];
        bool fl = (g1 == T.floor_geom || g2 == T.floor_geom);
        rf = fl && (g1 == T.rfoot_geom || g2 == T.rfoot_geom);
        lf = fl && (g1 == T.lfoot_geom || g2 == T.lfoot_geom);
      }
      const float rff = (P.f8 ? f8r != 0 : __any(rf)) ? 1.f : 0.f, lff = (P.f8 ? f8l != 0 : __any(lf)) ? 1.f : 0.f;
      const int Lm = (TASK && motion == 3) ? P.to_getup_len : clip.L;
      const int frame = TASK ? ((motion == 3) ? 1 : idx_curr % clip.L) : idx_curr;
      if (TASK) {
        const float ph = clampf((float)(idx_curr % Lm) / (float)Lm, 0.f, 1.f);
        if (lane == 0) obs_b = ph;
        if (lane == 1) obs_b = cy;
        if (lane == 2) obs_b = sy;
        if (lane == 3) obs_b = 1.f;
        if (lane == 6) obs_b = (motion == 3) ? 1.f : 0.f;
        if (lane == 7) obs_b = (motion == 2) ? 1.f : 0.f;
      } else {
        const float ph = clampf((float)idx_curr / (float)clip.L, 0.f, 1.f);
        if (lane == 0) obs_b = rff;
        if (lane == 1) obs_b = lff;
        if (lane == 2) obs_b = ph;
      }

      if (task_pass) {
        const float *row = clip.rows + (size_t)frame * DMK_CLIP_ROW;
        const float ra = row[lane];
        const float adiff = (lane < 28) ? fabsf(S.qpos[7 + (lane < 28 ? lane : 0)] - ra) : 0.f;
        float ecfg = wave_sum(adiff);
        const float dsum = ecfg;
        const float evel = wave_sum((lane >= 28 && lane < 56) ? fabsf(ra - S.qvel[6 + ((lane >= 28 && lane < 56) ? lane - 28 : 0)]) : 0.f);
        const float tquat[4] = {rl(ra, 56), rl(ra, 57), rl(ra, 58), rl(ra, 59)};
        const float cq[4] = {S.qpos[3], S.qpos[4], S.qpos[5], S.qpos[6]};
        float rc[3], rt[3];
        quat_to_rpy(cq, rc);
        quat_to_rpy(tquat, rt);
        ecfg += fabsf(rc[1] - rt[1]);
        const float r_cfg = expf(-ecfg);
        const float r_vel = expf(-0.1f * evel);
        float df = 0;
        if (lane < 12) {
          int e = lane / 3, cc = lane % 3;
          df = S.gpos[T.ee_geom[e]][cc] - row[60 + lane];
        }
        const float r_ee = expf(-40.f * wave_sum(df * df));
        float ce = 0;
        const float bmass_t = (lane < DMK_NB) ? T.b_mass[lb] : 0.f;
        for (int i = 0; i < 3; i++) {
          float d2 = row[72 + i] - wave_sum(bmass_t * S.xpos[lb][i]) * mtot_inv;
          ce += d2 * d2;
        }
        const float r_com = expf(-10.f * ce);
        float viol = 0;
        if (lane >= 6 && lane < DMK_NV) {
          float q = S.qpos[lane + 1];
          viol = ((q <= dlo * 0.99f) ? 1.f : 0.f) + ((q >= dhi * 0.99f) ? 1.f : 0.f);
        }
        const float qlim = wave_sum(viol) / 28.0f;
        terms[0] = r_cfg; terms[1] = r_vel; terms[2] = r_ee; terms[3] = r_com; terms[4] = qlim;
        reward = P.w_pose * r_cfg + P.w_vel * r_vel + P.w_ee * r_ee + P.w_com * r_com + P.w_jl * qlim;
        const float zc = S.com[2];
        done = false;
        reason = DM_REASON_NONE;
        if (TASK) {
          const float ALIM = 0.2617993877991494f, MAX_ANGLE = 1.0471975511965976f;
          const float droll = fabsf(rc[0] - rt[0]), dpitch = fabsf(rc[1] - rt[1]);
          float imitation = reward, task_r = 0.f;
          if (motion == 0 || motion == 1) {
            const float ex = row[78] - S.qvel[0], ey = row[79] - S.qvel[1];
            task_r = expf(-sqrtf(ex * ex + ey * ey) * 10.f);
          }
          if (motion == 3) { imitation = 0.f; task_r = expf(-(dsum + dpitch + droll) / 5.f) / 3.f; }
          reward = imitation * 0.7f + task_r * 0.3f;
          const unsigned long long badm = __ballot(adiff > ALIM);
          const bool all_close = !__any(!(adiff < ALIM));
          extra[0] = imitation; extra[1] = task_r;
          extra[2] = (float)(__popcll(badm) + (dpitch > ALIM ? 1 : 0) + (droll > ALIM ? 1 : 0));
          if (idx_curr >= Lm - 1) {
            if (motion == 2) { motion = 1; idx_curr = 0; }
            if (motion == 3) { motion = 2; idx_curr = 0; }
          }
          if (dpitch < ALIM && droll < ALIM && all_close && motion == 3) { motion = 2; idx_curr = 0; }
          if (motion == 0 || motion == 1) {
            const bool fallen = (zc < P.low_z) || (zc > P.high_z) || (droll > MAX_ANGLE) || (dpitch > MAX_ANGLE);
            if (fallen) {
              if (!(idx_curr > P.amnesty_steps)) { done = true; reason = DM_REASON_FALLEN_NO_AMNESTY; }
              motion = 3; idx_curr = 0;
            }
          }
          if (P.max_ep_length != 0 && ep_len >= P.max_ep_length) { done = true; reason = DM_REASON_MAX_EP_LEN; }
          clip = P.clips[motion == 3 ? 2 : motion];
          idx_curr += 1;
        } else {
          if (!(clip.flags & DM_CLIP_FLOOR)) {
            done = (zc < P.low_z) || (zc > P.high_z);
            reason = (zc < P.low_z) ? DM_REASON_LOW_Z : DM_REASON_HIGH_Z;
          }
          if (P.max_ep_length != 0 && ep_len >= P.max_ep_length) { done = true; reason = DM_REASON_MAX_EP_LEN; }
          if ((clip.flags & DM_CLIP_ACYCLIC) && idx_curr + 1 == clip.L) { done = true; reason = DM_REASON_ACYCLIC_END; }
          idx_curr = (idx_curr + 1) % clip.L;
        }
        ep_rew += reward;
        ep_len += 1;
        bool ob = !(fabsf(obs_a) <= P.obs_bound) || !(fabsf(obs_b) <= P.obs_bound);
        if (__any(ob)) {
          obs_a = 0; obs_b = 0; reward = 0; done = true; reason = DM_REASON_OBS_BOUNDS;
          for (int i = 0; i < 5; i++) terms[i] = 0;
          extra[0] = extra[1] = extra[2] = 0;
        }
      }
    }
    if (P.debug && !after_reset) {
      float *dbg = P.debug + (size_t)env * DM_DEBUG_STRIDE;
      if (lane < 42) dbg[lane] = (&S.xpos[0][0])[lane];
      if (lane < 48) dbg[42 + lane] = (&S.gpos[0][0])[lane];
      for (int i = lane; i < 84; i += 64) dbg[90 + i] = (&S.cvel[0][0])[i];
      if (lane < DMK_NV) { dbg[174 + lane] = S.qacc[lane]; dbg[208 + lane] = S.qacc_smooth[lane]; }
      if (lane == 0) { dbg[242] = ncon; dbg[243] = nefc; dbg[244] = solver_iter; dbg[245] = nlimit; dbg[246] = overflow;
                       dbg[247] = __int_as_float((int)stage_ncon); dbg[248] = __int_as_float((int)stage_nefc); }
      if (lane < DMK_MAXCON) {
        dbg[256 + 3 * lane] = (lane < ncon) ? (float)S.c_g1[lane] : -1.f;
        dbg[257 + 3 * lane] = (lane < ncon) ? (float)S.c_g2[lane] : -1.f;
        dbg[258 + 3 * lane] = (lane < ncon) ? S.c_dist[lane] : 0.f;
      }
    }
    if (task_pass) {
      if (P.rew && lane == 0) P.rew[env] = reward;
      if (P.done && lane == 0) P.done[env] = done ? 1 : 0;
      if (P.reason && lane == 0) P.reason[env] = reason;
      if (P.terms && lane < NTERMS)
        P.terms[(size_t)env * NTERMS + lane] = (lane == 0) ? terms[0] : (lane == 1) ? terms[1] : (lane == 2) ? terms[2] : (lane == 3) ? terms[3]
                                             : (lane == 4) ? terms[4] : (lane == 5) ? extra[0] : (lane == 6) ? extra[1] : extra[2];
      if (done && P.auto_reset && mode == DMK_MODE_STEP) {
        if (P.terminal_obs) {
          P.terminal_obs[(size_t)env * NOBS_T + lane] = obs_a;
          if (lane < NOBS_B) P.terminal_obs[(size_t)env * NOBS_T + 64 + lane] = obs_b;
        }
        int fi;
        if (TASK) {
          motion = (dm_hash32(P.seed, env, rcnt, 0x5EED) & 1) ? 2 : 0;
          clip = P.clips[motion];
          fi = (int)(dm_hash32(P.seed, env, rcnt, 0x5EEE) % (uint32_t)clip.L);
          idx_curr = fi + (motion == 0 ? P.amnesty_steps + 10 : 0);
          fi = idx_curr % clip.L;
        } else {
          fi = (int)(dm_hash32(P.seed, env, rcnt, 0x5EED) % (uint32_t)clip.L);
          idx_curr = fi;
        }
        rcnt++;
        const float *rr = clip.reset + (size_t)fi * DMK_RESET_ROW;
        SYNC();
        if (lane < DMK_NQ) S.qpos[lane] = rr[lane];
        if (lane < DMK_NV) S.qvel[lane] = rr[35 + lane];
        ep_len = 0; ep_rew = 0;
        SYNC();
        after_reset = true;
        sim_err = false;
        it = 4;
        continue;
      }
    }
    if (P.obs) {
      P.obs[(size_t)env * NOBS_T + lane] = obs_a;
      if (lane < NOBS_B) P.obs[(size_t)env * NOBS_T + 64 + lane] = obs_b;
    }
    break;
  }

  PROF(11);
#ifdef DM_PROFILE
  if (P.debug && lane < 16) { unsigned v = 0;
#pragma unroll
    for (int i = 0; i < 16; i++) if (lane == i) v = g_S.prof[i];
    P.debug[(size_t)env * DM_DEBUG_STRIDE + 352 + lane] = (float)v;
    if (lane < 4) P.debug[(size_t)env * DM_DEBUG_STRIDE + 368 + lane] = (float)g_S.prof_stage[lane]; }
#endif
  if (lane < DMK_NQ) st[DMS_QPOS + lane] = S.qpos[lane];
  if (lane < DMK_NV) { st[DMS_QVEL + lane] = S.qvel[lane]; st[DMS_WARM + lane] = S.warm[lane]; }
  if (lane < DMK_NU) st[DMS_CTRL + lane] = S.ctrl[lane];
  if (lane == 0) { sti[DMS_IDX] = idx_curr; sti[DMS_EPLEN] = ep_len; st[DMS_EPREW] = ep_rew; sti[DMS_RCNT] = rcnt; }
  if (TASK && lane == 0) sti[DMS_CLIP] = motion;
  if (P.f8 && lane == 0) { sti[DMS_F8R] = (int)f8r; sti[DMS_F8L] = (int)f8l; }
  if (P.cost && lane == 0) P.cost[env] = work;
}

extern "C" __global__ void __launch_bounds__(64 * DMK_ENVS_PER_BLOCK, DMK_WAVES_PER_SIMD) dm_step_kernel(DmLaunch P) {
  step_body<0>(P);
}
extern "C" __global__ void __launch_bounds__(64 * DMK_ENVS_PER_BLOCK, DMK_WAVES_PER_SIMD) dm_step_combined_kernel(DmLaunch P) {
  step_body<1>(P);
}
extern "C" __global__ void __launch_bounds__(64 * DMK_ENVS_PER_BLOCK, 3) dm_step_kernel_w3(DmLaunch P) {
  step_body<0>(P);
}
extern "C" __global__ void __launch_bounds__(64 * DMK_ENVS_PER_BLOCK, 3) dm_step_combined_kernel_w3(DmLaunch P) {
  step_body<1>(P);
}
#ifdef DM_EXPERIMENT_W4
extern "C" __global__ void __launch_bounds__(64 * DMK_ENVS_PER_BLOCK, 4) dm_step_kernel_w4(DmLaunch P) {
  step_body<0>(P);
}
#endif

extern "C" __global__ void dm_fill_actions_kernel(float *actions, int n, uint64_t seed, uint32_t step) {
  int i = blockIdx.x * blockDim.x + threadIdx.x;
  if (i >= n * DMK_NU) return;
  int env = i / DMK_NU, j = i % DMK_NU;
  actions[i] = -2.0f + 4.0f * (float)(dm_hash32(seed, env, step, j) >> 8) * (1.0f / 16777216.0f);
}
```

include/deepmimic_hip.h:

```cpp
#ifndef DEEPMIMIC_HIP_H
#define DEEPMIMIC_HIP_H

#include <stdint.h>

#include "dm_model.h"

#ifdef __cplusplus
extern "C" {
#endif

typedef struct DmEngine *DmHandle;

#define DM_OK 0
#define DM_EINVAL (-22)
#define DM_ENOMEM (-12)
#define DM_EHIP (-5)
#define DM_ENODEV (-19)

#define DM_MAX_CLIPS 8

#define DM_REASON_NONE 0
#define DM_REASON_LOW_Z 1
#define DM_REASON_HIGH_Z 2
#define DM_REASON_MAX_EP_LEN 3
#define DM_REASON_ACYCLIC_END 4
#define DM_REASON_SIM_ERROR 5
#define DM_REASON_OBS_BOUNDS 6
#define DM_REASON_FALLEN_NO_AMNESTY 7

#define DM_CFG_INT_MODEL 0
#define DM_CFG_INT_EULER 1
#define DM_CFG_INT_RK4 2

#define DM_TASK_DPENV 0
#define DM_TASK_COMBINED 1

typedef struct DmConfig {
  int32_t num_envs;
  int32_t max_ep_length;
  float vel_obs_scale;
  float low_z, high_z;
  float w_pose, w_vel, w_end_eff, w_com, w_joint_limit;
  float obs_bound;
  uint64_t seed;
  int32_t auto_reset;
  int32_t device;
  int32_t lpt_schedule;
  int32_t task;
  int32_t amnesty_steps;
  int32_t to_getup_len;
  int32_t integrator;
  int32_t stale_contact_slots;
} DmConfig;

void dm_default_config(DmConfig *cfg);

int dm_create(const DmModel *model, const DmConfig *cfg, DmHandle *out);
int dm_destroy(DmHandle h);
const char *dm_last_error(DmHandle h);
int dm_num_envs(DmHandle h);
int dm_obs_dim(DmHandle h);
int dm_terms_dim(DmHandle h);

int dm_load_clip(DmHandle h, int clip_id, int L, const double *host_qpos, const double *host_qvel,
                 const double *host_body_xpos, const double *host_geom_xpos);
#define DM_CLIP_FLOOR 1
#define DM_CLIP_ACYCLIC 2
int dm_set_clip_flags(DmHandle h, int clip_id, int flags);
int dm_set_env_clips(DmHandle h, const int32_t *clip_ids, void *stream);
int dm_get_env_clips(DmHandle h, int32_t *clip_ids, void *stream);

int dm_reset(DmHandle h, const uint8_t *mask, const int32_t *idx_init, float *obs_out, void *stream);

int dm_step(DmHandle h, const float *actions, float *obs, float *rew, uint8_t *done, float *terms,
            int32_t *reason, float *terminal_obs, void *stream);

int dm_physics_step(DmHandle h, const float *actions, void *stream);

int dm_step_forced(DmHandle h, const float *qpos, const float *qvel, float *obs, float *rew,
                   uint8_t *done, float *terms, int32_t *reason, void *stream);

int dm_set_state(DmHandle h, const int32_t *env_ids, int n, const float *qpos, const float *qvel,
                 const float *qacc_warmstart, const float *ctrl, int run_forward, void *stream);
int dm_forward(DmHandle h, const int32_t *env_ids, int n, void *stream);
int dm_get_state(DmHandle h, const int32_t *env_ids, int n, float *qpos, float *qvel,
                 float *qacc_warmstart, float *ctrl, void *stream);
int dm_get_counters(DmHandle h, int32_t *idx_curr, int32_t *episode_length, float *episode_reward,
                    void *stream);
int dm_set_counters(DmHandle h, const int32_t *idx_curr, const int32_t *episode_length, void *stream);

int dm_set_seed(DmHandle h, uint64_t seed);

#define DM_DEBUG_STRIDE 416
int dm_set_debug(DmHandle h, float *debug_buf);

int dm_get_work(DmHandle h, int32_t *work_out, void *stream);

int dm_fill_random_actions(DmHandle h, float *actions, uint32_t step_index, void *stream);

int dm_last_step_ms(DmHandle h, float *ms);
int dm_mean_step_ms(DmHandle h, float *ms, int32_t *count);
int dm_enable_timing(DmHandle h, int enable);

int dm_ppo_loss(const float *mean, const float *log_std, const float *value, const float *act, const float *old_logp,
                const float *adv, const float *ret, int B, int A, float clip_range, float vf_coef, float ent_coef,
                int normalize_advantage, float *grad_mean, float *grad_log_std, float *grad_value, float *out8,
                float *scratch, void *stream);

int dm_linear_wgrad(const float *dY, const float *X, float *dW, float *db, int B, int O, int I, void *stream);

int dm_ppo_gather(const long long *idx, int B, const float *obs, int D, const float *act, int A, const float *adv,
                  const float *ret, const float *logp, float *o_obs, float *o_act, float *o_adv, float *o_ret, float *o_logp,
                  void *stream);
int dm_ppo_gather_bf16(const long long *idx, int B, const unsigned short *obs, int D, const unsigned short *act, int A,
                       const float *adv, const float *ret, const float *logp, float *o_obs, float *o_act, float *o_adv, float *o_ret,
                       float *o_logp, void *stream);

#define DM_ADAM_PARTIALS 1024
int dm_flat_adam_step(float *p, const float *g, float *m, float *v, int n, float lr, float beta1, float beta2, float eps,
                      float max_norm, float grad_scale, float *state2, int state2_floats, void *stream);
int dm_flat_adam_update(float *p, const float *g, float *m, float *v, int n, float lr, float beta1, float beta2, float eps,
                        float max_norm, float grad_scale, float *state2, int state2_floats, void *stream);

typedef struct DmGatherSpec {
  const long long *idx; int B, D, A, reserved;
  const float *obs, *act, *adv, *ret, *logp;
  float *o_obs, *o_act, *o_adv, *o_ret, *o_logp;
} DmGatherSpec;
int dm_flat_adam_step_gather(float *p, const float *g, float *m, float *v, int n, float lr, float beta1, float beta2, float eps,
                             float max_norm, float grad_scale, float *state2, int state2_floats, int begin, const DmGatherSpec *next,
                             void *stream);
typedef struct DmGatherSpecBf16 {
  const long long *idx; int B, D, A, reserved;
  const unsigned short *obs, *act;
  const float *adv, *ret, *logp;
  float *o_obs, *o_act, *o_adv, *o_ret, *o_logp;
} DmGatherSpecBf16;
int dm_flat_adam_step_gather_bf16(float *p, const float *g, float *m, float *v, int n, float lr, float beta1, float beta2, float eps,
                                  float max_norm, float grad_scale, float *state2, int state2_floats, int begin,
                                  const DmGatherSpecBf16 *next, void *stream);

int dm_colsum(const float *Y, int B, int O, float *out, void *stream);

int dm_linear_tanh(const float *X, const float *W, const float *bias, float *Y, int B, int O, int I, void *stream);
int dm_tanh_linear_wgrad(const float *dY, const float *Y, const float *X, float *dW, float *db, int B, int O, int I, void *stream);
int dm_tanh_bwd_colsum(const float *dY, const float *Y, float *dZ, float *db, int B, int O, void *stream);

int dm_policy_sample(const float *mean, const float *log_std, int N, int A, unsigned long long seed, const unsigned *counter,
                     const float *lo, const float *hi, float *act, float *act_env, float *logp, void *stream);
int dm_rollout_store(int N, int D, int A, const float *last_obs, const float *act, const float *val, const float *logp,
                     const float *rew, const unsigned char *done, const float *new_obs, float *b_obs, float *b_act, float *b_val,
                     float *b_logp, float *b_rew, float *b_done, float *last_obs_out, unsigned *counter, void *stream);
int dm_rollout_store_bf16(int N, int D, int A, const float *last_obs, const float *act, const float *val, const float *logp,
                          const float *rew, const unsigned char *done, const float *new_obs, unsigned short *b_obs,
                          unsigned short *b_act, float *b_val, float *b_logp, float *b_rew, float *b_done, float *last_obs_out,
                          unsigned *counter, void *stream);

long long dm_rollout_finish_workspace_bytes(int T, int N);
int dm_rollout_finish(int T, int N, const float *rew, const void *done, int done_is_u8, const float *val, const float *last_val,
                      double gamma, double gae_lambda, float *adv, float *ret, float *ep_acc, float *ep_hist, unsigned *ep_count,
                      double *stats, void *work, long long work_bytes, void *stream);

long long dm_policy_packed_floats(int D, int H1, int H2, int A);
int dm_policy_pack(const float *W1, const float *W2, const float *W3, int D, int H1, int H2, int A, float *packed, void *stream);
int dm_policy_forward(const float *obs, int N, int D, int H1, int H2, int A, const float *pi_packed, const float *pi_b1,
                      const float *pi_b2, const float *pi_b3, const float *vf_packed, const float *vf_b1, const float *vf_b2,
                      const float *vf_b3, const float *log_std, unsigned long long seed, const unsigned *counter,
                      unsigned draw_offset, int deterministic, const float *lo, const float *hi, float *mean_out, float *act,
                      float *act_env, float *logp, float *val, float *obs_copy, void *stream);
int dm_policy_forward_bf16(const float *obs, int N, int D, int H1, int H2, int A, const float *pi_packed, const float *pi_b1,
                           const float *pi_b2, const float *pi_b3, const float *vf_packed, const float *vf_b1, const float *vf_b2,
                           const float *vf_b3, const float *log_std, unsigned long long seed, const unsigned *counter,
                           unsigned draw_offset, int deterministic, const float *lo, const float *hi, float *mean_out,
                           unsigned short *act, float *act_env, float *logp, float *val, unsigned short *obs_copy, void *stream);

typedef struct DmPpoMlpStep {
  int32_t B, D, H1, H2, A, normalize_advantage;
  float clip_range, vf_coef, ent_coef;
  int32_t reserved;
  const float *obs, *act, *adv, *ret, *old_logp, *log_std;
  const float *W[2][3];
  const float *b[2][3];
  float *gW[2][3];
  float *gb[2][3];
  float *g_log_std;
  float *out8;
  float *workspace;
  long long workspace_floats;
  float *zero_ptr;
  long long zero_floats;
  float *adam_state2;
  float *loss_acc;
} DmPpoMlpStep;
long long dm_ppo_mlp_workspace_floats(int B, int D, int H1, int H2, int A);
int dm_ppo_mlp_grad(const DmPpoMlpStep *step, void *stream);

typedef struct DmPpoWideStep {
  int32_t B, D, H1, H2, A, normalize_advantage;
  float clip_range, vf_coef, ent_coef;
  int32_t reserved;
  const float *obs, *act, *adv, *ret, *old_logp, *log_std;
  const float *W[2][3], *b[2][3];
  float *gW[2][3], *gb[2][3];
  float *g_log_std;
  void *wpk[2];
  void *xbT;
  void *h1T[2], *dz1T[2];
  void *h2T[2], *dz2T[2];
  void *dz3T[2];
  float *part;
  float *stats8, *out8;
  float *zero_ptr;
  long long zero_floats;
  float *adam_state2, *loss_acc;
} DmPpoWideStep;
long long dm_ppo_wide_packed_elems(int D, int H1, int H2);
int dm_ppo_wide_dp(int D);
int dm_ppo_wide_supported(int B, int D, int H1, int H2, int A);
int dm_ppo_wide_grad(const DmPpoWideStep *step, void *stream);

int dm_sac_act(const float *head, int N, int A, int ld, unsigned long long seed, const unsigned *counter, int warmup,
               int deterministic, const float *lo, const float *hi, float *act, float *act_env, void *stream);
int dm_sac_store(int N, int D, int A, int cap_steps, const float *last_obs, const float *act, const float *rew,
                 const uint8_t *done, const float *obs, const float *terminal_obs, float *r_obs, float *r_act, float *r_rew,
                 float *r_done, float *r_next, float *last_obs_out, unsigned *ring, unsigned *counter, float *ep_acc,
                 float *ep_hist, void *stream);
int dm_sac_gather(int B, int N, int D, int A, unsigned long long seed, const unsigned *counter, const unsigned *ring,
                  const float *r_obs, const float *r_act, const float *r_rew, const float *r_done, const float *r_next,
                  float *obs2, float *xq, float *xpi, float *xt, float *rew, float *done, int *idx_out, void *stream);
int dm_sac_head_fwd(const float *head, int R, int Rpi, int A, unsigned long long seed, const unsigned *counter, float *a_pi,
                    float *a_next, int lda, float *logp, float *sac_state, int alpha_step, float target_entropy, float lr,
                    void *stream);
int dm_sac_critic_loss(const float *q, const float *qt, const float *logp_next, const float *rew, const float *done, int B,
                       float gamma, float *sac_state, float *dq, float *db3, void *stream);
int dm_sac_actor_loss(const float *q, const float *logp, int B, float *sac_state, float *dq, void *stream);
int dm_sac_head_bwd(const float *head, int B, int A, unsigned long long seed, const unsigned *counter, const float *dx, int K,
                    int col, const float *sac_state, float *dhead, float *dbias, void *stream);
int dm_sac_linear_relu(const float *X, int ldx, const float *W, const float *bias, float *Y, int B, int O, int I, int nets,
                       void *stream);
int dm_sac_relu_bwd_colsum(const float *dY, const float *Y, float *dZ, float *db, int B, int O, int nets, void *stream);
int dm_sac_polyak(const float *p, float *t, long long n, float tau, unsigned *counter, void *stream);

#ifdef __cplusplus
}
#endif
#endif
```

Measured before the change: 13.69 million.

## Replace separate LPT schedule kernel with in-kernel triple-buffered bucket scheduling

Removes the single-block dm_schedule_kernel launched before every step. Instead, each step block picks its env from a triple-buffered cost-bucket list, and at the end of the step it atomically files that env into the next generation's bucket based on its measured work. The last block rotates the generation and clears the stale counters. Per-env carried scalars move from registers into an LDS struct to cut register pressure, guarded by a static_assert that keeps occupancy. The cost is cross-block atomics, a scan at block start and a larger scheduling buffer.

```diff
diff --git a/deepmimic_mujoco_amd/_lib.py b/deepmimic_mujoco_amd/_lib.py
--- a/deepmimic_mujoco_amd/_lib.py
+++ b/deepmimic_mujoco_amd/_lib.py
@@ -26,7 +26,8 @@
            "dm_sac_act", "dm_sac_store", "dm_sac_gather", "dm_sac_head_fwd", "dm_sac_critic_loss", "dm_sac_actor_loss",
            "dm_sac_head_bwd", "dm_sac_linear_relu", "dm_sac_relu_bwd_colsum", "dm_sac_polyak",
            "dm_rollout_finish", "dm_rollout_finish_workspace_bytes",
-           "dm_policy_forward_bf16", "dm_rollout_store_bf16", "dm_ppo_gather_bf16", "dm_flat_adam_step_gather_bf16"]
+           "dm_policy_forward_bf16", "dm_rollout_store_bf16", "dm_ppo_gather_bf16", "dm_flat_adam_step_gather_bf16",
+           "dm_get_launch_order"]
 
 
 class DmConfig(C.Structure):
@@ -140,6 +141,7 @@
     L.dm_set_debug.argtypes = [vp, vp]
     L.dm_set_seed.argtypes = [vp, C.c_uint64]
     L.dm_get_work.argtypes = [vp, vp, vp]
+    L.dm_get_launch_order.argtypes = [vp, vp, vp, vp]
     L.dm_set_clip_flags.argtypes = [vp, i32, i32]
     L.dm_fill_random_actions.argtypes = [vp, vp, C.c_uint32, vp]
     L.dm_last_step_ms.argtypes = [vp, C.POINTER(C.c_float)]
@@ -311,6 +313,12 @@
         self._chk(self.L.dm_get_work(self.h, _ptr(w), self._stream()), "dm_get_work")
         return w
 
+    def get_launch_order(self):
+        order = self.torch.zeros(self.N, dtype=self.torch.int32, device=self.device)
+        bucket = self.torch.zeros(self.N, dtype=self.torch.int32, device=self.device)
+        self._chk(self.L.dm_get_launch_order(self.h, _ptr(order), _ptr(bucket), self._stream()), "dm_get_launch_order")
+        return order, bucket
+
     def enable_timing(self, on=True, stride=1):
         self._chk(self.L.dm_enable_timing(self.h, max(1, int(stride)) if on else 0), "dm_enable_timing")
 
diff --git a/deepmimic_mujoco_amd/csrc/dm_abi.hip b/deepmimic_mujoco_amd/csrc/dm_abi.hip
--- a/deepmimic_mujoco_amd/csrc/dm_abi.hip
+++ b/deepmimic_mujoco_amd/csrc/dm_abi.hip
@@ -28,7 +28,7 @@
   int clipL[DM_MAX_CLIPS] = {0};
   int clipFlags[DM_MAX_CLIPS] = {0};
   float *debug = nullptr;
-  int32_t *dOrder = nullptr;
+  int32_t *dSched = nullptr;
   int32_t *dCost = nullptr;
   static constexpr int NEV = 512;
   hipEvent_t ev0[NEV] = {}, ev1[NEV] = {};
@@ -217,13 +217,17 @@
   if (hipMalloc(&e->dArScratch, (size_t)e->N * DMK_MAXROW * DMK_MAXROW * sizeof(float)) != hipSuccess) {
     hipFree(e->dState); hipFree(e->dT); delete e; return DM_ENOMEM;
   }
-  if (hipMalloc(&e->dOrder, e->N * sizeof(int32_t)) != hipSuccess || hipMalloc(&e->dCost, e->N * sizeof(int32_t)) != hipSuccess) {
+  if (hipMalloc(&e->dSched, DMK_SCHED_WORDS(e->N) * sizeof(int32_t)) != hipSuccess || hipMalloc(&e->dCost, e->N * sizeof(int32_t)) != hipSuccess) {
+    if (e->dSched) hipFree(e->dSched);
     hipFree(e->dArScratch); hipFree(e->dState); hipFree(e->dT); delete e; return DM_ENOMEM;
   }
   hipMemset(e->dCost, 0, e->N * sizeof(int32_t));
-  { std::vector<int32_t> ident(e->N);
+  {
+    std::vector<int32_t> head(DMK_SCHED_LIST, 0), ident(e->N);
+    head[DMK_SCHED_CNT + DMK_SCHED_NB - 1] = e->N;
     for (int i = 0; i < e->N; i++) ident[i] = i;
-    hipMemcpy(e->dOrder, ident.data(), e->N * sizeof(int32_t), hipMemcpyHostToDevice); }
+    hipMemcpy(e->dSched, head.data(), head.size() * sizeof(int32_t), hipMemcpyHostToDevice);
+    hipMemcpy(e->dSched + DMK_SCHED_LIST + (size_t)(DMK_SCHED_NB - 1) * e->N, ident.data(), e->N * sizeof(int32_t), hipMemcpyHostToDevice); }
   for (int i = 0; i < DmEngine::NEV; i++) { hipEventCreate(&e->ev0[i]); hipEventCreate(&e->ev1[i]); }
   *out = e;
   return DM_OK;
@@ -236,7 +240,7 @@
   for (int i = 0; i < DM_MAX_CLIPS; i++) { if (e->dClipRows[i]) hipFree(e->dClipRows[i]); if (e->dClipReset[i]) hipFree(e->dClipReset[i]); }
   if (e->dState) hipFree(e->dState);
   if (e->dArScratch) hipFree(e->dArScratch);
-  if (e->dOrder) hipFree(e->dOrder);
+  if (e->dSched) hipFree(e->dSched);
   if (e->dCost) hipFree(e->dCost);
   if (e->dT) hipFree(e->dT);
   for (int i = 0; i < DmEngine::NEV; i++) { if (e->ev0[i]) hipEventDestroy(e->ev0[i]); if (e->ev1[i]) hipEventDestroy(e->ev1[i]); }
@@ -285,8 +289,6 @@
   return DM_OK;
 }
 
-__global__ void dm_schedule_kernel(const int32_t *cost, int32_t *order, int n);
-
 __global__ void dm_set_clip_kernel(float *state, const int32_t *ids, int n) {
   int i = blockIdx.x * blockDim.x + threadIdx.x;
   if (i < n) reinterpret_cast<int *>(state + (size_t)i * DMK_STATE_STRIDE)[DMS_CLIP] = ids ? ids[i] : 0;
@@ -401,11 +403,7 @@
   fill_launch(e, P, DMK_MODE_STEP);
   P.actions = actions; P.obs = obs; P.rew = rew; P.done = done; P.terms = terms; P.reason = reason; P.terminal_obs = terminal_obs;
   P.cost = e->dCost;
-  if (e->cfg.lpt_schedule) {
-    HIPCHK(e, hipSetDevice(e->cfg.device));
-    hipLaunchKernelGGL(dm_schedule_kernel, dim3(1), dim3(1024), 0, (hipStream_t)stream, e->dCost, e->dOrder, e->N);
-    P.env_ids = e->dOrder;
-  }
+  if (e->cfg.lpt_schedule) P.sched = e->dSched;
   return launch(e, P, e->N, stream);
 }
 
@@ -415,11 +413,7 @@
   fill_launch(e, P, DMK_MODE_PHYSICS);
   P.actions = actions;
   P.auto_reset = 0;
-  if (e->cfg.lpt_schedule) {
-    HIPCHK(e, hipSetDevice(e->cfg.device));
-    hipLaunchKernelGGL(dm_schedule_kernel, dim3(1), dim3(1024), 0, (hipStream_t)stream, e->dCost, e->dOrder, e->N);
-    P.env_ids = e->dOrder;
-  }
+  if (e->cfg.lpt_schedule) P.sched = e->dSched;
   return launch(e, P, e->N, stream);
 }
 
@@ -476,28 +470,26 @@
   return DM_OK;
 }
 
-__global__ void dm_schedule_kernel(const int32_t *cost, int32_t *order, int n) {
-  __shared__ int hist[256];
-  __shared__ int base[256];
-  const int tid = threadIdx.x;
-  if (tid < 256) hist[tid] = 0;
-  __syncthreads();
-  for (int i = tid; i < n; i += 1024) {
-    int b = cost[i] >> 5;
-    b = 255 - (b > 255 ? 255 : (b < 0 ? 0 : b));
-    atomicAdd(&hist[b], 1);
-  }
-  __syncthreads();
-  if (tid == 0) {
-    int acc = 0;
-    for (int b = 0; b < 256; b++) { base[b] = acc; acc += hist[b]; }
-  }
-  __syncthreads();
-  for (int i = tid; i < n; i += 1024) {
-    int b = cost[i] >> 5;
-    b = 255 - (b > 255 ? 255 : (b < 0 ? 0 : b));
-    order[atomicAdd(&base[b], 1)] = i;
-  }
+__global__ void dm_launch_order_kernel(const int32_t *sc, int n, int32_t *order_out, int32_t *bucket_out) {
+  const int slot = blockIdx.x * blockDim.x + threadIdx.x;
+  if (slot >= n) return;
+  const int gen = sc[0];
+  int env = -1, bucket = -1, base = 0;
+  for (int b = 0; b < DMK_SCHED_NB; b++) {
+    const int c = sc[DMK_SCHED_CNT + gen * DMK_SCHED_NB + b];
+    if (slot < base + c) { env = sc[DMK_SCHED_LIST + ((size_t)(gen * DMK_SCHED_NB + b)) * (size_t)n + (slot - base)]; bucket = b; break; }
+    base += c;
+  }
+  if (order_out) order_out[slot] = env;
+  if (bucket_out) bucket_out[slot] = bucket;
+}
+
+extern "C" int dm_get_launch_order(DmHandle e, int32_t *order_out, int32_t *bucket_out, void *stream) {
+  if (!e || (!order_out && !bucket_out)) return DM_EINVAL;
+  HIPCHK(e, hipSetDevice(e->cfg.device));
+  hipLaunchKernelGGL(dm_launch_order_kernel, dim3((e->N + 255) / 256), dim3(256), 0, (hipStream_t)stream, e->dSched, e->N, order_out, bucket_out);
+  HIPCHK(e, hipGetLastError());
+  return DM_OK;
 }
 
 extern "C" int dm_get_work(DmHandle e, int32_t *work_out, void *stream) {
diff --git a/deepmimic_mujoco_amd/csrc/dm_device.h b/deepmimic_mujoco_amd/csrc/dm_device.h
--- a/deepmimic_mujoco_amd/csrc/dm_device.h
+++ b/deepmimic_mujoco_amd/csrc/dm_device.h
@@ -78,6 +78,7 @@
   unsigned long long prof_t, prof_t0; unsigned prof[16], prof_stage[4];
 #endif
   int32_t info[8];
+  struct { int32_t idx_curr, ep_len, rcnt; float ep_rew; uint32_t f8r, f8l; int32_t work, motion, clip_i; uint32_t stage_ncon, stage_nefc; } car;
   int16_t rowinfo[DMK_MAXROW];
   union {
     struct {
@@ -99,6 +100,10 @@
     } bb;
   } u;
 };
+
+#ifndef DM_PROFILE
+static_assert(sizeof(EnvLds) <= 12800, "EnvLds beyond 12 800 B loses the twelfth wave per CU");
+#endif
 
 #define DMS_QPOS 0
 #define DMS_QVEL 35
@@ -123,6 +128,11 @@
 enum { DMK_MODE_STEP = 0, DMK_MODE_FORCED = 1, DMK_MODE_RESET = 2, DMK_MODE_SETSTATE = 3,
        DMK_MODE_PHYSICS = 4 };
 
+#define DMK_SCHED_NB 64
+#define DMK_SCHED_CNT 64
+#define DMK_SCHED_LIST (DMK_SCHED_CNT + 3 * DMK_SCHED_NB)
+#define DMK_SCHED_WORDS(N) ((size_t)DMK_SCHED_LIST + (size_t)3 * DMK_SCHED_NB * (size_t)(N))
+
 struct DmLaunch {
   const DmDev *T;
   float *state;
@@ -140,6 +150,7 @@
   const float *in_warm;
   const float *in_ctrl;
   const int32_t *env_ids;
+  int32_t *sched;
   int32_t *cost;
   const uint8_t *mask;
   const int32_t *idx_init;
diff --git a/deepmimic_mujoco_amd/csrc/dm_kernels.hip b/deepmimic_mujoco_amd/csrc/dm_kernels.hip
--- a/deepmimic_mujoco_amd/csrc/dm_kernels.hip
+++ b/deepmimic_mujoco_amd/csrc/dm_kernels.hip
@@ -1483,6 +1483,51 @@
   return qacc_out;
 }
 
+typedef __attribute__((address_space(1))) int32_t *gsched_p;
+__device__ __forceinline__ int sched_load(const int32_t *p) {
+  return __hip_atomic_load(p, __ATOMIC_RELAXED, __HIP_MEMORY_SCOPE_AGENT);
+}
+__device__ __forceinline__ int sched_env(const int32_t *sc, const int slot, const int N, const int lane) {
+  const int gen = __builtin_amdgcn_readfirstlane(sched_load(sc));
+  const int c = sched_load(sc + DMK_SCHED_CNT + gen * DMK_SCHED_NB + lane);
+  int incl = c;
+#pragma unroll
+  for (int d = 1; d < 64; d <<= 1) {
+    const int t = __shfl_up(incl, d);
+    if (lane >= d) incl += t;
+  }
+  const unsigned long long m = __ballot(incl > slot);
+  if (!m) return -1;
+  const int b = __ffsll((long long)m) - 1;
+  const int base = __builtin_amdgcn_readlane(incl - c, b);
+  return __builtin_amdgcn_readfirstlane(sc[DMK_SCHED_LIST + ((size_t)(gen * DMK_SCHED_NB + b)) * (size_t)N + (slot - base)]);
+}
+__device__ __forceinline__ void sched_file(int32_t *sc, const int env, const int work, const int N, const int nslots, const int lane) {
+  asm volatile("" : "+s"(sc));
+  int last = 0, next = 0;
+  if (lane == 0) {
+    const int gen = sched_load(sc);
+    next = gen == 2 ? 0 : gen + 1;
+    int w = work < 0 ? 0 : work >> 5;
+    const int b = DMK_SCHED_NB - 1 - (w > DMK_SCHED_NB - 1 ? DMK_SCHED_NB - 1 : w);
+    const int pos = atomicAdd(sc + DMK_SCHED_CNT + next * DMK_SCHED_NB + b, 1);
+    if (pos >= 0 && pos < N) sc[DMK_SCHED_LIST + ((size_t)(next * DMK_SCHED_NB + b)) * (size_t)N + pos] = env;
+    int one = 1;
+    asm volatile("" : "+v"(one) : "v"(pos));
+    last = (atomicAdd(sc + 1, one) == nslots - 1) ? 1 : 0;
+  }
+  last = __builtin_amdgcn_readfirstlane(last);
+  if (last) {
+    next = __builtin_amdgcn_readfirstlane(next);
+    const int clear = next == 2 ? 0 : next + 1;
+    __hip_atomic_store(sc + DMK_SCHED_CNT + clear * DMK_SCHED_NB + lane, 0, __ATOMIC_RELAXED, __HIP_MEMORY_SCOPE_AGENT);
+    if (lane == 0) {
+      __hip_atomic_store(sc + 1, 0, __ATOMIC_RELAXED, __HIP_MEMORY_SCOPE_AGENT);
+      __hip_atomic_store(sc, next, __ATOMIC_RELAXED, __HIP_MEMORY_SCOPE_AGENT);
+    }
+  }
+}
+
 template <int TASK>
 __device__ __forceinline__ void step_body(const DmLaunch &P) {
   constexpr int NOBS_T = TASK ? DM_NOBS_COMBINED : DM_NOBS;
@@ -1493,9 +1538,10 @@
   EnvLds &S = g_S;
   const int slot = blockIdx.x;
   if (slot >= P.nslots) return;
-  const int env = P.env_ids ? P.env_ids[slot] : slot;
+  const int env = P.sched ? sched_env(P.sched, slot, P.N, lane) : (P.env_ids ? P.env_ids[slot] : slot);
   if (env < 0 || env >= P.N) return;
   const int mode = P.mode;
+  const bool files = P.sched && mode == DMK_MODE_STEP;
   if (mode == DMK_MODE_RESET && P.mask && !P.mask[env]) return;
   float *st = P.state + (size_t)env * DMK_STATE_STRIDE;
   int *sti = reinterpret_cast<int *>(st);
@@ -1516,11 +1562,15 @@
     for (int i = 0; i < 10; i++) S.cinert[0][i] = 0;
   }
 
+  {
   const int clip_id = sti[DMS_CLIP];
   int motion = TASK ? ((clip_id >= 0 && clip_id < 4) ? clip_id : 0) : 0;
-  DmClipDev clip = P.clips[TASK ? (motion == 3 ? 2 : motion) : ((clip_id >= 0 && clip_id < 8) ? clip_id : 0)];
-  if (clip.L < 1 || clip.rows == nullptr) return;
-  if (TASK && (P.clips[0].L < 1 || P.clips[1].L < 1 || P.clips[2].L < 2)) return;
+  const int clip_i = (clip_id >= 0 && clip_id < 8) ? clip_id : 0;
+  DmClipDev clip = P.clips[TASK ? (motion == 3 ? 2 : motion) : clip_i];
+  if (clip.L < 1 || clip.rows == nullptr || (TASK && (P.clips[0].L < 1 || P.clips[1].L < 1 || P.clips[2].L < 2))) {
+    if (files) sched_file(P.sched, env, 0, P.N, P.nslots, lane);
+    return;
+  }
   int idx_curr = sti[DMS_IDX], ep_len = sti[DMS_EPLEN], rcnt = sti[DMS_RCNT];
   if (TASK) idx_curr = idx_curr < 0 ? 0 : idx_curr;
   else idx_curr = idx_curr < 0 ? 0 : (idx_curr >= clip.L ? clip.L - 1 : idx_curr);
@@ -1561,16 +1611,15 @@
     if (lane < DMK_NV) S.qvel[lane] = rr[35 + lane];
     ep_len = 0; ep_rew = 0; rcnt++;
   }
+  if (lane == 0) {
+    S.car.idx_curr = idx_curr; S.car.ep_len = ep_len; S.car.rcnt = rcnt; S.car.ep_rew = ep_rew; S.car.f8r = f8r; S.car.f8l = f8l;
+    S.car.motion = motion; S.car.clip_i = clip_i; S.car.work = 0; S.car.stage_ncon = 0; S.car.stage_nefc = 0;
+  }
+  }
   SYNC();
 
   int it = (mode == DMK_MODE_STEP || mode == DMK_MODE_PHYSICS) ? 0 : 4;
-  bool after_reset = false, done = false, sim_err = false;
-  int reason = DM_REASON_NONE;
-  float reward = 0;
-  int ncon = 0, nefc = 0, nlimit = 0, solver_iter = 0, overflow = 0;
-  float com[3] = {0, 0, 0};
-  unsigned stage_ncon = 0, stage_nefc = 0;
-  int work = 0;
+  bool after_reset = false, sim_err = false;
 
   if (mode == DMK_MODE_SETSTATE && !P.run_forward) {
     if (lane < DMK_NQ) st[DMS_QPOS + lane] = S.qpos[lane];
@@ -1586,6 +1635,7 @@
   PROF(0);
   for (;;) {
    float qacc_out = 0;
+   int ncon = 0, nefc = 0, nlimit = 0, solver_iter = 0, overflow = 0;
    if (!sim_err) {
     GDev *Tp = (GDev *)P.T;
     asm volatile("" : "+s"(Tp));
@@ -1611,8 +1661,10 @@
       qacc_out = fwd_constraint(Ts, lane_st, ncon, cr >> 8, P.debug ? P.debug + (size_t)env * DM_DEBUG_STRIDE + 352 : nullptr,
                                 P.ar_scratch + (size_t)env * DMK_MAXROW * DMK_MAXROW);
       nefc = S.info[1]; nlimit = S.info[2]; solver_iter = S.info[3]; overflow = S.info[4];
-      if (it < 4) { stage_ncon |= (unsigned)(ncon & 0xFF) << (8 * it); stage_nefc |= (unsigned)(nefc & 0xFF) << (8 * it); }
-      work = (work >> 1) + 64 + (nefc > 0 ? 48 + 16 * nefc : 0) + nefc * solver_iter;
+      if (P.debug && it < 4 && lane == 0) {
+        S.car.stage_ncon |= (unsigned)(ncon & 0xFF) << (8 * it); S.car.stage_nefc |= (unsigned)(nefc & 0xFF) << (8 * it);
+      }
+      if (lane == 0) S.car.work = (S.car.work >> 1) + 64 + (nefc > 0 ? 48 + 16 * nefc : 0) + nefc * solver_iter;
       if (P.f8) {
         bool rfs = false, lfs = false;
         if (lane < ncon) {
@@ -1622,8 +1674,8 @@
           lfs = fl && (g1 == Ts.lfoot_geom || g2 == Ts.lfoot_geom);
         }
         const unsigned keep = ncon >= 32 ? 0u : (~0u << ncon);
-        f8r = (f8r & keep) | (unsigned)__ballot(rfs);
-        f8l = (f8l & keep) | (unsigned)__ballot(lfs);
+        const unsigned f8r = (S.car.f8r & keep) | (unsigned)__ballot(rfs), f8l = (S.car.f8l & keep) | (unsigned)__ballot(lfs);
+        if (lane == 0) { S.car.f8r = f8r; S.car.f8l = f8l; }
       }
     }
     if (it == 0 || (it == 4 && mode == DMK_MODE_FORCED && !after_reset)) {
@@ -1631,6 +1683,11 @@
       sim_err = __any(badv);
     }
    }
+   {
+    int lane_r = lane;
+    asm volatile("" : "+v"(lane_r));
+    const int lane = lane_r;
+    const int lb = lane < DMK_NB ? lane : 0, lk = lane < DMK_NV ? lane : 0, lg = lane < DMK_NG ? lane : 0;
 
     const bool euler = (P.integrator == DM_INT_EULER) && (mode == DMK_MODE_STEP || mode == DMK_MODE_PHYSICS);
     float x0q = 0, x0v = 0, accq = 0, accv = 0, curv = 0;
@@ -1702,7 +1759,7 @@
     PROF_STAGE(it);
     if (mode == DMK_MODE_PHYSICS) {
       if (sim_err) {
-        f8r = f8l = 0;
+        if (lane == 0) S.car.f8r = S.car.f8l = 0;
         SYNC();
         if (lane < DMK_NQ) S.qpos[lane] = T.qpos0[lane];
         if (lane < DMK_NV) { S.qvel[lane] = 0; S.warm[lane] = 0; }
@@ -1712,12 +1769,19 @@
       break;
     }
     const bool task_pass = !after_reset && (mode == DMK_MODE_STEP || mode == DMK_MODE_FORCED);
+    int idx_curr = __builtin_amdgcn_readfirstlane(S.car.idx_curr), ep_len = __builtin_amdgcn_readfirstlane(S.car.ep_len);
+    int rcnt = __builtin_amdgcn_readfirstlane(S.car.rcnt), motion = TASK ? __builtin_amdgcn_readfirstlane(S.car.motion) : 0;
+    float ep_rew = __int_as_float(__builtin_amdgcn_readfirstlane(__float_as_int(S.car.ep_rew)));
+    DmClipDev clip = P.clips[TASK ? (motion == 3 ? 2 : motion) : __builtin_amdgcn_readfirstlane(S.car.clip_i)];
+    bool done = false;
+    int reason = DM_REASON_NONE;
+    float reward = 0;
     float obs_a = 0, obs_b = 0;
     float terms[5] = {0, 0, 0, 0, 0};
     float extra[3] = {0, 0, 0};
     if (sim_err) {
       reward = 0; done = true; reason = DM_REASON_SIM_ERROR;
-      f8r = f8l = 0;
+      if (lane == 0) S.car.f8r = S.car.f8l = 0;
       SYNC();
       if (lane < DMK_NQ) S.qpos[lane] = T.qpos0[lane];
       if (lane < DMK_NV) { S.qvel[lane] = 0; S.warm[lane] = 0; }
@@ -1746,7 +1810,7 @@
         rf = fl && (g1 == T.rfoot_geom || g2 == T.rfoot_geom);
         lf = fl && (g1 == T.lfoot_geom || g2 == T.lfoot_geom);
       }
-      const float rff = (P.f8 ? f8r != 0 : __any(rf)) ? 1.f : 0.f, lff = (P.f8 ? f8l != 0 : __any(lf)) ? 1.f : 0.f;
+      const float rff = (P.f8 ? S.car.f8r != 0 : __any(rf)) ? 1.f : 0.f, lff = (P.f8 ? S.car.f8l != 0 : __any(lf)) ? 1.f : 0.f;
       const int Lm = (TASK && motion == 3) ? P.to_getup_len : clip.L;
       const int frame = TASK ? ((motion == 3) ? 1 : idx_curr % clip.L) : idx_curr;
       if (TASK) {
@@ -1858,7 +1922,7 @@
       for (int i = lane; i < 84; i += 64) dbg[90 + i] = (&S.cvel[0][0])[i];
       if (lane < DMK_NV) { dbg[174 + lane] = S.qacc[lane]; dbg[208 + lane] = S.qacc_smooth[lane]; }
       if (lane == 0) { dbg[242] = ncon; dbg[243] = nefc; dbg[244] = solver_iter; dbg[245] = nlimit; dbg[246] = overflow;
-                       dbg[247] = __int_as_float((int)stage_ncon); dbg[248] = __int_as_float((int)stage_nefc); }
+                       dbg[247] = __int_as_float((int)S.car.stage_ncon); dbg[248] = __int_as_float((int)S.car.stage_nefc); }
       if (lane < DMK_MAXCON) {
         dbg[256 + 3 * lane] = (lane < ncon) ? (float)S.c_g1[lane] : -1.f;
         dbg[257 + 3 * lane] = (lane < ncon) ? (float)S.c_g2[lane] : -1.f;
@@ -1894,6 +1958,7 @@
         if (lane < DMK_NQ) S.qpos[lane] = rr[lane];
         if (lane < DMK_NV) S.qvel[lane] = rr[35 + lane];
         ep_len = 0; ep_rew = 0;
+        if (lane == 0) { S.car.idx_curr = idx_curr; S.car.ep_len = ep_len; S.car.rcnt = rcnt; S.car.ep_rew = ep_rew; S.car.motion = motion; }
         SYNC();
         after_reset = true;
         sim_err = false;
@@ -1905,7 +1970,9 @@
       P.obs[(size_t)env * NOBS_T + lane] = obs_a;
       if (lane < NOBS_B) P.obs[(size_t)env * NOBS_T + 64 + lane] = obs_b;
     }
+    if (lane == 0) { S.car.idx_curr = idx_curr; S.car.ep_len = ep_len; S.car.ep_rew = ep_rew; S.car.motion = motion; }
     break;
+   }
   }
 
   PROF(11);
@@ -1916,13 +1983,17 @@
     P.debug[(size_t)env * DM_DEBUG_STRIDE + 352 + lane] = (float)v;
     if (lane < 4) P.debug[(size_t)env * DM_DEBUG_STRIDE + 368 + lane] = (float)g_S.prof_stage[lane]; }
 #endif
-  if (lane < DMK_NQ) st[DMS_QPOS + lane] = S.qpos[lane];
-  if (lane < DMK_NV) { st[DMS_QVEL + lane] = S.qvel[lane]; st[DMS_WARM + lane] = S.warm[lane]; }
-  if (lane < DMK_NU) st[DMS_CTRL + lane] = S.ctrl[lane];
-  if (lane == 0) { sti[DMS_IDX] = idx_curr; sti[DMS_EPLEN] = ep_len; st[DMS_EPREW] = ep_rew; sti[DMS_RCNT] = rcnt; }
-  if (TASK && lane == 0) sti[DMS_CLIP] = motion;
-  if (P.f8 && lane == 0) { sti[DMS_F8R] = (int)f8r; sti[DMS_F8L] = (int)f8l; }
-  if (P.cost && lane == 0) P.cost[env] = work;
+  int lane_w = threadIdx.x & 63;
+  asm volatile("" : "+v"(lane_w));
+  if (lane_w < DMK_NQ) st[DMS_QPOS + lane_w] = S.qpos[lane_w];
+  if (lane_w < DMK_NV) { st[DMS_QVEL + lane_w] = S.qvel[lane_w]; st[DMS_WARM + lane_w] = S.warm[lane_w]; }
+  if (lane_w < DMK_NU) st[DMS_CTRL + lane_w] = S.ctrl[lane_w];
+  if (lane_w == 0) { sti[DMS_IDX] = S.car.idx_curr; sti[DMS_EPLEN] = S.car.ep_len; st[DMS_EPREW] = S.car.ep_rew; sti[DMS_RCNT] = S.car.rcnt; }
+  if (TASK && lane_w == 0) sti[DMS_CLIP] = S.car.motion;
+  if (P.f8 && lane_w == 0) { sti[DMS_F8R] = (int)S.car.f8r; sti[DMS_F8L] = (int)S.car.f8l; }
+  const int work = __builtin_amdgcn_readfirstlane(S.car.work);
+  if (P.cost && lane_w == 0) P.cost[env] = work;
+  if (P.sched && mode == DMK_MODE_STEP) sched_file(P.sched, env, work, P.N, P.nslots, lane_w);
 }
 
 extern "C" __global__ void __launch_bounds__(64 * DMK_ENVS_PER_BLOCK, DMK_WAVES_PER_SIMD) dm_step_kernel(DmLaunch P) {
diff --git a/include/deepmimic_hip.h b/include/deepmimic_hip.h
--- a/include/deepmimic_hip.h
+++ b/include/deepmimic_hip.h
@@ -95,6 +95,7 @@
 int dm_set_debug(DmHandle h, float *debug_buf);
 
 int dm_get_work(DmHandle h, int32_t *work_out, void *stream);
+int dm_get_launch_order(DmHandle h, int32_t *order_out, int32_t *bucket_out, void *stream);
 
 int dm_fill_random_actions(DmHandle h, float *actions, uint32_t step_index, void *stream);
 
```

Measured after the change: 9.697 million. 0.708x the previous value.
